# H263/review-based-recommender

Measured on AMD Instinct MI355X. Metric: (user,item) pairs/sec, DeepCoNN train step (fwd+MSE+bwd+clip+Adam), bsz256 2x512tok, higher is better.
Workload: dtype f32; 1 GPU; DeepCoNN cfg2: batch 256 pairs/GPU, 2x512-token docs, D=300, conv widths 3/5/7 x 50, latent 32, V=50002, fp32, Zipf ids; global_batch=256, parallelism=dp1, resident_batches=4, optimizer=HipClipAdam (clip + Adam, 2 launches; word-table gradient in compact row form)

## Files before the change

include/rbr_hip.h:

```cpp
#ifndef RBR_HIP_H
#define RBR_HIP_H

#include <stddef.h>
#include <stdint.h>

#ifdef __cplusplus
extern "C" {
#endif

#define RBR_MAX_WIDTHS 8

#define RBR_PAD_SAME 0
#define RBR_PAD_VALID 1
#define RBR_ACT_RELU 0
#define RBR_ACT_TANH 1

#define RBR_ERR_BAD_ARG (-1)
#define RBR_ERR_UNSUPPORTED (-2)

typedef struct rbr_textcnn_desc {
    int32_t n_docs;
    int32_t L;
    int32_t D;
    int32_t V;
    int32_t n_widths;
    int32_t kz[RBR_MAX_WIDTHS];
    int32_t ch[RBR_MAX_WIDTHS];
    int32_t pad_mode;
    int32_t act;
    int32_t padding_idx;
    int32_t flags;
} rbr_textcnn_desc;
#define RBR_CONV_PAD_RUNS 1
#define RBR_CONV_GATE_SPLIT(k) (((k) & 0xf) << 8)
#define RBR_CONV_GATE_SPLIT_OF(flags) (((flags) >> 8) & 0xf)
#define RBR_CONV_CLASS_STAMPED (1 << 19)
#define RBR_CONV_CLASS_PRECISION_OF(flags) (((flags) >> 16) & 0x3)
#define RBR_CONV_CLASS_T_BF16 (1 << 18)
void rbr_textcnn_desc_stamp(rbr_textcnn_desc* d);

int rbr_version(void);
const char* rbr_last_error(void);

int rbr_pair_begin(void);
int rbr_pair_next(void);
int rbr_pair_end(int32_t* n_paired, int32_t* n_single);
void rbr_pair_abort(void);


size_t rbr_textcnn_packed_floats(const rbr_textcnn_desc* d);
size_t rbr_textcnn_partial_elems(const rbr_textcnn_desc* d);

int rbr_textcnn_pack(const rbr_textcnn_desc* d, const float* const* W, float* packed, void* stream);

size_t rbr_textcnn_fwd_ws_bytes(const rbr_textcnn_desc* d);
void rbr_set_conv_mode(int32_t mode);
#define RBR_PROD_F32 0
#define RBR_PROD_BF16X3 1
#define RBR_PROD_BF16X2 2
#define RBR_PROD_BF16 3
void rbr_set_prod_precision(int32_t mode);
int32_t rbr_get_prod_precision(void);
void rbr_set_b16_storage(int32_t on);
int rbr_textcnn_conv_fwd(const rbr_textcnn_desc* d, const int64_t* ids, const uint8_t* mask, const float* gate,
                         const float* table, const float* const* W, const float* packed, float* pval, int32_t* pidx,
                         void* ws, void* stream);

int rbr_textcnn_prod_prepare(const rbr_textcnn_desc* d, const int64_t* ids, const uint8_t* mask, const float* const* W,
                             int32_t* pidx, void* ws, void* stream);
int rbr_textcnn_prod_table(const rbr_textcnn_desc* d, const float* table, void* ws, void* stream);
int rbr_textcnn_prod_pool(const rbr_textcnn_desc* d, const int64_t* ids, const uint8_t* mask, const float* gate,
                          float* pval, int32_t* pidx, void* ws, void* stream);
struct rbr_id_set;
int rbr_textcnn_prod_prepare_ids(const rbr_textcnn_desc* d, int32_t n_sets, const struct rbr_id_set* sets, int64_t* err,
                                 const int64_t* ids, const uint8_t* mask, const float* const* W, int32_t* pidx, void* ws,
                                 void* stream);

int rbr_textcnn_pool_finalize(const rbr_textcnn_desc* d, const float* pval, const int32_t* pidx,
                              const float* const* bias, float* feat, int32_t* argmax, void* stream);

size_t rbr_textcnn_bwd_ws_floats(const rbr_textcnn_desc* d);
int rbr_textcnn_bwd_dw(const rbr_textcnn_desc* d, const int64_t* ids, const uint8_t* mask, const float* gate,
                       const float* table, const float* feat, const int32_t* argmax, const float* d_feat,
                       float* const* dW, float* const* dbias, float* ws, void* stream);
int rbr_textcnn_bwd_dtable(const rbr_textcnn_desc* d, const int64_t* ids, const uint8_t* mask, const float* gate,
                           const float* table, const float* packed, const float* feat, const int32_t* argmax,
                           const float* d_feat, float* dtable, float* dgate, void* stream);
size_t rbr_textcnn_bwd_prod_ws_bytes(const rbr_textcnn_desc* d);
size_t rbr_textcnn_bwd_dtable_list_ws_bytes(const rbr_textcnn_desc* d);
int rbr_textcnn_bwd_dtable_list(const rbr_textcnn_desc* d, const int64_t* ids, const uint8_t* mask, const float* const* W,
                                const float* feat, const int32_t* argmax, const float* d_feat, void* ws, float* dtable,
                                void* stream);
#define RBR_G_BUILD 1
#define RBR_G_PRODUCT 2
#define RBR_G_ACCUMULATE 4
#define RBR_G_ROWS 8
#define RBR_G_ZEROED 16
int rbr_textcnn_bwd_dtable_prod_ex(const rbr_textcnn_desc* d, const int64_t* ids, const uint8_t* mask, const float* gate,
                                   const float* feat, const int32_t* argmax, const float* d_feat, void* fwd_ws, void* bwd_ws,
                                   float* dtable, float* dgate, float* sq_part, int32_t flags, void* stream);
size_t rbr_textcnn_row_grad_partials(const rbr_textcnn_desc* d);

int rbr_textcnn_token_list(const rbr_textcnn_desc* d, void* fwd_ws, const int32_t** row_of_token, const int32_t** n_rows,
                           const int64_t** tok_of_row, int32_t* cap);
size_t rbr_textcnn_bwd_dw_from_g_ws_floats(const rbr_textcnn_desc* d);
int rbr_textcnn_bwd_dw_from_g(const rbr_textcnn_desc* d, const float* table, const float* feat, const float* d_feat,
                              void* fwd_ws, void* bwd_ws, float* const* dW, float* const* dbias, float* ws, void* stream);
size_t rbr_textcnn_taps_count(const rbr_textcnn_desc* d);
int rbr_textcnn_bwd_taps(const rbr_textcnn_desc* d, const int64_t* ids, const uint8_t* mask, const float* feat,
                         const int32_t* argmax, const float* d_feat, int32_t* tok, float* val, void* stream);
size_t rbr_textcnn_dtable_from_taps_ws_bytes(const rbr_textcnn_desc* d, int32_t n_sets);
int rbr_textcnn_dtable_from_taps(const rbr_textcnn_desc* d, int32_t n_sets, const int32_t* tok, const float* val,
                                 const float* const* W, void* ws, float* dtable, void* stream);
int32_t rbr_textcnn_taps_owner_rows(const rbr_textcnn_desc* d, int32_t n_sets);
int rbr_textcnn_dtable_from_taps_owner(const rbr_textcnn_desc* d, int32_t n_sets, int32_t rank, const int32_t* tok,
                                       const float* val, const float* const* W, void* ws, float* slab, int32_t* overflow,
                                       void* stream);
int rbr_textcnn_bwd(const rbr_textcnn_desc* d, const int64_t* ids, const uint8_t* mask, const float* gate,
                    const float* table, const float* packed, const float* feat, const int32_t* argmax,
                    const float* d_feat, float* const* dW, float* const* dbias, float* dtable, float* dgate,
                    float* ws, void* stream);

int rbr_textcnn_saliency(const rbr_textcnn_desc* d, const int64_t* ids, const uint8_t* mask, const float* gate,
                         const float* table, const float* const* W, const float* feat, const int32_t* argmax,
                         const float* d_feat, float* sal, void* stream);

typedef struct rbr_head_params {
    const float* Wu; const float* bu; const float* Eu;
    const float* Wi; const float* bi; const float* Ei;
    const float* h;  const float* g;
    const float* ub; const float* ib;
} rbr_head_params;

typedef struct rbr_head_grads {
    float* dWu; float* dbu; float* dEu;
    float* dWi; float* dbi; float* dEi;
    float* dh;  float* dg;
    float* dub; float* dib;
} rbr_head_grads;

int rbr_pair_head_fwd(int32_t B, int32_t H, int32_t K, const float* u_feat, const float* i_feat,
                      const int64_t* u_id, const int64_t* i_id, const rbr_head_params* p, const float* drop,
                      float* ul, float* il, float* pred, void* stream);

int rbr_pair_head_fwd_train(int32_t B, int32_t H, int32_t K, const float* u_feat, const float* i_feat,
                            const int64_t* u_id, const int64_t* i_id, const rbr_head_params* p, float p_drop,
                            uint64_t seed, uint64_t* rng_state, float* drop_out, float* zero_buf, int64_t zero_n,
                            float* ul, float* il, float* pred, void* stream);

int rbr_pair_head_fwd_pool(const rbr_textcnn_desc* d, const float* pval, const int32_t* pidx, const float* const* bias,
                           float* feat, int32_t* argmax, const int64_t* first, int32_t K, const int64_t* u_id, const int64_t* i_id,
                           const rbr_head_params* p, const float* drop, float p_drop, uint64_t seed, uint64_t* rng_state,
                           float* drop_out, float* zero_buf, int64_t zero_n, float* ul, float* il, float* pred,
                           const float* target, float* loss, float* d_pred_unit, int32_t* ticket, void* stream);

size_t rbr_pair_head_fwd_pool_lds_bytes(const rbr_textcnn_desc* d, int32_t K, int32_t with_d_feat);
int rbr_pair_head_fwd_pool_ex(const rbr_textcnn_desc* d, const float* pval, const int32_t* pidx, const float* const* bias,
                              float* feat, int32_t* argmax, const int64_t* first, int32_t K, const int64_t* u_id, const int64_t* i_id,
                              const rbr_head_params* p, const float* drop, float p_drop, uint64_t seed, uint64_t* rng_state,
                              float* drop_out, float* zero_buf, int64_t zero_n, float* ul, float* il, float* pred,
                              const float* target, float* loss, float* d_pred_unit, int32_t* ticket, float* d_feat_unit,
                              void* stream);

size_t rbr_pair_head_bwd_ws_floats(int32_t B, int32_t K);
int rbr_pair_head_bwd(int32_t B, int32_t H, int32_t K, const float* u_feat, const float* i_feat,
                      const int64_t* u_id, const int64_t* i_id, const rbr_head_params* p, const float* drop,
                      const float* ul, const float* il, const float* d_pred, int32_t pad_u, int32_t pad_i,
                      const rbr_head_grads* g, float* d_ufeat, float* d_ifeat, float* ws, void* stream);
int rbr_dropout_multiplier(int64_t n, float p, uint64_t seed, uint64_t* state, float* out, void* stream);

int rbr_mse_loss_fwd(int64_t n, const float* pred, const float* target, float* loss, float* d_pred_unit, void* stream);
int rbr_pair_dot_fwd(int32_t B, int32_t K, const float* x, float* out, void* stream);
int rbr_pair_dot_bwd(int32_t B, int32_t K, const float* x, const float* d_out, float* d_x, void* stream);
int rbr_block_cat(int32_t B, int32_t C1, int32_t C2, const float* a, const float* b, const float* c, const float* d, float* out,
                  void* stream);
int rbr_block_split(int32_t B, int32_t C1, int32_t C2, const float* g, float* a, float* b, float* c, float* d, void* stream);
int rbr_mse_loss_bwd(int64_t n, const float* pred, const float* target, const float* d_loss, float* d_pred,
                     void* stream);

int rbr_bpr_loss_fwd(int32_t B, int32_t n_neg, const float* pred, const float* valid, float* loss, float* d_pred_unit,
                     void* stream);
int rbr_bpr_loss_bwd(int32_t B, int32_t n_neg, const float* pred, const float* valid, const float* d_loss, float* d_pred,
                     void* stream);

size_t rbr_pair_softmax_ws_bytes(int32_t B, int32_t K);
int rbr_pair_softmax_fwd(int32_t mode, int32_t B, int32_t K, const float* ul, const float* il, const float* h,
                         const float* row_bias, const float* col_bias, const float* drop, float p_drop, uint64_t seed,
                         uint64_t* rng_state, const int64_t* u_id, const int64_t* i_id, const int64_t* seen_off,
                         const int32_t* seen_item, int64_t seen_nnz, int32_t U, int64_t item_lo, const float* logq, float inv_temp,
                         float* loss, float* pos, float* d_ul, float* d_il, float* d_h, float* d_col_bias, float* d_row_bias,
                         uint64_t* call_out, void* ws, void* stream);
int rbr_pair_softmax_bwd(int32_t mode, int32_t B, int32_t K, const float* ul, const float* il, const float* h,
                         const float* row_bias, const float* col_bias, const float* drop, float p_drop, uint64_t seed,
                         const uint64_t* call, const int64_t* u_id, const int64_t* i_id, const int64_t* seen_off,
                         const int32_t* seen_item, int64_t seen_nnz, int32_t U, int64_t item_lo, const float* logq, float inv_temp,
                         const float* d_loss, float* pos_scratch, float* d_ul, float* d_il, float* d_h, float* d_col_bias,
                         float* d_row_bias, void* ws, void* stream);

typedef struct rbr_attn_params {
    const float* W_rv; const float* W_id; const float* h; const float* b1; const float* b2; const float* ebd;
} rbr_attn_params;

typedef struct rbr_attn_grads {
    float* dW_rv; float* dW_id; float* dh; float* db1; float* db2; float* debd;
} rbr_attn_grads;

int rbr_review_attn_fwd(int32_t B, int32_t R, int32_t H, int32_t A, const float* feat, const int64_t* other_id,
                        const rbr_attn_params* p, const float* drop, float* out, float* att, float* hid, void* stream);
size_t rbr_review_attn_bwd_ws_floats(int32_t B, int32_t R, int32_t H, int32_t A);
int rbr_review_attn_bwd(int32_t B, int32_t R, int32_t H, int32_t A, const float* feat, const int64_t* other_id,
                        const rbr_attn_params* p, const float* drop, const float* att, const float* hid, const float* d_out,
                        const float* d_att, int32_t pad_idx, const rbr_attn_grads* g, float* d_feat, float* ws,
                        void* stream);
int rbr_review_attn2_fwd(int32_t B, int32_t R, int32_t H, int32_t A, const float* feat, const int64_t* other_id,
                         const rbr_attn_params* p0, const rbr_attn_params* p1, const float* drop, float* out, float* att,
                         float* hid, void* stream);
int rbr_review_attn2_bwd(int32_t B, int32_t R, int32_t H, int32_t A, const float* feat, const int64_t* other_id,
                         const rbr_attn_params* p0, const rbr_attn_params* p1, const float* drop, const float* att,
                         const float* hid, const float* d_out, const float* d_att, int32_t pad_idx0, int32_t pad_idx1,
                         const rbr_attn_grads* g0, const rbr_attn_grads* g1, int64_t n_ebd0, int64_t n_ebd1, float* d_feat,
                         float* ws, void* stream);

int rbr_datt_local_gate_fwd(int32_t B, int32_t L, int32_t E, int32_t win, const int64_t* ids, const float* table,
                            const float* w, const float* b0, float* gate, void* stream);
int rbr_datt_global_gate_fwd(int32_t B, int32_t L, int32_t E, const int64_t* ids, const float* table,
                             const float* w, const float* b0, float* gate, void* stream);
size_t rbr_datt_gate_bwd_ws_floats(int32_t B, int32_t L, int32_t E, int32_t win, int32_t is_global);
size_t rbr_datt_local_gate_prod_ws_bytes(int32_t B, int32_t L, int32_t E, int32_t win, int32_t V);
int rbr_datt_local_gate_fwd_prod(int32_t B, int32_t L, int32_t E, int32_t win, int32_t V, const int64_t* ids, const float* table,
                                 const float* w, const float* b0, float* gate, void* ws, const void* rows, void* stream);
int rbr_datt_local_gate_bwd_prod(int32_t B, int32_t L, int32_t E, int32_t win, int32_t V, const int64_t* ids, const float* table,
                                 const float* w, const float* gate, const float* dgate, int32_t pad_idx, float* dw, float* db0,
                                 float* dtable, void* ws, const void* rows, int32_t accumulate, void* stream);
int rbr_datt_local_gate_bwd(int32_t B, int32_t L, int32_t E, int32_t win, const int64_t* ids, const float* table,
                            const float* w, const float* gate, const float* dgate, int32_t pad_idx, float* dw,
                            float* db0, float* dtable, float* ws, void* stream);
int rbr_datt_global_gate_bwd(int32_t B, int32_t L, int32_t E, const int64_t* ids, const float* table,
                             const float* w, const float* gate, const float* dgate, int32_t pad_idx, float* dw,
                             float* db0, float* dtable, float* ws, void* stream);
size_t rbr_datt_token_rows_ws_bytes(int32_t B, int32_t L, int32_t V);
int rbr_datt_token_rows(int32_t B, int32_t L, int32_t V, const int64_t* ids, void* rows, void* stream);
size_t rbr_datt_global_gate_bwd_rows_ws_floats(int32_t B, int32_t L, int32_t E, int32_t V);
int rbr_datt_global_gate_bwd_rows(int32_t B, int32_t L, int32_t E, int32_t V, const int64_t* ids, const float* table,
                                  const float* w, const float* gate, const float* dgate, int32_t pad_idx, float* dw,
                                  float* db0, float* dtable, float* ws, const void* rows, int32_t accumulate, void* stream);

int rbr_linear_fwd(int32_t N, int32_t IN, int32_t OUT, const float* x, const float* W, const float* b, int32_t relu,
                   const float* drop, float* y, void* stream);
size_t rbr_linear_bwd_ws_floats(int32_t N, int32_t OUT);
int rbr_linear_bwd(int32_t N, int32_t IN, int32_t OUT, const float* x, const float* W, const float* y, const float* d_y,
                   int32_t relu, const float* drop, float* d_x, float* dW, float* db, float* ws, void* stream);
// ... 104 lines not shown
```

review-based-recommender_amd/_lib.py:

```python
from __future__ import annotations

import ctypes as C
import os
import threading
from typing import Optional, Sequence

import torch

HERE = os.path.dirname(os.path.abspath(__file__))
LIB_PATH = os.environ.get("RBR_LIB_PATH") or os.path.join(HERE, "csrc", "librbr_hip.so")

RBR_MAX_WIDTHS = 8
PAD_SAME, PAD_VALID = 0, 1
ACT_RELU, ACT_TANH = 0, 1
PROD_F32, PROD_BF16X3, PROD_BF16X2, PROD_BF16 = 0, 1, 2, 3
SCORE_FM, SCORE_DOT = 0, 1
PROD_PRECISIONS = {"f32": PROD_F32, "bf16x3": PROD_BF16X3, "bf16x2": PROD_BF16X2, "bf16": PROD_BF16}

c_f32p = C.c_void_p
c_i64p = C.c_void_p
c_u8p = C.c_void_p
c_i32p = C.c_void_p
c_stream = C.c_void_p


class TextCNNDesc(C.Structure):
    _fields_ = [
        ("n_docs", C.c_int32), ("L", C.c_int32), ("D", C.c_int32), ("V", C.c_int32),
        ("n_widths", C.c_int32),
        ("kz", C.c_int32 * RBR_MAX_WIDTHS), ("ch", C.c_int32 * RBR_MAX_WIDTHS),
        ("pad_mode", C.c_int32), ("act", C.c_int32), ("padding_idx", C.c_int32), ("flags", C.c_int32),
    ]


class HeadParams(C.Structure):
    _fields_ = [(n, C.c_void_p) for n in ("Wu", "bu", "Eu", "Wi", "bi", "Ei", "h", "g", "ub", "ib")]


class HeadGrads(C.Structure):
    _fields_ = [(n, C.c_void_p) for n in ("dWu", "dbu", "dEu", "dWi", "dbi", "dEi", "dh", "dg", "dub", "dib")]


class AttnParams(C.Structure):
    _fields_ = [(n, C.c_void_p) for n in ("W_rv", "W_id", "h", "b1", "b2", "ebd")]


class IdSet(C.Structure):
    _fields_ = [("inp", C.c_void_p), ("out", C.c_void_p), ("n", C.c_int64), ("limit", C.c_int64), ("replace", C.c_int64)]


MAX_ID_SETS = 8


class RowGrad(C.Structure):
    _fields_ = [("tensor", C.c_int32), ("V", C.c_int32), ("D", C.c_int32), ("row_of_token", C.c_void_p), ("rows", C.c_void_p),
                ("sq_part", C.c_void_p), ("n_sq", C.c_int32), ("coef_out", C.c_void_p)]


G_BUILD, G_PRODUCT, G_ACCUMULATE, G_ROWS, G_ZEROED = 1, 2, 4, 8, 16


def conv_gate_split(k: int) -> int:
    return (int(k) & 0xF) << 8


class AttnGrads(C.Structure):
    _fields_ = [(n, C.c_void_p) for n in ("dW_rv", "dW_id", "dh", "db1", "db2", "debd")]


_PP = C.POINTER(C.c_void_p)
_DESC = C.POINTER(TextCNNDesc)
i32 = C.c_int32

SIGNATURES = {
    "rbr_version": (C.c_int, []),
    "rbr_last_error": (C.c_char_p, []),
    "rbr_pair_begin": (C.c_int, []),
    "rbr_pair_next": (C.c_int, []),
    "rbr_pair_end": (C.c_int, [C.POINTER(i32), C.POINTER(i32)]),
    "rbr_pair_abort": (None, []),
    "rbr_textcnn_packed_floats": (C.c_size_t, [_DESC]),
    "rbr_textcnn_partial_elems": (C.c_size_t, [_DESC]),
    "rbr_textcnn_pack": (C.c_int, [_DESC, _PP, c_f32p, c_stream]),
    "rbr_textcnn_fwd_ws_bytes": (C.c_size_t, [_DESC]),
    "rbr_set_conv_mode": (None, [i32]),
    "rbr_set_prod_precision": (None, [i32]),
    "rbr_get_prod_precision": (i32, []),
    "rbr_textcnn_desc_stamp": (None, [_DESC]),
    "rbr_set_b16_storage": (None, [i32]),
    "rbr_textcnn_conv_fwd": (C.c_int, [_DESC, c_i64p, c_u8p, c_f32p, c_f32p, _PP, c_f32p, c_f32p, c_i32p, C.c_void_p,
                                       c_stream]),
    "rbr_textcnn_prod_prepare": (C.c_int, [_DESC, c_i64p, c_u8p, _PP, c_i32p, C.c_void_p, c_stream]),
    "rbr_textcnn_prod_table": (C.c_int, [_DESC, c_f32p, C.c_void_p, c_stream]),
    "rbr_textcnn_prod_pool": (C.c_int, [_DESC, c_i64p, c_u8p, c_f32p, c_f32p, c_i32p, C.c_void_p, c_stream]),
    "rbr_textcnn_pool_finalize": (C.c_int, [_DESC, c_f32p, c_i32p, _PP, c_f32p, c_i32p, c_stream]),
    "rbr_textcnn_bwd_ws_floats": (C.c_size_t, [_DESC]),
    "rbr_textcnn_bwd_dw": (C.c_int, [_DESC, c_i64p, c_u8p, c_f32p, c_f32p, c_f32p, c_i32p, c_f32p, _PP, _PP, c_f32p,
                                     c_stream]),
    "rbr_textcnn_bwd_dtable": (C.c_int, [_DESC, c_i64p, c_u8p, c_f32p, c_f32p, c_f32p, c_f32p, c_i32p, c_f32p, c_f32p,
                                         c_f32p, c_stream]),
    "rbr_textcnn_bwd_prod_ws_bytes": (C.c_size_t, [_DESC]),
    "rbr_textcnn_bwd_dtable_prod_ex": (C.c_int, [_DESC, c_i64p, c_u8p, c_f32p, c_f32p, c_i32p, c_f32p, C.c_void_p, C.c_void_p,
                                                 c_f32p, c_f32p, c_f32p, i32, c_stream]),
    "rbr_textcnn_row_grad_partials": (C.c_size_t, [_DESC]),
    "rbr_textcnn_token_list": (C.c_int, [_DESC, C.c_void_p, _PP, _PP, _PP, C.POINTER(i32)]),
    "rbr_textcnn_prod_prepare_ids": (C.c_int, [_DESC, i32, C.POINTER(IdSet), C.c_void_p, c_i64p, c_u8p, _PP, c_i32p, C.c_void_p,
                                               c_stream]),
    "rbr_dedup_fold_rows": (C.c_int, [i32, i32, c_i64p, c_f32p, c_stream]),
    "rbr_pair_head_fwd_pool": (C.c_int, [_DESC, c_f32p, c_i32p, _PP, c_f32p, c_i32p, c_i64p, i32, c_i64p, c_i64p, C.POINTER(HeadParams),
                                         c_f32p, C.c_float, C.c_uint64, C.c_void_p, c_f32p, c_f32p, C.c_int64, c_f32p, c_f32p,
                                         c_f32p, c_f32p, c_f32p, c_f32p, c_i32p, c_stream]),
    "rbr_pair_head_fwd_pool_lds_bytes": (C.c_size_t, [_DESC, i32, i32]),
    "rbr_pair_head_fwd_pool_ex": (C.c_int, [_DESC, c_f32p, c_i32p, _PP, c_f32p, c_i32p, c_i64p, i32, c_i64p, c_i64p, C.POINTER(HeadParams),
                                            c_f32p, C.c_float, C.c_uint64, C.c_void_p, c_f32p, c_f32p, C.c_int64, c_f32p, c_f32p,
                                            c_f32p, c_f32p, c_f32p, c_f32p, c_i32p, c_f32p, c_stream]),
    "rbr_clip_adam_step_rows": (C.c_int, [i32, _PP, _PP, _PP, _PP, C.POINTER(C.c_int64), C.c_float, C.c_float, C.c_float,
                                          C.c_float, C.c_float, c_f32p, c_f32p, c_f32p, C.POINTER(RowGrad), c_stream]),
    "rbr_row_grad_to_dense": (C.c_int, [i32, i32, c_i32p, c_f32p, c_f32p, c_stream]),
    "rbr_textcnn_bwd_dtable_list_ws_bytes": (C.c_size_t, [_DESC]),
    "rbr_textcnn_bwd_dtable_list": (C.c_int, [_DESC, c_i64p, c_u8p, _PP, c_f32p, c_i32p, c_f32p, C.c_void_p, c_f32p, c_stream]),
    "rbr_textcnn_bwd_dw_from_g_ws_floats": (C.c_size_t, [_DESC]),
    "rbr_textcnn_bwd_dw_from_g": (C.c_int, [_DESC, c_f32p, c_f32p, c_f32p, C.c_void_p, C.c_void_p, _PP, _PP, c_f32p, c_stream]),
    "rbr_textcnn_taps_count": (C.c_size_t, [_DESC]),
    "rbr_textcnn_bwd_taps": (C.c_int, [_DESC, c_i64p, c_u8p, c_f32p, c_i32p, c_f32p, c_i32p, c_f32p, c_stream]),
    "rbr_textcnn_dtable_from_taps_ws_bytes": (C.c_size_t, [_DESC, i32]),
    "rbr_textcnn_dtable_from_taps": (C.c_int, [_DESC, i32, c_i32p, c_f32p, _PP, C.c_void_p, c_f32p, c_stream]),
    "rbr_textcnn_taps_owner_rows": (i32, [_DESC, i32]),
    "rbr_textcnn_dtable_from_taps_owner": (C.c_int, [_DESC, i32, i32, c_i32p, c_f32p, _PP, C.c_void_p, c_f32p, c_i32p, c_stream]),
    "rbr_textcnn_bwd": (C.c_int, [_DESC, c_i64p, c_u8p, c_f32p, c_f32p, c_f32p, c_f32p, c_i32p, c_f32p, _PP, _PP,
                                  c_f32p, c_f32p, c_f32p, c_stream]),
    "rbr_textcnn_saliency": (C.c_int, [_DESC, c_i64p, c_u8p, c_f32p, c_f32p, _PP, c_f32p, c_i32p, c_f32p, c_f32p, c_stream]),
    "rbr_datt_local_gate_prod_ws_bytes": (C.c_size_t, [i32, i32, i32, i32, i32]),
    "rbr_datt_local_gate_fwd_prod": (C.c_int, [i32, i32, i32, i32, i32, c_i64p, c_f32p, c_f32p, c_f32p, c_f32p, C.c_void_p,
                                               C.c_void_p, c_stream]),
    "rbr_datt_local_gate_bwd_prod": (C.c_int, [i32, i32, i32, i32, i32, c_i64p, c_f32p, c_f32p, c_f32p, c_f32p, i32, c_f32p,
                                               c_f32p, c_f32p, C.c_void_p, C.c_void_p, i32, c_stream]),
    "rbr_review_bag_fwd": (C.c_int, [i32, i32, i32, c_i64p, c_u8p, c_f32p, c_f32p, c_f32p, c_f32p, c_stream]),
    "rbr_review_bag_bwd_ws_bytes": (C.c_size_t, [i32, i32]),
    "rbr_review_bag_bwd": (C.c_int, [i32, i32, i32, i32, c_i64p, c_u8p, c_f32p, c_f32p, c_f32p, i32, c_f32p, C.c_void_p,
                                     c_stream]),
    "rbr_additive_attn_fwd": (C.c_int, [i32, i32, i32, i32, c_f32p, c_u8p, c_f32p, c_f32p, c_f32p, c_f32p, c_f32p, c_f32p,
                                        c_f32p, c_stream]),
    "rbr_additive_attn_bwd_ws_floats": (C.c_size_t, [i32, i32, i32, i32]),
    "rbr_additive_attn_bwd": (C.c_int, [i32, i32, i32, i32, c_f32p, c_u8p, c_f32p, c_f32p, c_f32p, c_f32p, c_f32p, c_f32p,
                                        c_f32p, c_f32p, c_f32p, c_f32p, c_f32p, c_stream]),
    "rbr_clip_adam_ws_floats": (C.c_size_t, []),
    "rbr_clip_adam_step": (C.c_int, [i32, _PP, _PP, _PP, _PP, C.POINTER(C.c_int64), C.c_float, C.c_float, C.c_float,
                                     C.c_float, C.c_float, c_f32p, c_f32p, c_f32p, c_stream]),
    "rbr_pair_head_fwd": (C.c_int, [i32, i32, i32, c_f32p, c_f32p, c_i64p, c_i64p, C.POINTER(HeadParams), c_f32p,
                                    c_f32p, c_f32p, c_f32p, c_stream]),
    "rbr_pair_head_fwd_train": (C.c_int, [i32, i32, i32, c_f32p, c_f32p, c_i64p, c_i64p, C.POINTER(HeadParams), C.c_float,
                                          C.c_uint64, C.c_void_p, c_f32p, c_f32p, C.c_int64, c_f32p, c_f32p, c_f32p, c_stream]),
    "rbr_pair_head_bwd_ws_floats": (C.c_size_t, [i32, i32]),
    "rbr_pair_head_bwd": (C.c_int, [i32, i32, i32, c_f32p, c_f32p, c_i64p, c_i64p, C.POINTER(HeadParams), c_f32p,
                                    c_f32p, c_f32p, c_f32p, i32, i32, C.POINTER(HeadGrads), c_f32p, c_f32p, c_f32p,
                                    c_stream]),
    "rbr_dropout_multiplier": (C.c_int, [C.c_int64, C.c_float, C.c_uint64, C.c_void_p, c_f32p, c_stream]),
    "rbr_mse_loss_fwd": (C.c_int, [C.c_int64, c_f32p, c_f32p, c_f32p, c_f32p, c_stream]),
    "rbr_pair_dot_fwd": (C.c_int, [i32, i32, c_f32p, c_f32p, c_stream]),
    "rbr_pair_dot_bwd": (C.c_int, [i32, i32, c_f32p, c_f32p, c_f32p, c_stream]),
    "rbr_block_cat": (C.c_int, [i32, i32, i32, c_f32p, c_f32p, c_f32p, c_f32p, c_f32p, c_stream]),
    "rbr_block_split": (C.c_int, [i32, i32, i32, c_f32p, c_f32p, c_f32p, c_f32p, c_f32p, c_stream]),
    "rbr_mse_loss_bwd": (C.c_int, [C.c_int64, c_f32p, c_f32p, c_f32p, c_f32p, c_stream]),
    "rbr_bpr_loss_fwd": (C.c_int, [i32, i32, c_f32p, c_f32p, c_f32p, c_f32p, c_stream]),
    "rbr_bpr_loss_bwd": (C.c_int, [i32, i32, c_f32p, c_f32p, c_f32p, c_f32p, c_stream]),
    "rbr_pair_softmax_ws_bytes": (C.c_size_t, [i32, i32]),
    "rbr_pair_softmax_fwd": (C.c_int, [i32, i32, i32, c_f32p, c_f32p, c_f32p, c_f32p, c_f32p, c_f32p, C.c_float, C.c_uint64,
                                       C.c_void_p, c_i64p, c_i64p, c_i64p, c_i32p, C.c_int64, i32, C.c_int64, c_f32p, C.c_float,
                                       c_f32p, c_f32p, c_f32p, c_f32p, c_f32p, c_f32p, c_f32p, C.c_void_p, C.c_void_p, c_stream]),
    "rbr_pair_softmax_bwd": (C.c_int, [i32, i32, i32, c_f32p, c_f32p, c_f32p, c_f32p, c_f32p, c_f32p, C.c_float, C.c_uint64,
                                       C.c_void_p, c_i64p, c_i64p, c_i64p, c_i32p, C.c_int64, i32, C.c_int64, c_f32p, C.c_float,
                                       c_f32p, c_f32p, c_f32p, c_f32p, c_f32p, c_f32p, c_f32p, C.c_void_p, c_stream]),
    "rbr_sample_negatives": (C.c_int, [i32, i32, i32, i32, c_i64p, c_i64p, c_i64p, c_i32p, C.c_int64, i32, C.c_uint64, C.c_void_p,
                                       i32, C.c_int64, c_i64p, c_i64p, c_f32p, c_stream]),
    "rbr_review_attn_fwd": (C.c_int, [i32, i32, i32, i32, c_f32p, c_i64p, C.POINTER(AttnParams), c_f32p, c_f32p, c_f32p,
                                      c_f32p, c_stream]),
    "rbr_review_attn_bwd_ws_floats": (C.c_size_t, [i32, i32, i32, i32]),
    "rbr_review_attn_bwd": (C.c_int, [i32, i32, i32, i32, c_f32p, c_i64p, C.POINTER(AttnParams), c_f32p, c_f32p, c_f32p,
                                      c_f32p, c_f32p, i32, C.POINTER(AttnGrads), c_f32p, c_f32p, c_stream]),
    "rbr_review_attn2_fwd": (C.c_int, [i32, i32, i32, i32, c_f32p, c_i64p, C.POINTER(AttnParams), C.POINTER(AttnParams), c_f32p,
                                       c_f32p, c_f32p, c_f32p, c_stream]),
    "rbr_review_attn2_bwd": (C.c_int, [i32, i32, i32, i32, c_f32p, c_i64p, C.POINTER(AttnParams), C.POINTER(AttnParams), c_f32p,
                                       c_f32p, c_f32p, c_f32p, c_f32p, i32, i32, C.POINTER(AttnGrads), C.POINTER(AttnGrads),
                                       C.c_int64, C.c_int64, c_f32p, c_f32p, c_stream]),
    "rbr_datt_local_gate_fwd": (C.c_int, [i32, i32, i32, i32, c_i64p, c_f32p, c_f32p, c_f32p, c_f32p, c_stream]),
    "rbr_datt_global_gate_fwd": (C.c_int, [i32, i32, i32, c_i64p, c_f32p, c_f32p, c_f32p, c_f32p, c_stream]),
    "rbr_datt_gate_bwd_ws_floats": (C.c_size_t, [i32, i32, i32, i32, i32]),
    "rbr_datt_local_gate_bwd": (C.c_int, [i32, i32, i32, i32, c_i64p, c_f32p, c_f32p, c_f32p, c_f32p, i32, c_f32p,
                                          c_f32p, c_f32p, c_f32p, c_stream]),
    "rbr_datt_global_gate_bwd": (C.c_int, [i32, i32, i32, c_i64p, c_f32p, c_f32p, c_f32p, c_f32p, i32, c_f32p,
                                           c_f32p, c_f32p, c_f32p, c_stream]),
    "rbr_datt_token_rows_ws_bytes": (C.c_size_t, [i32, i32, i32]),
    "rbr_datt_token_rows": (C.c_int, [i32, i32, i32, c_i64p, C.c_void_p, c_stream]),
    "rbr_datt_global_gate_bwd_rows_ws_floats": (C.c_size_t, [i32, i32, i32, i32]),
    "rbr_datt_global_gate_bwd_rows": (C.c_int, [i32, i32, i32, i32, c_i64p, c_f32p, c_f32p, c_f32p, c_f32p, i32, c_f32p,
                                                c_f32p, c_f32p, c_f32p, C.c_void_p, i32, c_stream]),
    "rbr_linear_fwd": (C.c_int, [i32, i32, i32, c_f32p, c_f32p, c_f32p, i32, c_f32p, c_f32p, c_stream]),
    "rbr_linear_bwd_ws_floats": (C.c_size_t, [i32, i32]),
    "rbr_linear_bwd": (C.c_int, [i32, i32, i32, c_f32p, c_f32p, c_f32p, c_f32p, i32, c_f32p, c_f32p, c_f32p, c_f32p,
                                 c_f32p, c_stream]),
    "rbr_linear_fwd_ws_floats": (C.c_size_t, [i32, i32, i32]),
    "rbr_linear_bwd_ex_ws_floats": (C.c_size_t, [i32, i32, i32]),
    "rbr_linear_fwd_ex": (C.c_int, [i32, i32, i32, c_f32p, c_f32p, c_f32p, i32, c_f32p, c_f32p, c_f32p, c_stream]),
    "rbr_linear_bwd_ex": (C.c_int, [i32, i32, i32, c_f32p, c_f32p, c_f32p, c_f32p, i32, c_f32p, c_f32p, c_f32p, c_f32p,
                                    c_f32p, c_stream]),
    "rbr_conv_shift_add_fwd": (C.c_int, [i32, i32, i32, C.POINTER(i32), C.POINTER(i32), c_f32p, _PP, c_f32p, c_stream]),
    "rbr_conv_shift_add_bwd": (C.c_int, [i32, i32, i32, C.POINTER(i32), C.POINTER(i32), c_f32p, c_f32p, _PP, c_stream]),
    "rbr_sanitize_ids": (C.c_int, [i32, C.POINTER(IdSet), C.c_void_p, c_stream]),
    "rbr_dedup_ws_bytes": (C.c_size_t, [i32, i32]),
    "rbr_dedup_rows": (C.c_int, [i32, i32, c_i64p, c_i64p, i32, i32, c_u8p, C.c_void_p, c_i64p, c_u8p, c_stream]),
    "rbr_doc_gather": (C.c_int, [i32, i32, c_i64p, c_i64p, c_i32p, i32, c_i32p, i32, C.c_int64, C.c_int64, c_i64p, c_u8p, c_i64p,
                                 c_i64p, c_stream]),
    "rbr_review_gather": (C.c_int, [i32, i32, i32, c_i64p, c_i64p, c_i32p, c_i32p, i32, c_i32p, c_i32p, i32, i32, C.c_int64, C.c_int64,
                                    c_i64p, c_u8p, c_u8p, c_i64p, c_i64p, c_i64p, c_stream]),
    "rbr_pair_score_ids": (C.c_int, [i32, i32, i32, c_f32p, i32, c_f32p, i32, c_i64p, c_i64p, c_f32p, c_f32p, c_f32p, c_f32p, c_f32p,
                                     c_i64p, c_stream]),
    "rbr_pair_score_dense": (C.c_int, [i32, i32, i32, i32, c_f32p, c_f32p, c_f32p, c_f32p, c_f32p, c_f32p, c_f32p, c_stream]),
    "rbr_pair_score_topk_ws_bytes": (C.c_size_t, [i32, i32, i32, i32]),
    "rbr_pair_score_topk": (C.c_int, [i32, i32, i32, i32, i32, i32, c_f32p, c_f32p, c_f32p, c_f32p, c_f32p, c_f32p, c_i64p, c_i32p,
                                      C.c_int64, c_i64p, i32, c_i64p, c_f32p, C.c_void_p, c_stream]),
    "rbr_pair_score_rank_ws_bytes": (C.c_size_t, [i32, i32, i32]),
    "rbr_pair_score_rank": (C.c_int, [i32, i32, i32, i32, i32, c_f32p, c_f32p, c_f32p, c_f32p, c_f32p, c_f32p, c_i64p, c_i64p, c_i32p,
                                      C.c_int64, c_i64p, i32, c_i32p, c_i32p, c_i64p, C.c_void_p, c_stream]),
    "rbr_embedding_fwd": (C.c_int, [C.c_int64, i32, c_i64p, c_f32p, c_f32p, c_stream]),
    "rbr_embedding_bwd": (C.c_int, [C.c_int64, i32, c_i64p, c_f32p, i32, c_f32p, c_stream]),
    "rbr_hier_pool_fwd": (C.c_int, [i32, i32, i32, i32, c_i64p, c_u8p, c_f32p, i32, c_f32p, c_i32p, c_stream]),
    "rbr_hier_pool_bwd": (C.c_int, [i32, i32, i32, i32, c_i64p, c_u8p, c_i32p, c_f32p, c_f32p, i32, i32, c_f32p,
                                    c_stream]),
}

_lib = None
_lock = threading.Lock()


def lib() -> C.CDLL:
    global _lib
    if _lib is not None:
        return _lib
    with _lock:
# ... 121 lines not shown
```

review-based-recommender_amd/csrc/pair_head.hip:

```cpp
#include "rbr_common.h"

#include <algorithm>

namespace rbr {

__device__ __forceinline__ void head_dl(float su, float si, float dr, float dp, float hk, float& dul, float& dil, float& zdp) {
    const float prod = su * si;
    const float dz = (prod > 0.f) ? dp * hk * dr : 0.f;
    dul = dz * si;
    dil = dz * su;
    zdp = fmaxf(prod, 0.f) * dr * dp;
}

__device__ __forceinline__ void head_pair_dfeat(int H, int K, const float* ulb, const float* ilb, const float* drb, float dp,
                                                const rbr_head_params& p, float* s_dul, float* s_dil, float* d_uf, float* d_if) {
    const int t = threadIdx.x;
    for (int k = t; k < K; k += 256) {
        const float dr = (drb != nullptr) ? drb[k] : 1.f;
        float dul, dil, zdp;
        head_dl(ulb[k], ilb[k], dr, dp, p.h[k], dul, dil, zdp);
        s_dul[k] = dul;
        s_dil[k] = dil;
    }
    __syncthreads();
// ... 142 lines not shown
__global__ __launch_bounds__(256) void head_fwd_pool_kernel(const ConvPlan P, const HeadPool hp, int B, int K,
                                                            const long long* __restrict__ uid, const long long* __restrict__ iid,
                                                            const rbr_head_params p, const float* __restrict__ drop,
                                                            float* __restrict__ ul, float* __restrict__ il, float* __restrict__ pred,
                                                            const HeadTrain tr, const HeadMse mse, float* __restrict__ d_feat_unit) {
    __shared__ float s_part[2][4][32];
    __shared__ float s_l[2][32];
    __shared__ int s_last;
    __shared__ float s_dp;
    extern __shared__ __attribute__((aligned(16))) float s_feat[];
    const int b = blockIdx.x, t = threadIdx.x;
    if (b >= B) {
        for (long k = (long)(b - B) * 256 + t; k < tr.zero_n; k += (long)(gridDim.x - B) * 256) tr.zero_buf[k] = 0.f;
        if (t == 0) head_rng_ticket(tr, 0);
        return;
    }
    const int* flags = hp.pidx + (long)P.total_wt * P.nslots_total;
    const int nslots = P.ntiles * kTile, wpd = P.wpd;
    float* s_val = s_feat + 2 * P.C;
    int* s_flag = reinterpret_cast<int*>(s_val + 2 * wpd * nslots);
    __shared__ short s_chan[kMaxSlots];
    __shared__ unsigned char s_sw[kMaxSlots], s_skz[kMaxSlots];
    __shared__ int s_choff[RBR_MAX_WIDTHS];
    __shared__ const float* s_biasp[RBR_MAX_WIDTHS];
    static_assert(kMaxSlots <= 256, "one thread per slot below");
    if (t < kMaxSlots) { s_chan[t] = P.slot_chan[t]; s_sw[t] = P.slot_w[t]; s_skz[t] = P.slot_kz[t]; }
    if (t < RBR_MAX_WIDTHS) { s_choff[t] = P.ch_off[t]; s_biasp[t] = hp.bias.p[t]; }
    __shared__ int s_src[2];
    if (t < 2) s_src[t] = hp.first != nullptr ? (int)hp.first[t * B + b] : t * B + b;
    __syncthreads();
    for (int i = t; i < 2 * wpd; i += 256) {
        const int side = i >= wpd, w = side ? i - wpd : i;
        s_flag[i] = flags[s_src[side] * wpd + w];
    }
    __syncthreads();
    const float NEG = -__builtin_huge_valf();
    for (int i = t; i < 2 * wpd * nslots; i += 256) {
        const int side = i >= wpd * nslots, r = side ? i - wpd * nslots : i;
        const int w = r / nslots, ls = r - w * nslots;
        const long base = ((long)s_src[side] * wpd + w) * P.nslots_total + (long)P.tile_base * kTile + ls;
        float v = NEG;
        if (s_chan[ls] >= 0) {
            const int Lv = (P.pad_mode == RBR_PAD_VALID) ? (P.L - (int)s_skz[ls] + 1) : P.L;
            const int fl = s_flag[side * wpd + w];
            v = (fl == 1) ? hp.pval[base] : ((fl == 0 && w * kTile < Lv) ? 0.f : NEG);
        }
        s_val[i] = v;
    }
    __syncthreads();
    for (int idx = t; idx < 2 * nslots; idx += 256) {
        const int side = idx >= nslots, ls = side ? idx - nslots : idx;
        const int doc = side * B + b;
        const int chan = s_chan[ls];
        if (chan < 0) continue;
        float best = NEG;
        int bw_tile = -1;
        for (int w = 0; w < wpd; ++w) {
            const float v = s_val[(side * wpd + w) * nslots + ls];
            if (v > best) { best = v; bw_tile = w; }
        }
        int bidx = 0;
        if (bw_tile >= 0) {
            if (s_flag[side * wpd + bw_tile] == 1) bidx = hp.pidx[((long)s_src[side] * wpd + bw_tile) * P.nslots_total + (long)P.tile_base * kTile + ls];
            else bidx = bw_tile * kTile;
        }
        const int bw = s_sw[ls];
        const float y = best + s_biasp[bw][chan - s_choff[bw]];
        const float f = (P.act == RBR_ACT_RELU) ? fmaxf(y, 0.f) : tanhf(y);
        hp.feat[(long)doc * P.C + chan] = f;
        hp.argmax[(long)doc * P.C + chan] = bidx;
        s_feat[side * P.C + chan] = f;
    }
    __syncthreads();
    float* s_bwd = d_feat_unit != nullptr ? s_feat + ((2 * P.C + 2 * wpd * nslots + 2 * wpd + 3) & ~3) : nullptr;
    const float pr = head_pair(b, B, P.C, K, s_feat, s_feat + P.C, uid, iid, p, drop, ul, il, pred, tr, s_part, s_l, s_bwd);
    if (mse.target == nullptr) return;
    if (d_feat_unit != nullptr) {
        const int K4 = (K + 3) & ~3;
        if (t == 0) s_dp = (pr - mse.target[b]) * (2.f / (float)B);
        __syncthreads();
        head_pair_dfeat(P.C, K, s_bwd, s_bwd + K4, s_bwd + 2 * K4, s_dp, p, s_bwd, s_bwd + K4, d_feat_unit + (long)b * P.C,
                        d_feat_unit + (long)(B + b) * P.C);
    }
    if (t == 0) {
        __threadfence();
        s_last = atomicAdd(mse.ticket, 1) == B - 1;
    }
    __syncthreads();
    if (!s_last) return;
    __threadfence();
    float acc = 0.f;
    for (int i = t; i < B; i += 256) {
        const float d = __hip_atomic_load(pred + i, __ATOMIC_RELAXED, __HIP_MEMORY_SCOPE_AGENT) - mse.target[i];
        acc += d * d;
        if (mse.d_unit != nullptr) mse.d_unit[i] = d * (2.f / (float)B);
    }
    acc = wave_sum(acc);
    __syncthreads();
    if ((t & 63) == 0) s_l[0][t >> 6] = acc;
    __syncthreads();
    if (t == 0) {
        *mse.loss = (s_l[0][0] + s_l[0][1] + s_l[0][2] + s_l[0][3]) / (float)B;
        *mse.ticket = 0;
    }
}

__global__ __launch_bounds__(256) void head_bwd_kernel(int B, int H, int K, const float* __restrict__ uf,
                                                       const float* __restrict__ itf, const long long* __restrict__ uid,
                                                       const long long* __restrict__ iid, const rbr_head_params p,
                                                       const float* __restrict__ drop, const float* __restrict__ ul,
                                                       const float* __restrict__ il, const float* __restrict__ d_pred,
                                                       int pad_u, int pad_i, const rbr_head_grads g,
                                                       float* __restrict__ d_uf, float* __restrict__ d_if) {
    extern __shared__ __attribute__((aligned(16))) float sm[];
    const int t = threadIdx.x;
    if ((int)blockIdx.x < B) {
        const int K4 = (K + 3) & ~3;
        const int b = blockIdx.x;
        float* s_dul = sm;
        float* s_dil = sm + K4;
        const long u = uid[b], it = iid[b];
        const float dp = d_pred[b];
        head_pair_dfeat(H, K, ul + (long)b * K, il + (long)b * K, drop != nullptr ? drop + (long)b * K : nullptr, dp, p, s_dul, s_dil,
                        d_uf != nullptr ? d_uf + (long)b * H : nullptr, d_uf != nullptr ? d_if + (long)b * H : nullptr);
        for (int k = t; k < K; k += 256) {
            if (u != pad_u) atomicAdd(g.dEu + u * K + k, s_dul[k]);
            if (it != pad_i) atomicAdd(g.dEi + it * K + k, s_dil[k]);
        }
        if (t == 0) {
            if (u != pad_u) atomicAdd(g.dub + u, dp);
            if (it != pad_i) atomicAdd(g.dib + it, dp);
        }
        return;
    }
    float (*red)[8][32] = reinterpret_cast<float (*)[8][32]>(sm);
    const int rows = H + 1;
    const int rb = blockIdx.x - B;
    const int side = rb / rows, r = rb % rows;
    const int kk = t & 31, grp = t >> 5;
    const float* ft = side ? itf : uf;
    for (int k0 = 0; k0 < K; k0 += 32) {
        const int k = k0 + kk;
        float s = 0.f, hs = 0.f, gs = 0.f;
        if (k < K) {
            const float hk = p.h[k];
            for (int b0 = grp; b0 < B; b0 += 64) {
                float vu[8], vi[8], vd[8], vp[8], vf[8];
#pragma unroll
                for (int u = 0; u < 8; ++u) {
                    const int b = b0 + 8 * u;
                    const bool ok = b < B;
                    const long bb = ok ? b : grp;
                    vu[u] = ul[bb * K + k];
                    vi[u] = il[bb * K + k];
                    vd[u] = (drop != nullptr) ? drop[bb * K + k] : 1.f;
                    vp[u] = ok ? d_pred[bb] : 0.f;
                    vf[u] = (r < H) ? ft[bb * H + r] : 0.f;
                }
#pragma unroll
                for (int u = 0; u < 8; ++u) {
                    float dul, dil, zdp;
                    head_dl(vu[u], vi[u], vd[u], vp[u], hk, dul, dil, zdp);
                    const float dl = side ? dil : dul;
                    if (r < H) {
                        s = fmaf(vf[u], dl, s);
                    } else {
                        s += dl;
                        if (side == 0) {
                            hs += zdp;
                            if (k == 0) gs += vp[u];
                        }
                    }
                }
            }
        }
        __syncthreads();
        red[0][grp][kk] = s; red[1][grp][kk] = hs; red[2][grp][kk] = gs;
        __syncthreads();
        if (grp == 0 && k < K) {
            float a = 0.f, bsum = 0.f, c = 0.f;
#pragma unroll
            for (int q = 0; q < 8; ++q) { a += red[0][q][kk]; bsum += red[1][q][kk]; c += red[2][q][kk]; }
            if (r < H) {
                (side ? g.dWi : g.dWu)[(long)r * K + k] = a;
            } else {
                (side ? g.dbi : g.dbu)[k] = a;
                if (side == 0) {
                    g.dh[k] = bsum;
                    if (k == 0) g.dg[0] = c;
                }
            }
        }
    }
}

}

using namespace rbr;

static bool head_args_ok(int B, int H, int K) {
    if (B <= 0 || H <= 0 || K <= 0) { set_error("bad head shape B=%d H=%d K=%d", B, H, K); return false; }
    return true;
}

namespace rbr {
__global__ __launch_bounds__(256) void mse_fwd_kernel(long n, const float* __restrict__ pred, const float* __restrict__ target,
                                                      float* __restrict__ loss, float* __restrict__ d_unit) {
    __shared__ float s_red[4];
    float acc = 0.f;
    for (long i = threadIdx.x; i < n; i += 256) {
        const float d = pred[i] - target[i];
        acc += d * d;
        if (d_unit != nullptr) d_unit[i] = d * (2.f / (float)n);
    }
    acc = wave_sum(acc);
    if ((threadIdx.x & 63) == 0) s_red[threadIdx.x >> 6] = acc;
    __syncthreads();
    if (threadIdx.x == 0) *loss = (s_red[0] + s_red[1] + s_red[2] + s_red[3]) / (float)n;
}

__global__ __launch_bounds__(256) void mse_bwd_kernel(long n, const float* __restrict__ pred, const float* __restrict__ target,
                                                      const float* __restrict__ d_loss, float* __restrict__ d_pred) {
    const long i = (long)blockIdx.x * 256 + threadIdx.x;
    if (i < n) d_pred[i] = (pred[i] - target[i]) * (2.f / (float)n) * d_loss[0];
}

__device__ __forceinline__ float bpr_softplus(float x) { return fmaxf(x, 0.f) + log1pf(expf(-fabsf(x))); }
__device__ __forceinline__ float bpr_sigmoid(float x) {
    const float e = expf(-fabsf(x));
    return x >= 0.f ? 1.f / (1.f + e) : e / (1.f + e);
}

__global__ __launch_bounds__(256) void bpr_loss_kernel(int B, int n_neg, const float* __restrict__ pred, const float* __restrict__ valid,
                                                       const float* __restrict__ d_loss, float* __restrict__ loss,
                                                       float* __restrict__ d_pred) {
    __shared__ float s_red[2][4];
    float acc = 0.f, cnt = 0.f;
    for (int b = threadIdx.x; b < B; b += 256) {
        const float p = pred[b];
        for (int j = 0; j < n_neg; ++j) {
// ... 55 lines not shown
extern "C" int rbr_bpr_loss_fwd(int32_t B, int32_t n_neg, const float* pred, const float* valid, float* loss, float* d_pred_unit,
                                void* stream) {
    if (!bpr_args_ok("bpr_loss_fwd", B, n_neg, pred)) return RBR_ERR_BAD_ARG;
    if (!loss) { set_error("bpr_loss_fwd: null pointer"); return RBR_ERR_BAD_ARG; }
    hipLaunchKernelGGL(rbr::bpr_loss_kernel, dim3(1), dim3(256), 0, (hipStream_t)stream, B, n_neg, pred, valid,
                       (const float*)nullptr, loss, d_pred_unit);
    RBR_CHECK_LAUNCH("bpr_loss_fwd launch");
    return 0;
}

extern "C" int rbr_bpr_loss_bwd(int32_t B, int32_t n_neg, const float* pred, const float* valid, const float* d_loss, float* d_pred,
                                void* stream) {
    if (!bpr_args_ok("bpr_loss_bwd", B, n_neg, pred)) return RBR_ERR_BAD_ARG;
    if (!d_loss || !d_pred) { set_error("bpr_loss_bwd: null pointer"); return RBR_ERR_BAD_ARG; }
    hipLaunchKernelGGL(rbr::bpr_loss_kernel, dim3(1), dim3(256), 0, (hipStream_t)stream, B, n_neg, pred, valid, d_loss,
                       (float*)nullptr, d_pred);
    RBR_CHECK_LAUNCH("bpr_loss_bwd launch");
    return 0;
}

extern "C" int rbr_pair_head_fwd(int32_t B, int32_t H, int32_t K, const float* u_feat, const float* i_feat,
                                 const int64_t* u_id, const int64_t* i_id, const rbr_head_params* p, const float* drop,
                                 float* ul, float* il, float* pred, void* stream) {
    if (!head_args_ok(B, H, K)) return RBR_ERR_BAD_ARG;
    if (!u_feat || !i_feat || !u_id || !i_id || !p || !ul || !il || !pred) { set_error("null pointer"); return RBR_ERR_BAD_ARG; }
    hipLaunchKernelGGL(head_fwd_kernel, dim3(B), dim3(256), 0, (hipStream_t)stream, B, H, K, u_feat, i_feat,
                       reinterpret_cast<const long long*>(u_id), reinterpret_cast<const long long*>(i_id), *p, drop, ul,
                       il, pred, HeadTrain{});
    RBR_CHECK_LAUNCH("pair_head_fwd launch");
    return 0;
}

extern "C" int rbr_pair_head_fwd_train(int32_t B, int32_t H, int32_t K, const float* u_feat, const float* i_feat,
                                       const int64_t* u_id, const int64_t* i_id, const rbr_head_params* p, float p_drop,
                                       uint64_t seed, uint64_t* rng_state, float* drop_out, float* zero_buf, int64_t zero_n,
                                       float* ul, float* il, float* pred, void* stream) {
    if (!head_args_ok(B, H, K)) return RBR_ERR_BAD_ARG;
    if (!u_feat || !i_feat || !u_id || !i_id || !p || !ul || !il || !pred) { set_error("null pointer"); return RBR_ERR_BAD_ARG; }
    if (!(p_drop >= 0.f && p_drop < 1.f)) { set_error("pair_head_fwd_train: p_drop=%f outside [0,1)", (double)p_drop); return RBR_ERR_BAD_ARG; }
    if (p_drop > 0.f && (!rng_state || !drop_out)) { set_error("pair_head_fwd_train: dropout needs rng_state and drop_out"); return RBR_ERR_BAD_ARG; }
    if (zero_n < 0 || (zero_n > 0 && !zero_buf)) { set_error("pair_head_fwd_train: bad zero buffer"); return RBR_ERR_BAD_ARG; }
    HeadTrain tr{};
    tr.p_drop = p_drop; tr.seed = seed;
    tr.rng_state = (p_drop > 0.f) ? reinterpret_cast<unsigned long long*>(rng_state) : nullptr;
    tr.drop_out = drop_out; tr.zero_buf = zero_buf; tr.zero_n = zero_n;
    const int zblocks = zero_n > 0 ? (int)std::min<long>((zero_n + 1023) / 1024, 256) : 0;
    hipLaunchKernelGGL(head_fwd_kernel, dim3(B + zblocks), dim3(256), 0, (hipStream_t)stream, B, H, K, u_feat, i_feat,
                       reinterpret_cast<const long long*>(u_id), reinterpret_cast<const long long*>(i_id), *p,
                       static_cast<const float*>(nullptr), ul, il, pred, tr);
    RBR_CHECK_LAUNCH("pair_head_fwd_train launch");
    return 0;
}

static size_t head_fwd_pool_lds(const ConvPlan& P, int K, bool with_d_feat) {
    size_t lds = ((size_t)2 * P.C + (size_t)2 * P.wpd * P.ntiles * kTile + (size_t)2 * P.wpd) * sizeof(float);
    if (with_d_feat) lds = ((lds + 15) & ~(size_t)15) + (size_t)3 * ((K + 3) & ~3) * sizeof(float);
    return lds;
}

extern "C" size_t rbr_pair_head_fwd_pool_lds_bytes(const rbr_textcnn_desc* d, int32_t K, int32_t with_d_feat) {
    ConvPlan plans[kMaxGroups];
    if (K <= 0 || build_plans(d, plans, kMaxTiles) != 1) return 0;
    const size_t lds = head_fwd_pool_lds(plans[0], K, with_d_feat != 0);
    return lds > 60 * 1024 ? 0 : lds;
}

extern "C" int rbr_pair_head_fwd_pool_ex(const rbr_textcnn_desc* d, const float* pval, const int32_t* pidx, const float* const* bias,
                                         float* feat, int32_t* argmax, const int64_t* first, int32_t K, const int64_t* u_id,
                                         const int64_t* i_id, const rbr_head_params* p, const float* drop, float p_drop, uint64_t seed,
                                         uint64_t* rng_state, float* drop_out, float* zero_buf, int64_t zero_n, float* ul, float* il,
                                         float* pred, const float* target, float* loss, float* d_pred_unit, int32_t* ticket,
                                         float* d_feat_unit, void* stream) {
    ConvPlan plans[kMaxGroups];
    const int ng = build_plans(d, plans, kMaxTiles);
    if (!ng) return RBR_ERR_BAD_ARG;
    if (ng != 1) { set_error("pair_head_fwd_pool: %d channel groups (one launch covers %d slots)", ng, kMaxSlots); return RBR_ERR_UNSUPPORTED; }
    if (d->n_docs % 2) { set_error("pair_head_fwd_pool: odd document count %d", d->n_docs); return RBR_ERR_BAD_ARG; }
    const int B = d->n_docs / 2, C = plans[0].C;
    if (!head_args_ok(B, C, K)) return RBR_ERR_BAD_ARG;
    if (!pval || !pidx || !bias || !feat || !argmax || !u_id || !i_id || !p || !ul || !il || !pred) { set_error("null pointer"); return RBR_ERR_BAD_ARG; }
    if (!(p_drop >= 0.f && p_drop < 1.f)) { set_error("pair_head_fwd_pool: p_drop=%f outside [0,1)", (double)p_drop); return RBR_ERR_BAD_ARG; }
    if (p_drop > 0.f && (!rng_state || !drop_out)) { set_error("pair_head_fwd_pool: dropout needs rng_state and drop_out"); return RBR_ERR_BAD_ARG; }
    if (zero_n < 0 || (zero_n > 0 && !zero_buf)) { set_error("pair_head_fwd_pool: bad zero buffer"); return RBR_ERR_BAD_ARG; }
    if (target != nullptr && (!loss || !ticket)) { set_error("pair_head_fwd_pool: the loss needs loss and ticket"); return RBR_ERR_BAD_ARG; }
    if (d_feat_unit != nullptr && !target) { set_error("pair_head_fwd_pool: d_feat_unit needs the loss target"); return RBR_ERR_BAD_ARG; }
    HeadTrain tr{};
    tr.p_drop = p_drop; tr.seed = seed;
    tr.rng_state = (p_drop > 0.f) ? reinterpret_cast<unsigned long long*>(rng_state) : nullptr;
    tr.drop_out = drop_out; tr.zero_buf = zero_buf; tr.zero_n = zero_n;
    HeadPool hp{};
    hp.pval = pval; hp.pidx = pidx; hp.feat = feat; hp.argmax = argmax; hp.first = reinterpret_cast<const long long*>(first);
    for (int w = 0; w < d->n_widths; ++w) hp.bias.p[w] = bias[w];
    HeadMse mse{target, loss, d_pred_unit, ticket};
    const int zblocks = zero_n > 0 ? (int)std::min<long>((zero_n + 1023) / 1024, 256) : 0;
    const size_t lds = head_fwd_pool_lds(plans[0], K, d_feat_unit != nullptr);
    if (lds > 60 * 1024) { set_error("pair_head_fwd_pool: %zu bytes of LDS for the slab partials (documents too long)", lds); return RBR_ERR_UNSUPPORTED; }
    hipLaunchKernelGGL(head_fwd_pool_kernel, dim3(B + zblocks), dim3(256), lds, (hipStream_t)stream,
                       plans[0], hp, B, K, reinterpret_cast<const long long*>(u_id), reinterpret_cast<const long long*>(i_id), *p,
                       (p_drop > 0.f) ? nullptr : drop, ul, il, pred, tr, mse, d_feat_unit);
    RBR_CHECK_LAUNCH("pair_head_fwd_pool launch");
    return 0;
}

extern "C" int rbr_pair_head_fwd_pool(const rbr_textcnn_desc* d, const float* pval, const int32_t* pidx, const float* const* bias,
                                      float* feat, int32_t* argmax, const int64_t* first, int32_t K, const int64_t* u_id,
                                      const int64_t* i_id, const rbr_head_params* p, const float* drop, float p_drop, uint64_t seed,
                                      uint64_t* rng_state, float* drop_out, float* zero_buf, int64_t zero_n, float* ul, float* il,
                                      float* pred, const float* target, float* loss, float* d_pred_unit, int32_t* ticket, void* stream) {
    return rbr_pair_head_fwd_pool_ex(d, pval, pidx, bias, feat, argmax, first, K, u_id, i_id, p, drop, p_drop, seed, rng_state, drop_out,
                                     zero_buf, zero_n, ul, il, pred, target, loss, d_pred_unit, ticket, nullptr, stream);
}

extern "C" size_t rbr_pair_head_bwd_ws_floats(int32_t B, int32_t K) { (void)B; (void)K; return 0; }

extern "C" int rbr_pair_head_bwd(int32_t B, int32_t H, int32_t K, const float* u_feat, const float* i_feat,
                                 const int64_t* u_id, const int64_t* i_id, const rbr_head_params* p, const float* drop,
                                 const float* ul, const float* il, const float* d_pred, int32_t pad_u, int32_t pad_i,
                                 const rbr_head_grads* g, float* d_ufeat, float* d_ifeat, float* ws, void* stream) {
    if (!head_args_ok(B, H, K)) return RBR_ERR_BAD_ARG;
    if (!u_feat || !i_feat || !u_id || !i_id || !p || !ul || !il || !d_pred || !g || (!d_ufeat != !d_ifeat)) {
        set_error("null pointer");
        return RBR_ERR_BAD_ARG;
    }
    (void)ws;
    const size_t lds = std::max((size_t)2 * ((K + 3) & ~3), (size_t)3 * 8 * 32) * sizeof(float);
    hipLaunchKernelGGL(head_bwd_kernel, dim3((unsigned)(B + 2 * (H + 1))), dim3(256), lds, (hipStream_t)stream, B, H, K, u_feat,
                       i_feat, reinterpret_cast<const long long*>(u_id), reinterpret_cast<const long long*>(i_id), *p, drop,
                       ul, il, d_pred, pad_u, pad_i, *g, d_ufeat, d_ifeat);
    RBR_CHECK_LAUNCH("pair_head_bwd launch");
    return 0;
}

namespace rbr {
__global__ __launch_bounds__(256) void pair_dot_fwd_kernel(int B, int K, const float* __restrict__ x, float* __restrict__ out) {
    const int b = blockIdx.x * 16 + (threadIdx.x >> 4), l = threadIdx.x & 15;
    float s = 0.f;
    if (b < B)
        for (int k = l; k < K; k += 16) s = fmaf(x[(long)b * K + k], x[(long)(B + b) * K + k], s);
    s = wave_sum<16>(s);
    if (b < B && l == 0) out[b] = s;
}

__global__ __launch_bounds__(256) void pair_dot_bwd_kernel(int B, int K, const float* __restrict__ x, const float* __restrict__ d_out,
                                                           float* __restrict__ d_x) {
    const long n = (long)2 * B * K;
    for (long e = (long)blockIdx.x * 256 + threadIdx.x; e < n; e += (long)gridDim.x * 256) {
        const int row = (int)(e / K), k = (int)(e - (long)row * K);
        const int b = row < B ? row : row - B, other = row < B ? row + B : row - B;
        d_x[e] = d_out[b] * x[(long)other * K + k];
    }
}
}

extern "C" int rbr_pair_dot_fwd(int32_t B, int32_t K, const float* x, float* out, void* stream) {
    if (B <= 0 || K <= 0 || !x || !out) { set_error("bad pair_dot arguments"); return RBR_ERR_BAD_ARG; }
    hipLaunchKernelGGL(pair_dot_fwd_kernel, dim3((B + 15) / 16), dim3(256), 0, (hipStream_t)stream, B, K, x, out);
    RBR_CHECK_LAUNCH("pair_dot fwd launch");
    return 0;
}

extern "C" int rbr_pair_dot_bwd(int32_t B, int32_t K, const float* x, const float* d_out, float* d_x, void* stream) {
    if (B <= 0 || K <= 0 || !x || !d_out || !d_x) { set_error("bad pair_dot arguments"); return RBR_ERR_BAD_ARG; }
    const long n = (long)2 * B * K;
    hipLaunchKernelGGL(pair_dot_bwd_kernel, dim3((unsigned)std::min<long>((n + 255) / 256, 2048)), dim3(256), 0, (hipStream_t)stream, B, K,
                       x, d_out, d_x);
    RBR_CHECK_LAUNCH("pair_dot bwd launch");
    return 0;
}
```

review-based-recommender_amd/csrc/rbr_common.h:

```cpp
#pragma once

#include <hip/hip_runtime.h>

#include <algorithm>
#include <cstdarg>
#include <cstdio>
#include <cstring>

#include "../../include/rbr_hip.h"
#include "rbr_launch.h"
#include "rbr_wave.h"

namespace rbr {

constexpr int kWave = 64;
constexpr int kTile = 32;
constexpr int kMaxTiles = 8;
constexpr int kMaxGroups = 32;
constexpr int kMaxSlots = kMaxTiles * kTile;
constexpr int kMaxKF = 9;
constexpr int kMaxDim = 1 << 14;
constexpr int kMaxChannels = kMaxGroups * kMaxTiles * kTile;
constexpr int kMaxPieces = kMaxTiles * kMaxKF;
constexpr int kWavesPerWG = 4;
// ... 5 lines not shown
    int KF;
    int P;
    int DC;
    int nchunks;
    int wpd;
    int total_wt;
    int nslots_total;
    int tile_base;
    int group;
    int store_rows;
    int ntiles;
    int npieces;
    int pad_mode, act;
    int tiles_total;
    int piece_st[kMaxPieces];
    short slot_chan[kMaxSlots];
    unsigned char slot_w[kMaxSlots];
    unsigned char slot_off[kMaxSlots];
    unsigned char slot_kz[kMaxSlots];
    int n_widths;
    int kz[RBR_MAX_WIDTHS], ch[RBR_MAX_WIDTHS], ch_off[RBR_MAX_WIDTHS];
    int gate_split;
    int pad_runs;
};

struct PtrArray {
    const float* p[RBR_MAX_WIDTHS];
};
struct MutPtrArray {
    float* p[RBR_MAX_WIDTHS];
};

__device__ __forceinline__ float act_grad(int act, float f, float d) {
    return (act == RBR_ACT_RELU) ? (f > 0.f ? d : 0.f) : d * (1.f - f * f);
}

void set_error(const char* fmt, ...);
int check_hip(hipError_t e, const char* what);

bool desc_valid(const rbr_textcnn_desc* d);
int build_plans(const rbr_textcnn_desc* d, ConvPlan* plans , int tiles_per_group = 5);
constexpr int kProdGroupTiles = 8;

int run_conv_groups(const ConvPlan* plans, int ngroups, const long long* ids, const unsigned char* mask, const float* gate,
                    const float* table, const float* packed, float* pval, int* pidx, const int* sched, hipStream_t st);
int run_token_product(const rbr_textcnn_desc* d, const long long* ids, const unsigned char* mask, const float* gate,
                      const float* table, const float* const* W, float* pval, int* pidx, void* ws, hipStream_t st);
int forced_conv_mode();
int prod_precision();
int prod_precision_of(const rbr_textcnn_desc* d);
bool prod_b16_applicable(const rbr_textcnn_desc* d);
int prod_b16_groups(int cp_real);
size_t prod_b16_image_bytes(const rbr_textcnn_desc* d, int cp_real);
struct B16Pack;
B16Pack prod_b16_pack_job(const rbr_textcnn_desc* d);
int prod_b16_gemm(const rbr_textcnn_desc* d, int cp_real, int cap, int pitch, const int* counter, const long long* tok_of_row,
                  const float* table, const void* bimg, void* T, void* a16, hipStream_t st);
bool prod_b16_rows_applicable(const rbr_textcnn_desc* d);
size_t prod_b16_rows_image_bytes(int KG, int D);
long prod_b16_rows_image_items(int KG, int D);
int prod_b16_rows_partials(int cap, int D);
int prod_b16_rows_gemm(int KG, int D, int cap, const int* counter, const float* G, const void* bimg_t, float* rows, float* sq_part, bool plain_bf16,
                       hipStream_t st);
bool prod_t_bf16(const rbr_textcnn_desc* d);
size_t prod_b16_rows_bytes(const rbr_textcnn_desc* d, int cap);
struct ZeroRegions {
    int* p[3];
    long n[3];
};
int zero_regions(const ZeroRegions& r, hipStream_t st);
inline int zero_words(void* p, size_t bytes, hipStream_t st) {
    ZeroRegions r{{static_cast<int*>(p), nullptr, nullptr}, {(long)(bytes / sizeof(int)), 0, 0}};
    return zero_regions(r, st);
}

struct IdSets {
    const long long* in[RBR_MAX_ID_SETS];
    long long* out[RBR_MAX_ID_SETS];
    long long n[RBR_MAX_ID_SETS], limit[RBR_MAX_ID_SETS], replace[RBR_MAX_ID_SETS];
    long long first[RBR_MAX_ID_SETS + 1];
    int count;
};
int fill_id_sets(int n_sets, const rbr_id_set* sets, IdSets& S);
__device__ __forceinline__ void sanitize_id(const IdSets& S, long long k, long long* __restrict__ err) {
    int s = 0;
#pragma unroll
    for (int q = 1; q < RBR_MAX_ID_SETS; ++q)
        if (q < S.count && k >= S.first[q]) s = q;
    const long long e = k - S.first[s];
    long long v = S.in[s][e];
    const bool bad = (unsigned long long)v >= (unsigned long long)S.limit[s];
    if (bad) {
        err[1] = v; err[2] = s;
        atomicAdd(reinterpret_cast<unsigned long long*>(err), 1ull);
        v = S.replace[s];
    }
    S.out[s][e] = v;
}

constexpr int kSlabDup = 2;
constexpr int kPadRunHalo = 8;
__device__ __forceinline__ void tile_scan_block(const ConvPlan& P, const unsigned char* __restrict__ mask,
                                                int* __restrict__ sched, int blk, const long long* __restrict__ ids = nullptr) {
    const int wt = blk * 256 + threadIdx.x;
    int act = 0;
    if (wt < P.total_wt) {
        act = 1;
        if (mask != nullptr) {
            const int doc = wt / P.wpd, l0 = (wt % P.wpd) * kTile;
            const int lo = max(0, l0 - P.P), hi = min(P.L, l0 + kTile + P.KF - 1 - P.P);
            act = 0;
            const unsigned char* row = mask + (long)doc * P.L;
            if (l0 + kTile <= P.L && ((((uintptr_t)(row + l0)) & 15) == 0)) {
                const uint4 a = *reinterpret_cast<const uint4*>(row + l0), c = *reinterpret_cast<const uint4*>(row + l0 + 16);
                unsigned halo = 0;
                for (int p = lo; p < l0; ++p) halo |= row[p];
                for (int p = l0 + kTile; p < hi; ++p) halo |= row[p];
                act = (a.x | a.y | a.z | a.w | c.x | c.y | c.z | c.w | halo) != 0;
            } else {
                for (int p = lo; p < hi; ++p) act |= mask[(long)doc * P.L + p];
            }
            act = act ? 1 : 0;
        }
        sched[wt] = act;
    }
    if (mask == nullptr && ids != nullptr && P.pad_runs >= 0) {
        __shared__ unsigned char s_own[256];
        bool own = false;
        if (wt < P.total_wt) {
            const int doc = wt / P.wpd, l0 = (wt % P.wpd) * kTile;
            const int lo = l0 - P.P - kPadRunHalo, hi = l0 + kTile + P.KF - 1 - P.P + kPadRunHalo;
            if (lo >= 0 && hi <= P.L) {
                const long long* row = ids + (long)doc * P.L;
                const long long pad = (long long)P.pad_runs;
                own = true;
                int p = lo;
                if ((((uintptr_t)(row + p)) & 15) == 0) {
                    for (; p + 16 <= hi && own; p += 16) {
                        longlong2 t[8];
#pragma unroll
                        for (int u = 0; u < 8; ++u) t[u] = *reinterpret_cast<const longlong2*>(row + p + 2 * u);
#pragma unroll
                        for (int u = 0; u < 8; ++u) own = own && t[u].x == pad && t[u].y == pad;
                    }
                }
                for (; p < hi && own; ++p) own = row[p] == pad;
            }
        }
        s_own[threadIdx.x] = own ? 1 : 0;
        __syncthreads();
        if (wt < P.total_wt && own && (wt % P.wpd) != 0) {
            bool prev;
            if (threadIdx.x > 0) {
                prev = s_own[threadIdx.x - 1] != 0;
            } else {
                const int doc = wt / P.wpd, l0 = (wt % P.wpd - 1) * kTile;
                const int lo = l0 - P.P - kPadRunHalo, hi = l0 + kTile + P.KF - 1 - P.P + kPadRunHalo;
                prev = lo >= 0 && hi <= P.L;
                for (int q = lo; q < hi && prev; ++q) prev = ids[(long)doc * P.L + q] == (long long)P.pad_runs;
            }
            if (prev) { act = kSlabDup; sched[wt] = act; }
        }
    }
    const unsigned long long b = __ballot(act == 1);
    act = act == 1;
    const int lane = threadIdx.x & 63;
    int base = 0;
    if (lane == 0 && b) base = atomicAdd(sched + 2 * (long)P.total_wt, __popcll(b));
    base = __shfl(base, 0);
    if (act) sched[(long)P.total_wt + base + __popcll(b & ((1ull << lane) - 1))] = wt;
}
int scan_tiles(const ConvPlan& p, const unsigned char* mask, int* sched, hipStream_t st);

inline int choose_dc(int D) {
    if (D % 4 != 0) return 20;
    const int cands[3] = {60, 52, 20};
    int best_pad = 1 << 30;
    for (int c : cands) best_pad = std::min(best_pad, ((D + c - 1) / c) * c);
    for (int c : cands)
        if (((D + c - 1) / c) * c * 100 <= best_pad * 108) return c;
    return 20;
}


__device__ __forceinline__ void philox_round(unsigned& c0, unsigned& c1, unsigned& c2, unsigned& c3, unsigned k0, unsigned k1) {
    const unsigned long long p0 = 0xD2511F53ull * c0, p1 = 0xCD9E8D57ull * c2;
    const unsigned n0 = (unsigned)(p1 >> 32) ^ c1 ^ k0, n1 = (unsigned)p1;
    const unsigned n2 = (unsigned)(p0 >> 32) ^ c3 ^ k1, n3 = (unsigned)p0;
    c0 = n0; c1 = n1; c2 = n2; c3 = n3;
}

__device__ __forceinline__ void philox4x32_10(unsigned long long quad, unsigned long long call, unsigned long long seed,
                                              unsigned& c0, unsigned& c1, unsigned& c2, unsigned& c3) {
    c0 = (unsigned)quad; c1 = (unsigned)(quad >> 32); c2 = (unsigned)call; c3 = (unsigned)(call >> 32);
    unsigned k0 = (unsigned)seed, k1 = (unsigned)(seed >> 32);
#pragma unroll
    for (int r = 0; r < 10; ++r) {
        philox_round(c0, c1, c2, c3, k0, k1);
        k0 += 0x9E3779B9u; k1 += 0xBB67AE85u;
    }
}
__device__ __forceinline__ bool dropout_keep(unsigned word, float p) {
    return (float)(word >> 8) * (1.f / 16777216.f) >= p;
}

}

#define RBR_CHECK_LAUNCH(what)                                   \
    do {                                                         \
        int _e = rbr::check_hip(hipGetLastError(), what);        \
        if (_e) return _e;                                       \
        if (rbr::pair_region_open()) {                           \
            rbr::set_error("%s: this entry point launches directly and cannot be used inside rbr_pair_begin / rbr_pair_end", what); \
            return RBR_ERR_UNSUPPORTED;                          \
        }                                                        \
    } while (0)
```

review-based-recommender_amd/csrc/textcnn_prod.hip:

```cpp
#include "rbr_common.h"
#include "textcnn_b16.h"

#include <rocprim/rocprim.hpp>

#include <algorithm>
#include <cstdlib>

namespace rbr {

struct ProdArgs {
    int n_docs, L, V, cap;
    int zrow;
    int pitch;
    int poff[RBR_MAX_WIDTHS];
    int rank_off[RBR_MAX_WIDTHS];
    int cp_real;
};
RBR_SHARED_KERNEL_ARG(ProdArgs);

__device__ __forceinline__ void mark_scan_kernel(const ConvPlan& P, int nb_scan, long n_tok, const long long* __restrict__ ids,
                                                        const unsigned char* __restrict__ mask, int* __restrict__ sched,
                                                        unsigned char* __restrict__ used) {
    if ((int)blockIdx.x < nb_scan) {
        tile_scan_block(P, mask, sched, blockIdx.x, ids);
        return;
    }
    const long nb = gridDim.x - nb_scan;
    for (long k = (long)(blockIdx.x - nb_scan) * 256 + threadIdx.x; k < n_tok; k += nb * 256)
        if (mask == nullptr || mask[k]) used[ids[k]] = 1;
}

__global__ __launch_bounds__(256) void prep_kernel(const IdSets S, long long* __restrict__ err, const ZeroRegions R, int nb_ids) {
    if ((int)blockIdx.x < nb_ids) {
        const long long total = S.first[S.count];
        for (long long k = (long long)blockIdx.x * 256 + threadIdx.x; k < total; k += (long long)nb_ids * 256) sanitize_id(S, k, err);
        return;
    }
    const long nz = R.n[0] + R.n[1] + R.n[2], nb = gridDim.x - nb_ids;
    for (long k = (long)(blockIdx.x - nb_ids) * 256 + threadIdx.x; k < nz; k += nb * 256) {
        if (k < R.n[0]) R.p[0][k] = 0;
        else if (k < R.n[0] + R.n[1]) R.p[1][k - R.n[0]] = 0;
        else R.p[2][k - R.n[0] - R.n[1]] = 0;
    }
}

struct PackJob {
    ConvPlan P;
    int n_widths, D, cp_real;
    int kz[RBR_MAX_WIDTHS], ch[RBR_MAX_WIDTHS], poff[RBR_MAX_WIDTHS];
};

__device__ __forceinline__ float prod_weight(const PackJob& J, const PtrArray& W, int pc, int d) {
    int w = 0;
#pragma unroll
    for (int k = 1; k < RBR_MAX_WIDTHS; ++k)
        if (k < J.n_widths && pc >= J.poff[k]) w = k;
    const int rel = pc - J.poff[w];
    const int j = rel / J.ch[w], cl = rel - j * J.ch[w];
    return W.p[w][((long)cl * J.D + d) * J.kz[w] + j];
}

__device__ __forceinline__ void compact_pack_kernel(const PackJob& J, int nb_compact, int V, int cap,
                                                           const unsigned char* __restrict__ used, int* __restrict__ row_of_token,
                                                           long long* __restrict__ tok_of_row, unsigned char* __restrict__ row_mask,
                                                           int* __restrict__ counter, float* __restrict__ zero_row, int pitch,
                                                           const PtrArray& W, float* __restrict__ packed, float* __restrict__ WT,
                                                           const B16Pack& JB, unsigned char* __restrict__ bimg) {
    if ((int)blockIdx.x < nb_compact) {
        if (blockIdx.x == 0)
            for (int k = threadIdx.x; k < pitch; k += 256) zero_row[k] = 0.f;
        __shared__ int s_cnt[4], s_wave[4];
        const int lane = threadIdx.x & 63, wave = threadIdx.x >> 6;
        const int below = blockIdx.x * 256;
        int c = 0;
        const int4* u4 = reinterpret_cast<const int4*>(used);
        for (int q = threadIdx.x; q < below / 16; q += 256) {
            const int4 m = u4[q];
            c += __popc(m.x) + __popc(m.y) + __popc(m.z) + __popc(m.w);
        }
        c = wave_sum(c);
        const int v = below + threadIdx.x;
        const int u = (v < V) ? used[v] : 0;
        const unsigned long long b = __ballot(u);
        if (lane == 0) { s_cnt[wave] = c; s_wave[wave] = __popcll(b); }
        __syncthreads();
        int base = (s_cnt[0] + s_cnt[1]) + (s_cnt[2] + s_cnt[3]);
        for (int k = 0; k < wave; ++k) base += s_wave[k];
        if (v < V) {
            int row = -1;
            if (u) {
                row = base + __popcll(b & ((1ull << lane) - 1));
                if (row < cap) { tok_of_row[row] = v; row_mask[row] = 1; } else row = -1;
            }
            row_of_token[v] = row;
        }
        if ((int)blockIdx.x == nb_compact - 1 && threadIdx.x == 0)
            *counter = (s_cnt[0] + s_cnt[1]) + (s_cnt[2] + s_cnt[3]) + s_wave[0] + s_wave[1] + s_wave[2] + s_wave[3];
        return;
    }
    const long nb = gridDim.x - nb_compact, b0 = blockIdx.x - nb_compact;
    const ConvPlan& P = J.P;
    const int DC = P.DC;
    const long n_img = packed != nullptr ? (long)P.nchunks * P.tiles_total * kTile * DC : 0;
    const long n_wt = (long)J.cp_real * J.D;
    const long n_b16 = bimg != nullptr ? b16_pack_items(JB) : 0;
    for (long idx = b0 * 256 + threadIdx.x; idx < n_img + n_wt + n_b16; idx += nb * 256) {
        if (idx >= n_img + n_wt) {
            b16_pack_item(JB, W, bimg, idx - n_img - n_wt);
        } else if (idx < n_img) {
            long r = idx;
            const int dd = (int)(r % DC); r /= DC;
            const int slot = (int)(r % kTile); r /= kTile;
            const int t = (int)(r % P.tiles_total);
            const int dc = (int)(r / P.tiles_total);
            const int pc = t * kTile + slot;
            const int d = dc * DC + dd;
            packed[idx] = (pc < J.cp_real && d < J.D) ? prod_weight(J, W, pc, d) : 0.f;
        } else {
            const long e = idx - n_img;
            const int pc = (int)(e / J.D), d = (int)(e - (long)pc * J.D);
            WT[e] = prod_weight(J, W, pc, d);
        }
    }
}

typedef float f32x4 __attribute__((ext_vector_type(4)));
typedef float f32x4u __attribute__((ext_vector_type(4), aligned(4)));

typedef unsigned u32x2u __attribute__((ext_vector_type(2), aligned(2)));
template <bool TB16>
__device__ __forceinline__ void gather_pool_kernel(const ConvPlan& P, const ProdArgs& A, const long long* __restrict__ ids,
                                                          const unsigned char* __restrict__ mask, const float* __restrict__ gate,
                                                          const int* __restrict__ row_of_token, const void* __restrict__ Tv,
                                                          const int* __restrict__ sched, float* __restrict__ pval,
                                                          int* __restrict__ pidx) {
    const float* T = static_cast<const float*>(Tv);
    const unsigned short* T16 = static_cast<const unsigned short*>(Tv);
    __shared__ int s_row[kWavesPerWG][kTile + kMaxKF];
    __shared__ float s_gate[kWavesPerWG][kTile + kMaxKF];
    __shared__ float s_gate_b[kWavesPerWG][kTile + kMaxKF];
    const int wave = threadIdx.x >> 6, lane = threadIdx.x & 63;
    const int n_active = sched[2 * (long)P.total_wt];
    const int slot_in_list = blockIdx.x * kWavesPerWG + wave;
    if (slot_in_list >= n_active) return;
    const int wt = sched[P.total_wt + slot_in_list];
    const int doc = wt / P.wpd, l0 = (wt % P.wpd) * kTile;
    const int L = P.L, XR = kTile + P.KF - 1;
    for (int r = lane; r < XR; r += 64) {
        const int p = l0 - P.P + r;
        int row = A.zrow;
        float gv = 1.f, gvb = 1.f;
        if (p >= 0 && p < L) {
            const long tok = (long)doc * L + p;
            if (mask == nullptr || mask[tok]) {
                const int rr = row_of_token[ids[tok]];
                row = rr >= 0 ? rr : A.zrow;
                if (gate != nullptr) {
                    gv = gate[tok];
                    if (P.gate_split > 0) gvb = gate[(long)P.n_docs * L + tok];
                }
            }
        }
        s_row[wave][r] = row;
        s_gate[wave][r] = gv;
        s_gate_b[wave][r] = gvb;
    }
    __builtin_amdgcn_wave_barrier();
    const float NEG = -__builtin_huge_valf();
    for (int w = 0; w < P.n_widths; ++w) {
        const int kz = P.kz[w], ch = P.ch[w];
        const int off = (P.pad_mode == RBR_PAD_SAME) ? (P.KF - kz) / 2 : 0;
        const int Lv = (P.pad_mode == RBR_PAD_VALID) ? (L - kz + 1) : L;
        const int nquads = (ch + 3) >> 2;
        const int lq = nquads <= 16 ? 4 : (nquads <= 32 ? 5 : 6);
        const int QL = 1 << lq, PS = 64 >> lq;
        const int ps = lane >> lq, ql = lane & (QL - 1);
        const float* sg = (P.gate_split > 0 && w >= P.gate_split) ? s_gate_b[wave] : s_gate[wave];
        for (int qb = 0; qb < nquads; qb += QL) {
            const int q = qb + ql;
            const bool valid = q < nquads;
            const float* tcol = T + A.poff[w] + 4 * (valid ? q : 0);
            const unsigned short* tcol16 = T16 + A.poff[w] + 4 * (valid ? q : 0);
            float best[4] = {NEG, NEG, NEG, NEG};
            int bidx[4] = {0x7fffffff, 0x7fffffff, 0x7fffffff, 0x7fffffff};
            for (int p0 = 0; p0 < kTile; p0 += 2 * PS) {
                f32x4 y[2] = {{0.f, 0.f, 0.f, 0.f}, {0.f, 0.f, 0.f, 0.f}};
#pragma unroll
                for (int j = 0; j < kMaxKF; ++j) {
                    if (j < kz) {
#pragma unroll
                        for (int u = 0; u < 2; ++u) {
                            const int r = p0 + PS * u + ps + j + off;
                            f32x4 v;
                            if (TB16) {
                                const u32x2u b = *reinterpret_cast<const u32x2u*>(tcol16 + (long)s_row[wave][r] * A.pitch + j * ch);
                                v = f32x4{__uint_as_float(b.x << 16), __uint_as_float(b.x & 0xffff0000u),
                                          __uint_as_float(b.y << 16), __uint_as_float(b.y & 0xffff0000u)};
                            } else {
                                v = *reinterpret_cast<const f32x4u*>(tcol + (long)s_row[wave][r] * A.pitch + j * ch);
                            }
                            const float gv = sg[r];
                            y[u].x = fmaf(v.x, gv, y[u].x); y[u].y = fmaf(v.y, gv, y[u].y);
                            y[u].z = fmaf(v.z, gv, y[u].z); y[u].w = fmaf(v.w, gv, y[u].w);
                        }
                    }
                }
// ... 974 lines not shown
        A.t_pitch = pp[0].nslots_total;
    }
    int cp_real = 0;
    for (int w = 0; w < d->n_widths; ++w) {
        A.kz[w] = d->kz[w]; A.ch[w] = d->ch[w]; A.ch_off[w] = plans[0].ch_off[w];
        A.poff[w] = cp_real; cp_real += d->kz[w] * d->ch[w];
    }
    const bool want_g = dtable != nullptr || !(phases & kGProduct);
    if (phases & kGBuild) {
        if ((want_g && !(phases & kGZeroed)) || dgate != nullptr || B.rows_gemm) {
            const long n_img = B.rows_gemm ? prod_b16_rows_image_items(B.KG, d->D) : 0;
            const int nb_zero = 2048, nb_img = (int)std::min<long>((n_img + 255) / 256, 1024);
            if (int e_ = rbr::launch<zero_g_rows_kernel, 256>(dim3(nb_zero + nb_img), dim3(256), 0, st, "textcnn zero_g_rows launch", counter, Lo.cap, B.KG / 4, (want_g && !(phases & kGZeroed)) ? reinterpret_cast<f32x4*>(G) : nullptr, dgate, dgate != nullptr ? (long)d->n_docs * d->L * (RBR_CONV_GATE_SPLIT_OF(d->flags) ? 2 : 1) : 0L, nb_zero, WT, cp_real, d->D, n_img, reinterpret_cast<unsigned char*>(static_cast<char*>(bwd_ws) + B.bimg_t))) return e_;
        }
        const long n_items = (long)d->n_docs * A.C * A.KF;
        if (int e_ = rbr::launch<build_g_kernel, 256>(dim3((unsigned)((n_items + 255) / 256)), dim3(256), 0, st, "textcnn build_g launch", A, reinterpret_cast<const long long*>(ids), mask, gate, row_of_token, T, feat, argmax, d_feat, want_g ? G : nullptr, dgate, prod_t_bf16(d) ? 1 : 0)) return e_;
    }
    if (dtable == nullptr || !(phases & kGProduct)) return 0;
    const size_t lds = (size_t)B.KGW * 8 * kWavesPerWG + (size_t)kWavesPerWG * d->D * sizeof(float);
    const dim3 grid((unsigned)std::min(Lo.cap, kGtwMaxBlocks));
    if (phases & kGRows) {
        if (sq_part == nullptr) { set_error("compact row gradient needs sq_part"); return RBR_ERR_BAD_ARG; }
        if (B.rows_gemm)
            return prod_b16_rows_gemm(B.KG, d->D, Lo.cap, counter, G, static_cast<char*>(bwd_ws) + B.bimg_t, dtable, sq_part,
                                      prod_precision_of(d) == RBR_PROD_BF16, st);
        if (int e_ = rbr::launch<g_times_w_kernel<kGtwRows>, 256>(grid, dim3(256), lds, st, "textcnn g_times_w launch", A, B.KGW, counter, G, WT, tok_of_row, row_of_token, d->V, dtable, sq_part)) return e_;
    } else if (phases & kGAccumulate) {
        if (int e_ = rbr::launch<g_times_w_kernel<kGtwAccumulate>, 256>(grid, dim3(256), lds, st, "textcnn g_times_w launch", A, B.KGW, counter, G, WT, tok_of_row, row_of_token, d->V, dtable, (float*)nullptr)) return e_;
    } else {
        if (int e_ = rbr::launch<g_times_w_kernel<kGtwDense>, 256>(grid, dim3(256), lds, st, "textcnn g_times_w launch", A, B.KGW, counter, G, WT, tok_of_row, row_of_token, d->V, dtable, (float*)nullptr)) return e_;
    }
    return 0;
}

namespace {

struct ProdState {
    ProdLayout Lo;
    ConvPlan pp[kMaxGroups];
    ProdArgs A;
    unsigned char* used;
    int *row_of_token, *counter, *sched_p;
    long long* tok_of_row;
    unsigned char* row_mask;
    float *packed_p, *WT, *T;
    char* base;
};

int prod_state(const rbr_textcnn_desc* d, void* ws, ProdState& S) {
    if (ws == nullptr) { set_error("null workspace"); return RBR_ERR_BAD_ARG; }
    if (!prod_applicable(d)) { set_error("token-product path does not apply to this shape"); return RBR_ERR_UNSUPPORTED; }
    if (!prod_layout(d, S.Lo)) return RBR_ERR_BAD_ARG;
    const ProdLayout& Lo = S.Lo;
    S.base = static_cast<char*>(ws);
    S.used = reinterpret_cast<unsigned char*>(S.base + Lo.used);
    S.row_of_token = reinterpret_cast<int*>(S.base + Lo.row_of_token);
    S.tok_of_row = reinterpret_cast<long long*>(S.base + Lo.tok_of_row);
    S.row_mask = reinterpret_cast<unsigned char*>(S.base + Lo.row_mask);
    S.counter = reinterpret_cast<int*>(S.base + Lo.counter);
    S.sched_p = reinterpret_cast<int*>(S.base + Lo.sched);
    S.packed_p = reinterpret_cast<float*>(S.base + Lo.packed);
    S.WT = reinterpret_cast<float*>(S.base + Lo.wt);
    S.T = reinterpret_cast<float*>(S.base + Lo.table_T);
    if (!build_plans(&S.Lo.dp, S.pp, kProdGroupTiles)) return RBR_ERR_BAD_ARG;
    S.pp[0].store_rows = 1;
    ProdArgs A{};
    A.n_docs = d->n_docs; A.L = d->L; A.V = d->V; A.cap = Lo.cap; A.zrow = Lo.cap; A.pitch = S.pp[0].nslots_total;
    int o = 0;
    for (int w = 0; w < d->n_widths; ++w) { A.poff[w] = o; o += d->kz[w] * d->ch[w]; }
    A.cp_real = o;
    for (int w = 0; w < d->n_widths; ++w) {
        int r = 0;
        for (int v = 0; v < d->n_widths; ++v)
            if (d->kz[v] < d->kz[w] || (d->kz[v] == d->kz[w] && v < w)) r += d->ch[v];
        A.rank_off[w] = r;
    }
    S.A = A;
    return 0;
}

}

static int prod_prepare(const rbr_textcnn_desc* d, const int64_t* ids, const uint8_t* mask, const float* const* W, int32_t* pidx,
                        void* ws, void* stream, const IdSets* id_sets, int64_t* err) {
    ConvPlan plans[kMaxGroups];
    if (!build_plans(d, plans)) return RBR_ERR_BAD_ARG;
    if (!ids || !W || !pidx) { set_error("null pointer"); return RBR_ERR_BAD_ARG; }
    ProdState S;
    if (int e = prod_state(d, ws, S)) return e;
    hipStream_t st = (hipStream_t)stream;
    int* sched = pidx + (size_t)plans[0].total_wt * plans[0].nslots_total;
    ZeroRegions zr{{reinterpret_cast<int*>(S.base + S.Lo.used), S.sched_p + 2 * (size_t)S.pp[0].total_wt,
                    sched + 2 * (size_t)plans[0].total_wt},
                   {(long)((S.Lo.row_of_token - S.Lo.used) / sizeof(int)), kSchedCounters, kSchedCounters}};
    if (id_sets != nullptr) {
        const long long total = id_sets->first[id_sets->count];
        const int nb_ids = (int)std::min<long long>((total + 255) / 256, 2048);
        const long nz = zr.n[0] + zr.n[1] + zr.n[2];
        const int nb_zero = (int)std::min<long>((nz + 255) / 256, 256);
        hipLaunchKernelGGL(prep_kernel, dim3(nb_ids + nb_zero), dim3(256), 0, st, *id_sets, reinterpret_cast<long long*>(err), zr, nb_ids);
        RBR_CHECK_LAUNCH("textcnn prep launch");
    } else if (int e = zero_regions(zr, st)) {
        return e;
    }
    const long n_tok = (long)d->n_docs * d->L;
    const int nb_scan = (plans[0].total_wt + 255) / 256;
    const int nb_mark = (int)std::min<long>((n_tok + 255) / 256, 2048);
    if (int e_ = rbr::launch<mark_scan_kernel, 256>(dim3(nb_scan + nb_mark), dim3(256), 0, st, "textcnn mark_scan launch", plans[0], nb_scan, n_tok, reinterpret_cast<const long long*>(ids), mask, sched, S.used)) return e_;
    PackJob J{};
    J.P = S.pp[0]; J.n_widths = d->n_widths; J.D = d->D; J.cp_real = S.A.cp_real;
    for (int w = 0; w < d->n_widths; ++w) { J.kz[w] = d->kz[w]; J.ch[w] = d->ch[w]; J.poff[w] = S.A.poff[w]; }
    PtrArray wp{};
    for (int w = 0; w < d->n_widths; ++w) wp.p[w] = W[w];
    const int nb_compact = (d->V + 255) / 256;
    const bool b16 = prod_b16_applicable(d);
    B16Pack JB{};
    if (b16) JB = prod_b16_pack_job(d);
    const long n_pack = (b16 ? (long)JB.ngroups * JB.nchunks * 4 * 64 : (long)S.pp[0].nchunks * S.pp[0].tiles_total * kTile * S.pp[0].DC) +
                        (long)S.A.cp_real * d->D;
    const int nb_pack = (int)std::min<long>((n_pack + 255) / 256, 2048);
    if (int e_ = rbr::launch<compact_pack_kernel, 256>(dim3(nb_compact + nb_pack), dim3(256), 0, st, "textcnn compact_pack launch", J, nb_compact, d->V, S.Lo.cap, S.used, S.row_of_token, S.tok_of_row, S.row_mask, S.counter, prod_t_bf16(d) ? reinterpret_cast<float*>(reinterpret_cast<unsigned short*>(S.T) + (size_t)S.Lo.cap * S.A.pitch)
                                      : S.T + (size_t)S.Lo.cap * S.A.pitch, prod_t_bf16(d) ? S.A.pitch / 2 : S.A.pitch, wp, b16 ? nullptr : S.packed_p, S.WT, JB, b16 ? reinterpret_cast<unsigned char*>(S.base + S.Lo.bimg) : nullptr)) return e_;
    return 0;
}

extern "C" int rbr_textcnn_prod_prepare(const rbr_textcnn_desc* d, const int64_t* ids, const uint8_t* mask,
                                        const float* const* W, int32_t* pidx, void* ws, void* stream) {
    return prod_prepare(d, ids, mask, W, pidx, ws, stream, nullptr, nullptr);
}

extern "C" int rbr_textcnn_prod_prepare_ids(const rbr_textcnn_desc* d, int32_t n_sets, const rbr_id_set* sets, int64_t* err,
                                            const int64_t* ids, const uint8_t* mask, const float* const* W, int32_t* pidx, void* ws,
                                            void* stream) {
    if (!err) { set_error("null err"); return RBR_ERR_BAD_ARG; }
    IdSets S;
    if (int e = fill_id_sets(n_sets, sets, S)) return e;
    const long long n_tok = (long long)d->n_docs * d->L;
    const bool one = sets[0].out == ids && sets[0].n == n_tok;
    const bool two = n_sets >= 2 && sets[0].out == ids && sets[1].out == sets[0].out + sets[0].n && sets[0].n + sets[1].n == n_tok;
    if (!one && !two) { set_error("prod_prepare_ids: `ids` is not the clean copy of the first id set(s)"); return RBR_ERR_BAD_ARG; }
    return prod_prepare(d, ids, mask, W, pidx, ws, stream, &S, err);
}

namespace {
constexpr size_t kListMaxG = (size_t)256 << 20;
bool list_bwd_layout(const rbr_textcnn_desc* d, ProdLayout& Lo, ProdBwdLayout& B, size_t& list_bytes) {
    if (!prod_layout(d, Lo) || !prod_bwd_layout(d, Lo, B)) return false;
    if (B.total > kListMaxG) return false;
    ConvPlan pp[kMaxGroups];
    if (!build_plans(&Lo.dp, pp, kProdGroupTiles)) return false;
    list_bytes = Lo.table_T + align256((size_t)pp[0].nslots_total * sizeof(float));
    return true;
}
}

extern "C" size_t rbr_textcnn_bwd_dtable_list_ws_bytes(const rbr_textcnn_desc* d) {
    ConvPlan plans[kMaxGroups];
    if (!build_plans(d, plans)) return 0;
    static const char* env = getenv("RBR_DTABLE_MODE");
    if (env && !strcmp(env, "scatter")) return 0;
    ProdLayout Lo; ProdBwdLayout B; size_t list_bytes;
    if (!list_bwd_layout(d, Lo, B, list_bytes)) return 0;
    return align256(list_bytes) + B.total;
}

extern "C" int rbr_textcnn_bwd_dtable_list(const rbr_textcnn_desc* d, const int64_t* ids, const uint8_t* mask, const float* const* W,
                                           const float* feat, const int32_t* argmax, const float* d_feat, void* ws, float* dtable,
                                           void* stream) {
    ConvPlan plans[kMaxGroups];
    if (!build_plans(d, plans)) return RBR_ERR_BAD_ARG;
    if (!ids || !W || !feat || !argmax || !d_feat || !ws || !dtable) { set_error("null pointer"); return RBR_ERR_BAD_ARG; }
    ProdLayout Lo; ProdBwdLayout B; size_t list_bytes;
    if (!list_bwd_layout(d, Lo, B, list_bytes)) { set_error("token-list table gradient does not apply to this shape"); return RBR_ERR_UNSUPPORTED; }
    hipStream_t st = (hipStream_t)stream;
    char* base = static_cast<char*>(ws);
    ConvPlan pp[kMaxGroups];
    if (!build_plans(&Lo.dp, pp, kProdGroupTiles)) return RBR_ERR_BAD_ARG;
    int* sched_p = reinterpret_cast<int*>(base + Lo.sched);
    ZeroRegions zr{{reinterpret_cast<int*>(base + Lo.used), sched_p + 2 * (size_t)pp[0].total_wt, nullptr},
                   {(long)((Lo.row_of_token - Lo.used) / sizeof(int)), kSchedCounters, 0}};
    if (int e = zero_regions(zr, st)) return e;
    const long n_tok = (long)d->n_docs * d->L;
    if (int e_ = rbr::launch<mark_scan_kernel, 256>(dim3((unsigned)std::min<long>((n_tok + 255) / 256, 2048)), dim3(256), 0, st, "textcnn mark launch", plans[0], 0, n_tok, reinterpret_cast<const long long*>(ids), mask, (int*)nullptr, reinterpret_cast<unsigned char*>(base + Lo.used))) return e_;
    PackJob J{};
    J.P = pp[0]; J.n_widths = d->n_widths; J.D = d->D;
    int o = 0;
    for (int w = 0; w < d->n_widths; ++w) { J.kz[w] = d->kz[w]; J.ch[w] = d->ch[w]; J.poff[w] = o; o += d->kz[w] * d->ch[w]; }
    J.cp_real = o;
    PtrArray wp{};
    for (int w = 0; w < d->n_widths; ++w) wp.p[w] = W[w];
    const int nb_compact = (d->V + 255) / 256;
    const int nb_pack = (int)std::min<long>(((long)J.cp_real * d->D + 255) / 256, 2048);
    if (int e_ = rbr::launch<compact_pack_kernel, 256>(dim3(nb_compact + nb_pack), dim3(256), 0, st, "textcnn compact launch", J, nb_compact, d->V, Lo.cap, reinterpret_cast<unsigned char*>(base + Lo.used), reinterpret_cast<int*>(base + Lo.row_of_token), reinterpret_cast<long long*>(base + Lo.tok_of_row), reinterpret_cast<unsigned char*>(base + Lo.row_mask), reinterpret_cast<int*>(base + Lo.counter), reinterpret_cast<float*>(base + Lo.table_T), pp[0].nslots_total, wp, (float*)nullptr, reinterpret_cast<float*>(base + Lo.wt), B16Pack{}, (unsigned char*)nullptr)) return e_;
    return dtable_through_list(d, plans, ids, mask, nullptr, feat, argmax, d_feat, base, base + align256(list_bytes), dtable, nullptr, st);
}

extern "C" int rbr_textcnn_prod_table(const rbr_textcnn_desc* d, const float* table, void* ws, void* stream) {
    if (!table) { set_error("null pointer"); return RBR_ERR_BAD_ARG; }
    PairSolo solo;
    ProdState S;
    if (int e = prod_state(d, ws, S)) return e;
    if (prod_b16_applicable(d))
        return prod_b16_gemm(d, S.A.cp_real, S.Lo.cap, S.A.pitch, S.counter, S.tok_of_row, table, S.base + S.Lo.bimg, S.T,
                             S.base + S.Lo.a16, (hipStream_t)stream);
    return run_conv_groups(S.pp, 1, S.tok_of_row, S.row_mask, nullptr, table, S.packed_p, S.T, nullptr, S.sched_p, (hipStream_t)stream);
}

extern "C" int rbr_textcnn_prod_pool(const rbr_textcnn_desc* d, const int64_t* ids, const uint8_t* mask, const float* gate,
                                     float* pval, int32_t* pidx, void* ws, void* stream) {
    ConvPlan plans[kMaxGroups];
    const int ngroups = build_plans(d, plans);
    if (!ngroups) return RBR_ERR_BAD_ARG;
    if (!ids || !pval || !pidx) { set_error("null pointer"); return RBR_ERR_BAD_ARG; }
    PairSolo solo;
    ProdState S;
    if (int e = prod_state(d, ws, S)) return e;
    hipStream_t st = (hipStream_t)stream;
    const int* sched = pidx + (size_t)plans[0].total_wt * plans[0].nslots_total;
    const int max_items = (plans[0].total_wt + kWavesPerWG - 1) / kWavesPerWG;
    if (prod_t_bf16(d))
        { if (int e_ = rbr::launch<gather_pool_kernel<true>, 256>(dim3(max_items), dim3(256), 0, st, "textcnn gather_pool launch", plans[0], S.A, reinterpret_cast<const long long*>(ids), mask, gate, S.row_of_token, static_cast<const void*>(S.T), sched, pval, pidx)) return e_; }
    else
        if (int e_ = rbr::launch<gather_pool_kernel<false>, 256>(dim3(max_items), dim3(256), 0, st, "textcnn gather_pool launch", plans[0], S.A, reinterpret_cast<const long long*>(ids), mask, gate, S.row_of_token, static_cast<const void*>(S.T), sched, pval, pidx)) return e_;
    return 0;
// ... 236 lines not shown
```

review-based-recommender_amd/functional.py:

```python
from __future__ import annotations

import contextlib
import ctypes as C
import os
import weakref
from typing import Optional, Sequence

import torch

from . import _lib
from ._lib import ACT_RELU, ACT_TANH, PAD_SAME, PAD_VALID, TIMER, check, current_stream, dev_ptr, ptr_array

F32, I64, I32, U8 = torch.float32, torch.int64, torch.int32, torch.uint8


def _mask_u8(mask: Optional[torch.Tensor]) -> Optional[torch.Tensor]:
    if mask is None:
        return None
    if mask.dtype == torch.bool:
        return mask.contiguous().view(torch.uint8)
    if mask.dtype == torch.uint8:
        return mask.contiguous()
    raise RuntimeError(f"mask must be bool or uint8, got {mask.dtype}")

# ... 168 lines not shown
            raise RuntimeError(f"{name} must be a contiguous {dtype} tensor of shape {list(shape)}, got {t.dtype} {list(t.shape)}")
    if B == 0:
        return revs, word_masks, rev_masks, rids, ids
    _call(None, _lib.lib().rbr_review_gather, B, R, T, dev_ptr(u_ids, I64, "u_ids"), dev_ptr(i_ids, I64, "i_ids"),
          dev_ptr(user_revs, I32, "user_revs"), dev_ptr(user_rids, I32, "user_rids"), user_revs.shape[0],
          dev_ptr(item_revs, I32, "item_revs"), dev_ptr(item_rids, I32, "item_rids"), item_revs.shape[0],
          int(bool(leave_one_out)), int(pad_token), int(replace_id), dev_ptr(revs, I64, "revs"),
          dev_ptr(word_masks.view(U8), U8, "word_masks"), dev_ptr(None if rev_masks is None else rev_masks.view(U8), U8, "rev_masks"),
          dev_ptr(rids, I64, "rids"), dev_ptr(ids, I64, "ids"), _id_err(dev).data_ptr(), current_stream())
    return revs, word_masks, rev_masks, rids, ids


def set_tap_sink(sink, table: Optional[torch.Tensor] = None) -> None:
    if sink is None:
        if table is None:
            _TAP_SINKS.clear()
        else:
            _TAP_SINKS.pop(table.data_ptr(), None)
        return
    _TAP_SINKS[sink.table.data_ptr()] = sink


def _fanout_acc(table: torch.Tensor):
    node = table.grad_fn
    return getattr(node, "acc", None) if type(node).__name__ == "_TableFanoutBackward" else None


def _table_acc(acc, device):
    if acc is None or acc[1] != torch.cuda.current_stream(device):
        return None
    return acc[0]


class _TableFanout(torch.autograd.Function):

    @staticmethod
    def forward(ctx, table, n):
        ctx.set_materialize_grads(False)
        ctx.acc = (torch.zeros_like(table), torch.cuda.current_stream(table.device))
        return tuple(table.view(table.shape) for _ in range(n))

    @staticmethod
    def backward(ctx, *grads):
        total, seen = None, set()
        for g in grads:
            if g is None or g.data_ptr() in seen:
                continue
            seen.add(g.data_ptr())
            total = g if total is None else total + g
        return total, None


def table_fanout(table: torch.Tensor, n: int):
    if not (torch.is_grad_enabled() and table.requires_grad and table.is_cuda):
        return (table,) * n
    return _TableFanout.apply(table, n)


class _ConvSaved:

    def __init__(self, **kw):
        self.__dict__.update(kw)


def _conv_desc(table, n_docs, L, ws, pad_mode, act, padding_idx, flags: int = 0):
    V, D = table.shape
    return _lib.make_desc(n_docs, L, D, V, [int(w.shape[2]) for w in ws], [int(w.shape[0]) for w in ws], pad_mode, act, padding_idx,
                          flags)


def _conv_operands(table, ids, mask, weights, pad_mode, act, padding_idx, flags: int = 0):
    table_c = table.contiguous()
    dev_ptr(table_c, F32, "word table")
    if ids.dim() != 2:
        raise RuntimeError("ids must be [n_docs, L]")
    ids = ids.contiguous()
    mask8 = _mask_u8(mask)
    if mask8 is not None and mask8.shape != ids.shape:
        raise AssertionError("inputs.shape[:-1] == masks.shape")
    ws = [w.contiguous() for w in weights]
    return table_c, ids, mask8, ws, _conv_desc(table_c, ids.shape[0], ids.shape[1], ws, pad_mode, act, padding_idx, flags)


def _conv_fwd_buffers(rec, desc, dev, feat=None, argmax=None):
    L_ = _lib.lib()
    n_part = L_.rbr_textcnn_partial_elems(C.byref(desc))
    if not n_part:
        check(-1, "rbr_textcnn plan")
    ws_bytes = L_.rbr_textcnn_fwd_ws_bytes(C.byref(desc))
    Ctot = sum(desc.ch[:desc.n_widths])
    rec.pval = torch.empty(n_part, dtype=F32, device=dev)
    rec.pidx = torch.empty(n_part, dtype=I32, device=dev)
    rec.feat = feat if feat is not None else torch.empty(desc.n_docs, Ctot, dtype=F32, device=dev)
    rec.argmax = argmax if argmax is not None else torch.empty(desc.n_docs, Ctot, dtype=I32, device=dev)
    rec.prod_ws = torch.empty(ws_bytes, dtype=torch.uint8, device=dev) if ws_bytes else None
    return rec


def _prod_forward(desc, rec, table, ids, mask8, gate, ws, st, *, id_sets=None, prepare_key="textcnn_prod_prepare"):
    L_ = _lib.lib()
    d, wsp = C.byref(desc), rec.prod_ws.data_ptr()
    ids_p, mask_p, pidx_p = dev_ptr(ids, I64, "ids"), dev_ptr(mask8, U8, "mask"), dev_ptr(rec.pidx, I32, "pidx")
    if id_sets is not None:
        _call(prepare_key, L_.rbr_textcnn_prod_prepare_ids, d, *id_sets, ids_p, mask_p, ptr_array(ws, F32, "conv weight"), pidx_p,
              wsp, st)
    else:
        _call(prepare_key, L_.rbr_textcnn_prod_prepare, d, ids_p, mask_p, ptr_array(ws, F32, "conv weight"), pidx_p, wsp, st)
    _call("textcnn_prod_table", L_.rbr_textcnn_prod_table, d, dev_ptr(table, F32, "word table"), wsp, st)
    _call("textcnn_prod_pool", L_.rbr_textcnn_prod_pool, d, ids_p, mask_p, dev_ptr(gate, F32, "gate"), dev_ptr(rec.pval, F32, "pval"),
          pidx_p, wsp, st)


def _pool_finalize(desc, rec, bs, st):
    _call(None, _lib.lib().rbr_textcnn_pool_finalize, C.byref(desc), dev_ptr(rec.pval, F32, "pval"), dev_ptr(rec.pidx, I32, "pidx"),
          ptr_array(bs, F32, "conv bias"), dev_ptr(rec.feat, F32, "feat"), dev_ptr(rec.argmax, I32, "argmax"), st)


class _TextCNN(torch.autograd.Function):

    @staticmethod
    def forward(ctx, table, gate, ids, mask, kernel_sizes, pad_mode, act, padding_idx, conv_flags, *wb):
        ctx.fanout_acc = _fanout_acc(table)
        n = len(kernel_sizes)
        weights, biases = wb[:n], wb[n:]
        table_c, ids, mask8, ws, desc = _conv_operands(table, ids, mask, weights, pad_mode, act, padding_idx, conv_flags)
        for k, w, b in zip(kernel_sizes, weights, biases):
            assert w.shape[1] == table.shape[1] and w.shape[2] == k and b.shape[0] == w.shape[0]
        bs = [b.contiguous() for b in biases]
        if gate is not None:
            gate = gate.contiguous()
        L_ = _lib.lib()
        dev = table.device
        n_packed = L_.rbr_textcnn_packed_floats(C.byref(desc))
        if not n_packed:
            check(-1, "rbr_textcnn plan")
        buf = _conv_fwd_buffers(_ConvSaved(), desc, dev)
        st = current_stream()
        packed = None
        if buf.prod_ws is not None:
            _prod_forward(desc, buf, table_c, ids, mask8, gate, ws, st)
        else:
            packed = _TextCNN._pack(L_, desc, ws, n_packed, dev, st)
            _call("textcnn_conv_fwd", L_.rbr_textcnn_conv_fwd, C.byref(desc), dev_ptr(ids, I64, "ids"), dev_ptr(mask8, U8, "mask"),
                  dev_ptr(gate, F32, "gate"), dev_ptr(table_c, F32, "word table"), ptr_array(ws, F32, "conv weight"),
                  dev_ptr(packed, F32, "packed"), dev_ptr(buf.pval, F32, "pval"), dev_ptr(buf.pidx, I32, "pidx"), None, st)
        _pool_finalize(desc, buf, bs, st)
        feat, argmax = buf.feat, buf.argmax
        ctx.desc = desc
        ctx.n = n
        ctx.has_gate = gate is not None
        ctx.has_mask = mask8 is not None
        ctx.prod_ws = buf.prod_ws
        ctx.save_for_backward(table_c, ids, packed, feat, argmax, *([mask8] if mask8 is not None else []),
                              *([gate] if gate is not None else []), *ws)
        ctx.mark_non_differentiable(argmax)
        ctx.set_materialize_grads(False)
        return feat, argmax

    @staticmethod
    def _pack(L_, desc, ws, n_packed, dev, st):
        packed = torch.empty(n_packed, dtype=F32, device=dev)
        _call(None, L_.rbr_textcnn_pack, C.byref(desc), ptr_array(ws, F32, "conv weight"), dev_ptr(packed, F32, "packed"), st)
        return packed

    @staticmethod
    def backward(ctx, d_feat, _d_argmax):
        saved = list(ctx.saved_tensors)
        table, ids, packed, feat, argmax = saved[:5]
        k = 5
        mask8 = None
        gate = None
        if ctx.has_mask:
            mask8 = saved[k]; k += 1
        if ctx.has_gate:
            gate = saved[k]; k += 1
        S = _ConvSaved(table=table, ids=ids, packed=packed, feat=feat, argmax=argmax, mask8=mask8, gate=gate, ws=list(saved[k:]),
                       desc=ctx.desc, prod_ws=ctx.prod_ws, fanout_acc=ctx.fanout_acc)
        dtable, dgate, dWs, dbs = _textcnn_backward(S, d_feat, ctx.needs_input_grad[0], ctx.has_gate and ctx.needs_input_grad[1])
        return (dtable, dgate, None, None, None, None, None, None, None, *dWs, *dbs)


class _Fork:

    def __init__(self, dev, on: bool = True):
        self.side = _side_stream(dev) if on else None
        self.done = None
# ... 300 lines not shown

    @staticmethod
    def forward(ctx, u_feat, i_feat, u_id, i_id, drop, pad_u, pad_i, Wu, bu, Eu, Wi, bi, Ei, h, g, ub, ib):
        ctx.stacked = i_feat is None
        if ctx.stacked:
            pair = u_feat.contiguous()
            if pair.shape[0] % 2:
                raise RuntimeError(f"stacked pair features need an even row count, got {tuple(pair.shape)}")
            u_feat, i_feat = pair[:pair.shape[0] // 2], pair[pair.shape[0] // 2:]
        B, H = u_feat.shape
        K = Wu.shape[1]
        dev = u_feat.device
        L_ = _lib.lib()
        u_feat, i_feat = u_feat.contiguous(), i_feat.contiguous()
        u_id, i_id = u_id.contiguous(), i_id.contiguous()
        params = [t.contiguous() for t in (Wu, bu, Eu, Wi, bi, Ei, h, g, ub, ib)]
        hp = _lib.HeadParams(*[dev_ptr(t, F32, n) for t, n in zip(params, ("Wu", "bu", "Eu", "Wi", "bi", "Ei", "h", "g", "ub", "ib"))])
        ul = torch.empty(B, K, dtype=F32, device=dev)
        il = torch.empty(B, K, dtype=F32, device=dev)
        pred = torch.empty(B, dtype=F32, device=dev)
        ctx.flat = None
        if isinstance(drop, float):
            p_drop = drop
            if p_drop >= 1.0:
                raise RuntimeError("pair_head: drop probability must be < 1 on the fused path")
            acc_n = sum(t.numel() for t, n in zip(params, _HEAD_NAMES) if n in _HEAD_ACC) if any(ctx.needs_input_grad[7:]) else 0
            flat = torch.empty(acc_n, dtype=F32, device=dev) if acc_n else None
            seed, state = _drop_rng(dev)
            drop = torch.empty(B, K, dtype=F32, device=dev) if p_drop > 0.0 else None
            _call(None, L_.rbr_pair_head_fwd_train, B, H, K, dev_ptr(u_feat, F32, "u_feat"), dev_ptr(i_feat, F32, "i_feat"),
                  dev_ptr(u_id, I64, "u_id"), dev_ptr(i_id, I64, "i_id"), C.byref(hp), float(p_drop), seed, state.data_ptr(),
                  dev_ptr(drop, F32, "drop"), dev_ptr(flat, F32, "zero_buf"), acc_n, dev_ptr(ul, F32, "ul"), dev_ptr(il, F32, "il"),
                  dev_ptr(pred, F32, "pred"), current_stream())
            ctx.flat = flat
        else:
            if drop is not None:
                drop = drop.contiguous()
            _call(None, L_.rbr_pair_head_fwd, B, H, K, dev_ptr(u_feat, F32, "u_feat"), dev_ptr(i_feat, F32, "i_feat"),
                  dev_ptr(u_id, I64, "u_id"), dev_ptr(i_id, I64, "i_id"), C.byref(hp), dev_ptr(drop, F32, "drop"),
                  dev_ptr(ul, F32, "ul"), dev_ptr(il, F32, "il"), dev_ptr(pred, F32, "pred"), current_stream())
        ctx.dims = (B, H, K, int(pad_u), int(pad_i))
        ctx.has_drop = drop is not None
        ctx.save_for_backward(u_feat, i_feat, u_id, i_id, ul, il, *params, *([drop] if drop is not None else []))
        return pred

    @staticmethod
    def backward(ctx, d_pred):
        B, H, K, pad_u, pad_i = ctx.dims
        saved = list(ctx.saved_tensors)
        u_feat, i_feat, u_id, i_id, ul, il = saved[:6]
        params = saved[6:16]
        drop = saved[16] if ctx.has_drop else None
        dev = u_feat.device
        L_ = _lib.lib()
        names = ("Wu", "bu", "Eu", "Wi", "bi", "Ei", "h", "g", "ub", "ib")
        hp = _lib.HeadParams(*[dev_ptr(t, F32, n) for t, n in zip(params, names)])
        acc = [t for t, n in zip(params, names) if n in _HEAD_ACC]
        flat, ctx.flat = ctx.flat, None
        if flat is None:
            flat = torch.zeros(sum(t.numel() for t in acc), dtype=F32, device=dev)
        zeroed = iter(v.view_as(t) for v, t in zip(flat.split([t.numel() for t in acc]), acc))
        grads = [next(zeroed) if n in ("Eu", "Ei", "ub", "ib") else torch.empty_like(t) for t, n in zip(params, names)]
        hg = _lib.HeadGrads(*[dev_ptr(t, F32, "d" + n) for t, n in zip(grads, names)])
        d_pair = torch.empty(2 * B, H, dtype=F32, device=dev)
        d_uf, d_if = d_pair[:B], d_pair[B:]
        wsn = L_.rbr_pair_head_bwd_ws_floats(B, K)
        ws = torch.empty(wsn, dtype=F32, device=dev) if wsn else None
        d_pred = d_pred.contiguous()
        _call(None, L_.rbr_pair_head_bwd, B, H, K, dev_ptr(u_feat, F32, "u_feat"), dev_ptr(i_feat, F32, "i_feat"),
              dev_ptr(u_id, I64, "u_id"), dev_ptr(i_id, I64, "i_id"), C.byref(hp), dev_ptr(drop, F32, "drop"),
              dev_ptr(ul, F32, "ul"), dev_ptr(il, F32, "il"), dev_ptr(d_pred, F32, "d_pred"), pad_u, pad_i, C.byref(hg),
              dev_ptr(d_uf, F32, "d_ufeat"), dev_ptr(d_if, F32, "d_ifeat"), dev_ptr(ws, F32, "ws"), current_stream())
        if ctx.stacked:
            return (d_pair, None, None, None, None, None, None, *grads)
        return (d_uf, d_if, None, None, None, None, None, *grads)


def pair_head(u_feat, i_feat, u_id, i_id, Wu, bu, Eu, Wi, bi, Ei, h, g, ub, ib, *, drop=None, pad_u=0, pad_i=0):
    return _PairHead.apply(u_feat, i_feat, u_id, i_id, drop, pad_u, pad_i, Wu, bu, Eu, Wi, bi, Ei, h, g, ub, ib)


class _LossRequest:

    def __init__(self, target):
        self.target, self.pred_ptr, self.loss = target, None, None

    def loss_for(self, pred: torch.Tensor):
        if self.loss is not None and self.pred_ptr == pred.data_ptr() and pred.numel() == self.target.numel():
            return self.loss
        return None


_LOSS_REQUEST: list = []


@contextlib.contextmanager
def fused_loss(target: torch.Tensor):
    req = _LossRequest(target)
    _LOSS_REQUEST.append(req)
    try:
        yield req
    finally:
        _LOSS_REQUEST.remove(req)


_TICKETS: dict = {}


def _ticket(dev) -> torch.Tensor:
    idx = dev.index if dev.index is not None else torch.cuda.current_device()
    key = (idx, torch.cuda.current_stream(idx).cuda_stream)
    t = _TICKETS.get(key)
    if t is None:
        t = _TICKETS[key] = torch.zeros(4, dtype=I32, device=dev)
    return t


def prepare_stream_state(dev) -> None:
    dev = torch.device(dev)
    _ticket(dev)
    idx = dev.index if dev.index is not None else torch.cuda.current_device()
    need = max((t.numel() for (d, _), t in _PS_WS.items() if d == idx), default=0)
    if need:
        _pair_softmax_ws(dev, need)


def encode_head_applicable(table, n_docs, L, kernel_sizes, channels, padding_idx) -> bool:
    if not table.is_cuda or table.dtype != F32 or n_docs % 2 or os.environ.get("RBR_FUSED_STEP", "1") == "0":
        return False
    ntiles, wpd = (sum(channels) + 31) // 32, (L + 31) // 32
    if ntiles > 8 or (2 * sum(channels) + 2 * wpd * ntiles * 32 + 2 * wpd) * 4 > 60 * 1024:
        return False
    desc = _lib.make_desc(n_docs, L, table.shape[1], table.shape[0], kernel_sizes, channels, PAD_SAME, ACT_RELU, padding_idx)
    return _lib.lib().rbr_textcnn_fwd_ws_bytes(C.byref(desc)) > 0


class _EncodeHead(torch.autograd.Function):

    @staticmethod
    def forward(ctx, table, id_sets, ids, mask, u_id, i_id, drop, target, padding_idx, pad_u, pad_i, n_widths, first, *params):
        bs_ = [b.contiguous() for b in params[n_widths:2 * n_widths]]
        head = [t.contiguous() for t in params[2 * n_widths:]]
        L_ = _lib.lib()
        dev = table.device
        st = current_stream()
        sets = None
        if id_sets is not None:
            tens = [t.contiguous() for t, _, _ in id_sets]
            flat = torch.empty(sum(t.numel() for t in tens), dtype=I64, device=dev)
            arr = (_lib.IdSet * len(tens))()
            outs, o = [], 0
            for k, (t, (_, rows, rep)) in enumerate(zip(tens, id_sets)):
                dev_ptr(t, I64, "ids")
                v = flat[o:o + t.numel()].view(t.shape)
                outs.append(v)
                o += t.numel()
                arr[k] = _lib.IdSet(t.data_ptr(), v.data_ptr(), t.numel(), int(rows), 0 if rep is None or rep < 0 else int(rep))
            n_tok = tens[0].numel() + tens[1].numel()
            ids = flat[:n_tok].view(2 * tens[0].shape[0], tens[0].shape[1])
            u_id, i_id = outs[2], outs[3]
            sets = (len(tens), arr, _id_err(dev).data_ptr())
        else:
            u_id, i_id = u_id.contiguous(), i_id.contiguous()
        table_c, ids, mask8, ws_, desc = _conv_operands(table, ids, mask, params[:n_widths], PAD_SAME, ACT_RELU, padding_idx)
        B = ids.shape[0] // 2
        conv = _conv_fwd_buffers(_ConvSaved(), desc, dev)
        if conv.prod_ws is None:
            check(-1, "encode_head plan (encode_head_applicable() was not consulted)")
        pval, pidx, feat, argmax = conv.pval, conv.pidx, conv.feat, conv.argmax
        training = any(ctx.needs_input_grad)
        _prod_forward(desc, conv, table_c, ids, mask8, None, ws_, st, id_sets=sets)
        K = head[0].shape[1]
        hp = _lib.HeadParams(*[dev_ptr(t, F32, n) for t, n in zip(head, _HEAD_NAMES)])
        ul = torch.empty(B, K, dtype=F32, device=dev)
        il = torch.empty(B, K, dtype=F32, device=dev)
        pred = torch.empty(B, dtype=F32, device=dev)
        p_drop, drop_t, flat_zero, acc_n = 0.0, None, None, 0
        seed, state = 0, None
        if isinstance(drop, float):
            if drop >= 1.0:
                raise RuntimeError("pair_head: drop probability must be < 1 on the fused path")
            p_drop = drop
            acc_n = sum(t.numel() for t, n in zip(head, _HEAD_NAMES) if n in _HEAD_ACC) if training else 0
            flat_zero = torch.empty(acc_n, dtype=F32, device=dev) if acc_n else None
            if p_drop > 0.0:
                seed, state = _drop_rng(dev)
                drop_t = torch.empty(B, K, dtype=F32, device=dev)
        elif drop is not None:
            drop_t = drop.contiguous()
        loss = d_unit = d_feat_unit = None
        if target is not None:
            target = target.contiguous()
            loss = torch.empty((), dtype=F32, device=dev)
            d_unit = torch.empty(B, dtype=F32, device=dev)
            if training and first is None and os.environ.get("RBR_HEAD_BWD_IN_FWD", "1") != "0" \
                    and L_.rbr_pair_head_fwd_pool_lds_bytes(C.byref(desc), K, 1):
                d_feat_unit = torch.empty(2 * B, feat.shape[1], dtype=F32, device=dev)
        _call("pair_head_fwd_pool", L_.rbr_pair_head_fwd_pool_ex, C.byref(desc), dev_ptr(pval, F32, "pval"), dev_ptr(pidx, I32, "pidx"),
              ptr_array(bs_, F32, "conv bias"), dev_ptr(feat, F32, "feat"), dev_ptr(argmax, I32, "argmax"),
              dev_ptr(first, I64, "first"), K, dev_ptr(u_id, I64, "u_id"), dev_ptr(i_id, I64, "i_id"), C.byref(hp),
              dev_ptr(drop_t, F32, "drop") if p_drop == 0.0 else None, float(p_drop), seed,
              state.data_ptr() if state is not None else None,
              dev_ptr(drop_t, F32, "drop") if p_drop > 0.0 else None, dev_ptr(flat_zero, F32, "zero_buf"),
              acc_n, dev_ptr(ul, F32, "ul"), dev_ptr(il, F32, "il"), dev_ptr(pred, F32, "pred"),
              dev_ptr(target, F32, "target"), dev_ptr(loss, F32, "loss"), dev_ptr(d_unit, F32, "d_unit"),
              _ticket(dev).data_ptr() if target is not None else None, dev_ptr(d_feat_unit, F32, "d_feat_unit"), st)
        ctx.d_feat_unit = d_feat_unit
        ctx.conv = _ConvSaved(table=table_c, ids=ids, packed=None, feat=feat, argmax=argmax, mask8=mask8, gate=None, ws=ws_,
                              desc=desc, prod_ws=conv.prod_ws, fanout_acc=None)
        ctx.head = (u_id, i_id, ul, il, head, drop_t, flat_zero, d_unit)
        ctx.first = first
        ctx.dims = (B, feat.shape[1], K, int(pad_u), int(pad_i), n_widths)
        ctx.set_materialize_grads(False)
        if loss is None:
            loss = torch.empty((), dtype=F32, device=dev)
            ctx.mark_non_differentiable(loss)
        return pred, loss

    @staticmethod
    def backward(ctx, d_pred, d_loss):
        B, H, K, pad_u, pad_i, n_widths = ctx.dims
        u_id, i_id, ul, il, head, drop_t, flat, d_unit = ctx.head
        S = ctx.conv
        dev = S.table.device
        L_ = _lib.lib()
        need_conv = any(ctx.needs_input_grad[13:13 + 2 * n_widths]) or ctx.needs_input_grad[0]
        unit = _UNIT.get(dev)
        early = (ctx.d_feat_unit is not None and need_conv and d_pred is None and ctx.first is None and d_loss is not None
                 and unit is not None and d_loss.data_ptr() == unit.data_ptr())
        if d_loss is not None:
            g = d_unit if (unit is not None and d_loss.data_ptr() == unit.data_ptr()) else d_unit * d_loss
            d_pred = g if d_pred is None else d_pred + g
        if d_pred is None:
            d_pred = torch.zeros(B, dtype=F32, device=dev)
        d_pred = d_pred.contiguous()
        hp = _lib.HeadParams(*[dev_ptr(t, F32, n) for t, n in zip(head, _HEAD_NAMES)])
        accs = [t for t, n in zip(head, _HEAD_NAMES) if n in _HEAD_ACC]
        if flat is None:
            flat = torch.zeros(sum(t.numel() for t in accs), dtype=F32, device=dev)
        ctx.head = (u_id, i_id, ul, il, head, drop_t, None, d_unit)
        zeroed = iter(v.view_as(t) for v, t in zip(flat.split([t.numel() for t in accs]), accs))
        grads = [next(zeroed) if n in _HEAD_ACC else torch.empty_like(t) for t, n in zip(head, _HEAD_NAMES)]
        hg = _lib.HeadGrads(*[dev_ptr(t, F32, "d" + n) for t, n in zip(grads, _HEAD_NAMES)])
        d_pair = ctx.d_feat_unit if early else torch.empty(2 * B, H, dtype=F32, device=dev)
        feat = S.feat

        def head_bwd():
            _call(None, L_.rbr_pair_head_bwd, B, H, K, dev_ptr(feat[:B], F32, "u_feat"), dev_ptr(feat[B:], F32, "i_feat"),
                  dev_ptr(u_id, I64, "u_id"), dev_ptr(i_id, I64, "i_id"), C.byref(hp), dev_ptr(drop_t, F32, "drop"),
                  dev_ptr(ul, F32, "ul"), dev_ptr(il, F32, "il"), dev_ptr(d_pred, F32, "d_pred"), pad_u, pad_i, C.byref(hg),
                  None if early else dev_ptr(d_pair[:B], F32, "d_ufeat"), None if early else dev_ptr(d_pair[B:], F32, "d_ifeat"),
                  None, current_stream())

        if early:
            dtable, _, dWs, dbs = _textcnn_backward(S, d_pair, ctx.needs_input_grad[0], False, side_job=head_bwd)
            return (dtable, None, None, None, None, None, None, None, None, None, None, None, None, *dWs, *dbs, *grads)
        head_bwd()
        if need_conv and ctx.first is not None:
            _call(None, L_.rbr_dedup_fold_rows, 2 * B, H, dev_ptr(ctx.first, I64, "first"), dev_ptr(d_pair, F32, "d_feat"),
                  current_stream())
        if need_conv:
            dtable, _, dWs, dbs = _textcnn_backward(S, d_pair, ctx.needs_input_grad[0], False)
        else:
            dtable, dWs, dbs = None, [None] * n_widths, [None] * n_widths
        return (dtable, None, None, None, None, None, None, None, None, None, None, None, None, *dWs, *dbs, *grads)


def encode_head(table, ids, mask, u_id, i_id, conv_weights, conv_biases, head_params, *, id_sets=None, drop=None,
                padding_idx=0, pad_u=0, pad_i=0, first=None):
    req = _LOSS_REQUEST[-1] if _LOSS_REQUEST else None
    target = None
    if req is not None and req.loss is None and req.target.is_cuda and req.target.dtype == F32 and req.target.dim() == 1 \
            and torch.is_grad_enabled():
        B = (id_sets[0][0].shape[0] if id_sets is not None else ids.shape[0] // 2)
        if req.target.shape[0] == B:
            target = req.target
    pred, loss = _EncodeHead.apply(table, id_sets, ids, mask, u_id, i_id, drop, target, padding_idx, pad_u, pad_i,
                                   len(conv_weights), first, *conv_weights, *conv_biases, *head_params)
    if target is not None:
        req.pred_ptr, req.loss = pred.data_ptr(), loss
    return pred


def stack_rows(a: torch.Tensor, b: torch.Tensor) -> torch.Tensor:
    if (a.dtype == b.dtype and a.shape[1:] == b.shape[1:] and a.is_contiguous() and b.is_contiguous()
            and not a.requires_grad and not b.requires_grad and a.device == b.device
            and a.untyped_storage().data_ptr() == b.untyped_storage().data_ptr()
            and b.storage_offset() == a.storage_offset() + a.numel()):
        return a.as_strided((a.shape[0] + b.shape[0], *a.shape[1:]), a.stride(), a.storage_offset())
    return torch.cat([a, b], dim=0)


def clone_adjacent(tensors):
    out = list(tensors)
    k = 0
    while k < len(out):
        a = out[k]
        b = out[k + 1] if k + 1 < len(out) else None
        if b is not None and a.shape == b.shape and a.dtype == b.dtype and a.device == b.device and a.dim() >= 1:
            both = torch.empty((2 * a.shape[0], *a.shape[1:]), dtype=a.dtype, device=a.device)
            both[:a.shape[0]].copy_(a)
            both[a.shape[0]:].copy_(b)
            out[k], out[k + 1] = both[:a.shape[0]], both[a.shape[0]:]
            k += 2
        else:
            out[k] = a.clone()
            k += 1
    return tuple(out)


def dropout_multiplier(shape, p: float, training: bool, device, lane: int = 0) -> Optional[torch.Tensor]:
    if not training or p <= 0.0:
        return None
    if p >= 1.0:
        return torch.zeros(shape, dtype=F32, device=device)
    dev = torch.device(device)
    seed, state = _drop_rng(dev, lane)
    out = torch.empty(shape, dtype=F32, device=dev)
    _call(None, _lib.lib().rbr_dropout_multiplier, out.numel(), float(p), seed, state.data_ptr(), dev_ptr(out, F32, "out"),
          current_stream())
    return out


def _drop_rng(dev, lane: int = 0):
    dev = torch.device(dev)
    if dev.type != "cuda":
        raise RuntimeError(f"dropout: device must be a HIP device (got {dev}); there is no CPU path")
    idx = dev.index if dev.index is not None else torch.cuda.current_device()
    state = _DROP_STATE.get((idx, lane))
    if state is None:
        state = _DROP_STATE[(idx, lane)] = torch.zeros(2, dtype=torch.int64, device=dev)
    seed = (torch.cuda.default_generators[idx].initial_seed() + 0x9E3779B97F4A7C15 * lane) & 0xFFFFFFFFFFFFFFFF
    return seed, state


_DROP_STATE: dict = {}



class _MseLoss(torch.autograd.Function):

    @staticmethod
    def forward(ctx, pred, target):
        pred, target = pred.contiguous(), target.contiguous()
        if pred.shape != target.shape:
            raise RuntimeError(f"mse_loss: pred {tuple(pred.shape)} vs target {tuple(target.shape)}")
        loss = torch.empty((), dtype=F32, device=pred.device)
        d_unit = torch.empty_like(pred) if ctx.needs_input_grad[0] else None
        _call(None, _lib.lib().rbr_mse_loss_fwd, pred.numel(), dev_ptr(pred, F32, "pred"), dev_ptr(target, F32, "target"),
              dev_ptr(loss, F32, "loss"), dev_ptr(d_unit, F32, "d_pred_unit"), current_stream())
        ctx.save_for_backward(pred, target, *([d_unit] if d_unit is not None else []))
        return loss

    @staticmethod
    def backward(ctx, d_loss):
        pred, target = ctx.saved_tensors[:2]
        unit = _UNIT.get(pred.device)
        if unit is not None and len(ctx.saved_tensors) == 3 and d_loss.data_ptr() == unit.data_ptr():
            return ctx.saved_tensors[2], None
        d_pred = torch.empty_like(pred)
        d_loss = d_loss.contiguous()
# ... 1051 lines not shown
```

review-based-recommender_amd/models/deepconn/deepconn.py:

```python
import torch
import torch.nn as nn

from ... import functional as RF
from .layers import FM, LastFeat, NgramFeat, WordEmbedding, latent_rows, rating_head


class DeepCoNNpp(nn.Module):
    def __init__(self, user_size, item_size, vocab_size, kernel_sizes, embedding_dim, hidden_dim, latent_dim, doc_len,
                 pretrained_embeddings, dropout, arch="CNN"):
        super().__init__()
        self.user_size = user_size
        self.item_size = item_size
        self.vocab_size = vocab_size
        self.hidden_dim = hidden_dim

        self.word_embeddings = WordEmbedding(vocab_size, embedding_dim, pretrained_embeddings=pretrained_embeddings)
        self.ngram = NgramFeat(kernel_sizes, embedding_dim, hidden_dim, doc_len, arch=arch)
        self.user_feat = LastFeat(user_size, hidden_dim, latent_dim, padding_idx=0)
        self.item_feat = LastFeat(item_size, hidden_dim, latent_dim, padding_idx=0)
        self.fm = FM(user_size, item_size, latent_dim, dropout, user_padding_idx=0, item_padding_idx=0)
        self.dedup_by_id = False
        self.validate_ids = True

    def _fused_ok(self, u_revs, i_revs) -> bool:
        if self.ngram.arch != "CNN" or u_revs.shape != i_revs.shape or u_revs.dim() != 2:
            return False
        conv = self.ngram.feature_layer[0]
        return RF.encode_head_applicable(self.word_embeddings.weight, 2 * u_revs.shape[0], u_revs.shape[1], conv.kernel_sizes,
                                         [conv.out_features_per_kz] * len(conv.kernel_sizes), self.word_embeddings.padding_idx)

    def forward(self, u_revs, i_revs, u_rev_masks, i_rev_masks, u_ids, i_ids):
        bz = u_revs.shape[0]
        stacked = None
        if self._fused_ok(u_revs, i_revs):
            pad = self.word_embeddings.padding_idx
            conv = self.ngram.feature_layer[0]
            uf, itf, fm = self.user_feat, self.item_feat, self.fm
            training = fm.training and torch.is_grad_enabled()
            if training and fm.dropout.p < 1.0:
                drop = float(fm.dropout.p)
            else:
                drop = RF.dropout_multiplier((bz, fm.h.shape[0]), fm.dropout.p, fm.training, u_revs.device)
            head = (uf.W, uf.b, uf.ebd.weight, itf.W, itf.b, itf.ebd.weight, fm.h, fm.g_bias, fm.user_bias.weight, fm.item_bias.weight)
            masks = RF.stack_rows(u_rev_masks, i_rev_masks)
            first = None
            if self.dedup_by_id:
                first, masks = RF.dedup_rows(u_ids, i_ids, self.user_size, self.item_size, masks, u_revs.shape[1])
            if self.validate_ids:
                sets = [(u_revs, self.vocab_size, pad), (i_revs, self.vocab_size, pad), (u_ids, self.user_size, 0),
                        (i_ids, self.item_size, 0)]
                preds = RF.encode_head(self.word_embeddings.weight, None, masks, None, None, conv.weights(), conv.biases(), head,
                                       id_sets=sets, drop=drop, padding_idx=pad, pad_u=fm.user_padding_idx, pad_i=fm.item_padding_idx,
                                       first=first)
            else:
                preds = RF.encode_head(self.word_embeddings.weight, RF.stack_rows(u_revs, i_revs), masks, u_ids, i_ids,
                                       conv.weights(), conv.biases(), head, drop=drop, padding_idx=pad,
                                       pad_u=fm.user_padding_idx, pad_i=fm.item_padding_idx, first=first)
            return preds.view(bz)
        if self.validate_ids:
            pad = self.word_embeddings.padding_idx
            stacked, u_ids, i_ids = RF.sanitize_ids([(u_revs, self.vocab_size, pad), (i_revs, self.vocab_size, pad),
                                                     (u_ids, self.user_size, 0), (i_ids, self.item_size, 0)], stack_first_two=True)
            u_revs, i_revs = stacked[:bz], stacked[bz:]
        if self.dedup_by_id:
            ids = stacked if stacked is not None else RF.stack_rows(u_revs, i_revs)
            first, masks = RF.dedup_rows(u_ids, i_ids, self.user_size, self.item_size,
                                         RF.stack_rows(u_rev_masks, i_rev_masks), ids.shape[1])
            feats = self.ngram.encode(self.word_embeddings.weight, ids, masks, padding_idx=self.word_embeddings.padding_idx)
            u_rev_feats, i_rev_feats = feats.index_select(0, first), None
        else:
            ids = stacked if stacked is not None else RF.stack_rows(u_revs, i_revs)
            masks = RF.stack_rows(u_rev_masks, i_rev_masks)
            feats = self.ngram.encode(self.word_embeddings.weight, ids, masks, padding_idx=self.word_embeddings.padding_idx)
            u_rev_feats, i_rev_feats = feats, None
        preds = rating_head(self.user_feat, self.item_feat, self.fm, u_rev_feats, i_rev_feats, u_ids, i_ids)
        return preds.view(bz)

    def pair_latents(self, u_revs, i_revs, u_rev_masks, i_rev_masks, u_ids, i_ids):
        pad = self.word_embeddings.padding_idx
        if self.validate_ids:
            ids, u_ids, i_ids = RF.sanitize_ids([(u_revs, self.vocab_size, pad), (i_revs, self.vocab_size, pad),
                                                 (u_ids, self.user_size, 0), (i_ids, self.item_size, 0)], stack_first_two=True)
        else:
            ids = RF.stack_rows(u_revs, i_revs)
        masks = RF.stack_rows(u_rev_masks, i_rev_masks)
        feats = self.ngram.encode(self.word_embeddings.weight, ids, masks, padding_idx=pad)
        return latent_rows(self.user_feat, self.item_feat, feats, u_ids, i_ids)

    def _encode_side(self, docs, masks, ids, last):
        with RF.eval_mode(self):
            pad = self.word_embeddings.padding_idx
            if self.validate_ids:
                (docs,) = RF.sanitize_ids([(docs, self.vocab_size, pad)])
            feats = self.ngram.encode(self.word_embeddings.weight, docs.contiguous(), masks.contiguous(), padding_idx=pad)
            return last(feats, ids)

    def encode_users(self, u_revs, u_rev_masks, u_ids):
        return self._encode_side(u_revs, u_rev_masks, u_ids, self.user_feat)

    def encode_items(self, i_revs, i_rev_masks, i_ids):
        return self._encode_side(i_revs, i_rev_masks, i_ids, self.item_feat)

    def _explain_side(self, docs, masks, d_latent, last):
        if self.ngram.arch != "CNN":
            raise ValueError("explain_users / explain_items cover DeepCoNN++ and NARRE with arch='CNN' (the TextCNN's max-pool "
                             f"routing is what they read); arch={self.ngram.arch!r} is not covered")
        with RF.eval_mode(self):
            pad = self.word_embeddings.padding_idx
            if self.validate_ids:
                (docs,) = RF.sanitize_ids([(docs, self.vocab_size, pad)])
            conv, table = self.ngram.feature_layer[0], self.word_embeddings.weight
            docs, masks = docs.contiguous(), masks.contiguous()
            feat, argmax = RF.textcnn(table, docs, masks, conv.weights(), conv.biases(), padding_idx=pad, return_argmax=True)
            g = RF.linear(d_latent, last.W)
            tokens = RF.textcnn_saliency(table, docs, masks, conv.weights(), feat, argmax, g)
            return tokens, (g * feat).sum(1)

    def explain_users(self, u_revs, u_rev_masks, u_ids, d_latent):
        return self._explain_side(u_revs, u_rev_masks, d_latent, self.user_feat)

    def explain_items(self, i_revs, i_rev_masks, i_ids, d_latent):
        return self._explain_side(i_revs, i_rev_masks, d_latent, self.item_feat)

    def score_mode_and_params(self):
        fm = self.fm
        return "fm", fm.h, fm.g_bias, fm.user_bias.weight, fm.item_bias.weight
```

review-based-recommender_amd/train_step.py:

```python
from __future__ import annotations

import contextlib
import os

import torch
import torch.nn as nn
import torch.nn.functional as F

from . import functional as RF

LR = 2e-3
MAX_GRAD_NORM = 5.0


def make_optimizer(model: nn.Module, lr: float = LR, fused: bool | None = None,
                   capturable: bool = False, hip_clip_adam: bool = False) -> torch.optim.Optimizer:
    params = list(model.parameters())
    if hip_clip_adam:
        return HipClipAdam(params, lr=lr)
    if fused is None:
        fused = len(params) > 0 and all(p.is_cuda for p in params)
    if fused:
        return torch.optim.Adam(params, lr=lr, fused=True, capturable=capturable)
    return torch.optim.Adam(params, lr=lr, capturable=capturable)
# ... 117 lines not shown
            for ps in by_counter.values():
                for k in range(0, len(ps), self.MAX_TENSORS):
                    batches.append((g, ps[k:k + self.MAX_TENSORS]))
        if self._row_grads and (len(batches) > 1 or len(self._row_grads) > 1):
            self.materialize_grads()
        if len(batches) > 1 and max_grad_norm is not None:
            gn = nn.utils.clip_grad_norm_([p for _, p in todo], max_grad_norm)
            self._gnorm.copy_(gn)
            max_grad_norm = None
        elif len(batches) > 1:
            self._gnorm.copy_(torch.linalg.vector_norm(torch.stack(torch._foreach_norm([p.grad for _, p in todo]))))
        for g, ps in batches:
            step = self._shared_counter(ps)
            states = [self.state[p] for p in ps]
            grads = [p.grad for p in ps]
            for p, gr in zip(ps, grads):
                if not (p.is_contiguous() and (gr is None or gr.is_contiguous())):
                    raise RuntimeError("HipClipAdam needs contiguous parameters and gradients")
            numel = (C.c_int64 * len(ps))(*[p.numel() for p in ps])
            b1, b2 = g["betas"]
            ev = _lib.TIMER.record("clip_adam_step")
            args = (len(ps), _lib.ptr_array(ps, torch.float32, "param"), _lib.ptr_array(grads, torch.float32, "grad"),
                    _lib.ptr_array([s_["exp_avg"] for s_ in states], torch.float32, "exp_avg"),
                    _lib.ptr_array([s_["exp_avg_sq"] for s_ in states], torch.float32, "exp_avg_sq"),
                    numel, float(max_grad_norm) if max_grad_norm is not None else 0.0,
                    float(g["lr"]), float(b1), float(b2), float(g["eps"]), _lib.dev_ptr(step, torch.float32, "step"),
                    _lib.dev_ptr(self._gnorm, torch.float32, "gnorm") if len(batches) == 1 else None,
                    _lib.dev_ptr(self._ws, torch.float32, "ws"))
            rowp = [k for k, p in enumerate(ps) if p in self._row_grads]
            if rowp:
                rg = self._row_grads[ps[rowp[0]]]
                if rg.coef is None:
                    rg.coef = torch.empty((), dtype=torch.float32, device=dev)
                crg = _lib.RowGrad(rowp[0], rg.V, rg.D, rg.row_of_token_ptr, rg.rows.data_ptr(), rg.sq.data_ptr(), rg.sq.numel(),
                                   rg.coef.data_ptr())
                _lib.check(L_.rbr_clip_adam_step_rows(*args, C.byref(crg), st), "rbr_clip_adam_step_rows")
            else:
                _lib.check(L_.rbr_clip_adam_step(*args, st), "rbr_clip_adam_step")
            if ev is not None:
                ev.record()
        return self._gnorm

    @torch.no_grad()
    def step(self, closure=None):
        loss = None
        if closure is not None:
            with torch.enable_grad():
                loss = closure()
        self.clip_and_step(None)
        return loss

    def load_state_dict(self, state_dict):
        super().load_state_dict(state_dict)
        for g in self.param_groups:
            shared = {}
            for p in g["params"]:
                st = self.state.get(p)
                if st and "step" in st:
                    key = (float(st["step"]), st["exp_avg"].device)
                    if key not in shared:
                        shared[key] = torch.as_tensor(key[0], dtype=torch.float32, device=key[1])
                    st["step"] = shared[key]


def train_step(model: nn.Module, optimizer: torch.optim.Optimizer, batch, ratings: torch.Tensor,
               max_grad_norm: float = MAX_GRAD_NORM, grad_sync=None, objective=None):
    optimizer.zero_grad()
    if objective is None:
        pred, loss = _forward_loss_backward(model, batch, ratings, optimizer if grad_sync is None else None)
    else:
        pred, loss = _forward_objective_backward(model, batch, objective, optimizer if grad_sync is None else None)
    if grad_sync is not None:
        if isinstance(optimizer, HipClipAdam):
            optimizer.materialize_grads()
        grad_sync(model)
    gnorm = clip_and_step(model, optimizer, max_grad_norm)
    return loss.detach(), gnorm, pred.detach()


def _forward_loss_backward(model: nn.Module, batch, ratings: torch.Tensor, optimizer=None):
    scope = optimizer.row_grad_scope() if isinstance(optimizer, HipClipAdam) else contextlib.nullcontext()
    fusable = ratings.is_cuda and ratings.dtype == torch.float32
    with scope:
        with (RF.fused_loss(ratings) if fusable else contextlib.nullcontext()) as req:
            out = model(*batch)
            pred = out[0] if isinstance(out, tuple) else out
            loss = req.loss_for(pred) if req is not None else None
        if loss is not None:
            loss.backward(RF.unit_scalar(pred.device))
            return pred, loss
        return pred, _loss_and_backward(pred, ratings)


def _forward_objective_backward(model: nn.Module, batch, objective, optimizer=None):
    scope = optimizer.row_grad_scope() if isinstance(optimizer, HipClipAdam) else contextlib.nullcontext()
    with scope:
        if hasattr(objective, "forward_loss"):
            pred, loss = objective.forward_loss(model, batch)
        else:
            out = model(*batch)
            pred = out[0] if isinstance(out, tuple) else out
            loss = objective(pred)
        loss.backward(RF.unit_scalar(pred.device) if pred.is_cuda else None)
    return pred, loss


class BprObjective:

    def __init__(self, feed):
        self.feed = feed

    def __call__(self, pred: torch.Tensor) -> torch.Tensor:
        n_neg = self.feed.n_neg
        if pred.dim() != 1 or pred.shape[0] % (1 + n_neg):
            raise RuntimeError(f"BprObjective: pred {tuple(pred.shape)} is not (1 + {n_neg}) * B scores")
        return RF.bpr_loss(pred, n_neg, self.feed.buffers(pred.shape[0] // (1 + n_neg))[2])


class InBatchSoftmaxObjective:

    def __init__(self, model, feed, temperature: float = 1.0, logq=None):
        for name in ("pair_latents", "score_mode_and_params"):
            if not hasattr(model, name):
                raise ValueError(f"InBatchSoftmaxObjective needs a two-tower model with {name}(); {type(model).__name__} has none")
        if not hasattr(feed, "seen") or not hasattr(feed, "item_lo") or not hasattr(feed, "_last"):
            raise ValueError("InBatchSoftmaxObjective takes a data.InBatchFeed (the batch's ids, the seen CSR, item_lo)")
        temperature = float(temperature)
        if not (temperature > 0.0 and temperature < float("inf")):
            raise ValueError(f"temperature must be positive and finite, got {temperature}")
        self.feed, self.temperature = feed, temperature
        self.logq = None if logq is None else logq.detach().to(torch.float32).contiguous().view(-1, 1)

    def forward_loss(self, model, batch):
        feed = self.feed
        if feed._last is None:
            raise RuntimeError("InBatchSoftmaxObjective: the feed has gathered no batch yet (feed.inputs / feed.gather come first)")
        u_ids, i_ids = feed.u_ids, feed.i_ids
        ul, il = model.pair_latents(*batch)
        if ul.shape[0] != u_ids.shape[0]:
            raise RuntimeError(f"InBatchSoftmaxObjective: the batch has {ul.shape[0]} pairs, the feed's last gather {u_ids.shape[0]}")
        mode, h, g, ub, ib = model.score_mode_and_params()
        row_bias = col_bias = logq = None
        p_drop = 0.0
        u_idx, i_idx = u_ids, i_ids
        if getattr(model, "validate_ids", True) and (ub is not None or ib is not None or self.logq is not None):
            u_idx, i_idx = RF.sanitize_ids([(u_ids, ub.shape[0] if ub is not None else (1 << 62), 0),
                                            (i_ids, ib.shape[0] if ib is not None else self.logq.shape[0], 0)])
        if mode == "fm":
            fm = model.fm
            if fm.training and torch.is_grad_enabled():
                p_drop = float(fm.dropout.p)
            if ub is not None:
                row_bias = RF.embedding(ub, u_idx, fm.user_padding_idx).view(-1) + g
                col_bias = RF.embedding(ib, i_idx, fm.item_padding_idx).view(-1)
            else:
                row_bias = g.expand(ul.shape[0])
        if self.logq is not None:
            logq = RF.embedding(self.logq, i_idx, None).view(-1)
        drop = None
        if p_drop >= 1.0:
            drop, p_drop = torch.zeros(ul.shape[0], ul.shape[0], ul.shape[1], dtype=torch.float32, device=ul.device), 0.0
        loss, pos = RF.pair_softmax_loss(ul, il, u_ids, i_ids, mode, h=h, row_bias=row_bias, col_bias=col_bias, drop=drop,
                                         seen=feed.seen, item_lo=feed.item_lo, logq=logq, temperature=self.temperature, p_drop=p_drop)
        return pos, loss


def _loss_and_backward(pred: torch.Tensor, ratings: torch.Tensor) -> torch.Tensor:
# ... 2 lines not shown
        loss.backward(RF.unit_scalar(pred.device))
    else:
        loss = F.mse_loss(pred, ratings)
        loss.backward()
    return loss


def clip_and_step(model: nn.Module, optimizer: torch.optim.Optimizer, max_grad_norm: float) -> torch.Tensor:
    if isinstance(optimizer, HipClipAdam):
        return optimizer.clip_and_step(max_grad_norm)
    gnorm = nn.utils.clip_grad_norm_(model.parameters(), max_grad_norm)
    optimizer.step()
    return gnorm


def _flat_layout(tensors, align: int = 256):
    offs, o, k = [], 0, 0
    while k < len(tensors):
        a = tensors[k]
        b = tensors[k + 1] if k + 1 < len(tensors) else None
        o = (o + align - 1) // align * align
        offs.append(o)
        o += a.numel() * a.element_size()
        if b is not None and a.shape == b.shape and a.dtype == b.dtype and a.dim() >= 1:
            offs.append(o)
            o += b.numel() * b.element_size()
            k += 2
        else:
            k += 1
    offs.append((o + align - 1) // align * align)
    return offs


def _flat_views(flat: torch.Tensor, layout, like):
    return [flat[o:o + t.numel() * t.element_size()].view(t.dtype).view(t.shape) for o, t in zip(layout, like)]


def _lib_mod():
    from . import _lib
    return _lib


def _capture_stream(dev) -> torch.cuda.Stream:
    cs = torch.cuda.Stream(device=dev)
    with torch.cuda.stream(cs):
        RF.prepare_stream_state(dev)
    torch.cuda.synchronize(dev)
    return cs


class GraphedForward:

    def __init__(self, model: nn.Module, batch, warmup: int = 2, capture_error_mode: str = "global", feed=None,
                 with_ids: bool = True):
        batch = list(batch)
        if not batch or not batch[0].is_cuda:
            raise RuntimeError("GraphedForward needs HIP tensors")
        self.model = model
        self._feed, self._with_ids = feed, with_ids
        self.ids = None
        if feed is not None:
            self._id_layout = _flat_layout(batch)
            self._id_flat = torch.empty(self._id_layout[-1], dtype=torch.uint8, device=batch[0].device)
            self.ids = tuple(_flat_views(self._id_flat, self._id_layout, batch))
            for v, src in zip(self.ids, batch):
                v.copy_(src)
            batch = list(feed.empty_inputs(batch[0].shape[0], with_ids))
        self._layout = _flat_layout(batch)
        self._flat = torch.empty(self._layout[-1], dtype=torch.uint8, device=batch[0].device)
        views = _flat_views(self._flat, self._layout, batch)
        for v, src in zip(views, batch):
            v.copy_(src)
        self.batch = tuple(views)
        side = torch.cuda.Stream()
        side.wait_stream(torch.cuda.current_stream())
        with torch.cuda.stream(side), torch.no_grad():
            for _ in range(warmup):
                self._prologue()
                model(*self.batch)
        torch.cuda.current_stream().wait_stream(side)
        torch.cuda.synchronize()
        self.graph = torch.cuda.CUDAGraph()
        self._capture_stream = _capture_stream(batch[0].device)
        with torch.no_grad(), _lib_mod().capture_guard(self._capture_stream), \
                torch.cuda.graph(self.graph, stream=self._capture_stream, capture_error_mode=capture_error_mode):
            self._prologue()
            out = model(*self.batch)
        self.pred = out[0] if isinstance(out, tuple) else out

    @classmethod
    def from_ids(cls, model: nn.Module, cache, u_ids: torch.Tensor, i_ids: torch.Tensor, with_ids: bool = True, **kw):
        return cls(model, (u_ids, i_ids), feed=cache, with_ids=with_ids, **kw)

    def _prologue(self):
        if self._feed is not None:
            self._feed.gather(self.ids[0], self.ids[1], out=self.batch)

    def _inputs(self):
        return (self.ids, self._id_flat, self._id_layout) if self._feed is not None else (self.batch, self._flat, self._layout)

    def matches(self, batch) -> bool:
        ref = self._inputs()[0]
        return len(batch) == len(ref) and all(a.shape == b.shape and a.dtype == b.dtype for a, b in zip(batch, ref))

    def pack(self, batch) -> torch.Tensor:
        _, flat, layout = self._inputs()
        blob = torch.empty_like(flat)
        for v, src in zip(_flat_views(blob, layout, list(batch)), batch):
            v.copy_(src)
        return blob

    def __call__(self, batch=None, packed: torch.Tensor | None = None) -> torch.Tensor:
        dsts, flat, _ = self._inputs()
        if packed is not None:
            if packed.shape != flat.shape or packed.dtype != torch.uint8:
                raise RuntimeError("packed batch does not match the forward's input layout (use GraphedForward.pack)")
            flat.copy_(packed, non_blocking=True)
        if batch is not None:
            if not self.matches(batch):
                raise RuntimeError("batch shapes differ from the recorded forward's (run ragged batches eagerly)")
            for dst, src in zip(dsts, batch):
                if dst is not src:
                    dst.copy_(src, non_blocking=True)
        self.graph.replay()
        return self.pred


def _count_kernel_nodes(graph: torch.cuda.CUDAGraph) -> int:
    import ctypes as C
    hip = C.CDLL("libamdhip64.so")
    g = C.c_void_p(graph.raw_cuda_graph())
    n = C.c_size_t(0)
    if hip.hipGraphGetNodes(g, None, C.byref(n)) != 0:
        raise RuntimeError("hipGraphGetNodes failed")
    nodes = (C.c_void_p * max(1, n.value))()
    if hip.hipGraphGetNodes(g, nodes, C.byref(n)) != 0:
        raise RuntimeError("hipGraphGetNodes failed")
    kernels = 0
    for k in range(n.value):
        ty = C.c_int(-1)
        if hip.hipGraphNodeGetType(C.c_void_p(nodes[k]), C.byref(ty)) != 0:
            raise RuntimeError("hipGraphNodeGetType failed")
        kernels += int(ty.value == 0)
    return kernels


class _StepSlot:
    __slots__ = ("flat", "batch", "ratings", "ids", "id_flat", "g_fwd_bwd", "g_update", "static_grads", "loss", "gnorm", "pred")


class GraphedTrainStep:

    def __init__(self, model: nn.Module, optimizer: torch.optim.Optimizer, batch, ratings: torch.Tensor,
                 max_grad_norm: float = MAX_GRAD_NORM, grad_sync=None, warmup: int = 3, capture_error_mode: str | None = None,
                 slots: int = 1, keep_graph: bool = False, feed=None, with_ids: bool = True, objective=None):
        if not ratings.is_cuda:
            raise RuntimeError("GraphedTrainStep needs HIP tensors")
        if slots < 1:
            raise ValueError("slots must be >= 1")
        if objective is not None and grad_sync is not None:
            raise ValueError("a recorded step with an objective is not available with grad_sync (data-parallel training keeps "
                             "the MSE step)")
        self.objective = objective
        self.model, self.optimizer, self.grad_sync, self.max_grad_norm = model, optimizer, grad_sync, max_grad_norm
        self._keep_graph = bool(keep_graph)
        self._feed, self._with_ids = feed, with_ids
        id_block = None
        if feed is not None:
            id_block = list(batch) + [ratings]
            self._id_layout = _flat_layout(id_block)
            inputs = list(feed.empty_inputs(batch[0].shape[0], with_ids))
        else:
            inputs = list(batch) + [ratings]
        self._layout = _flat_layout(inputs)
        self._slots = []
        for _ in range(slots):
            sl = _StepSlot()
            sl.flat = torch.empty(self._layout[-1], dtype=torch.uint8, device=ratings.device)
            views = _flat_views(sl.flat, self._layout, inputs)
            for v, src in zip(views, inputs):
                v.copy_(src)
            if id_block is None:
                sl.batch, sl.ratings = tuple(views[:-1]), views[-1]
                sl.ids = sl.id_flat = None
            else:
                sl.batch = tuple(views)
                sl.id_flat = torch.empty(self._id_layout[-1], dtype=torch.uint8, device=ratings.device)
                idv = _flat_views(sl.id_flat, self._id_layout, id_block)
                for v, src in zip(idv, id_block):
                    v.copy_(src)
                sl.ids, sl.ratings = tuple(idv[:-1]), idv[-1]
            sl.g_update = sl.static_grads = None
            self._slots.append(sl)
        first = self._slots[0]
        saved_params = [p.detach().clone() for p in model.parameters()]
        saved_state = {p: {k: v.clone() for k, v in optimizer.state[p].items() if torch.is_tensor(v)}
                       for group in optimizer.param_groups for p in group["params"] if p in optimizer.state}
        side = torch.cuda.Stream()
        side.wait_stream(torch.cuda.current_stream())
        with torch.cuda.stream(side):
            for _ in range(warmup):
                self._prologue(first)
                train_step(model, optimizer, first.batch, first.ratings, max_grad_norm, grad_sync, objective)
        torch.cuda.current_stream().wait_stream(side)
        torch.cuda.synchronize()
        mode = capture_error_mode or ("thread_local" if grad_sync is not None else "global")
        self._capture_stream = _capture_stream(ratings.device)
        cs = self._capture_stream
        for sl in self._slots:
            optimizer.zero_grad(set_to_none=True)
            sl.g_fwd_bwd = torch.cuda.CUDAGraph(keep_graph=True) if self._keep_graph else torch.cuda.CUDAGraph()
            if grad_sync is None:
                with _lib_mod().capture_guard(cs), torch.cuda.graph(sl.g_fwd_bwd, stream=cs, capture_error_mode=mode):
                    self._prologue(sl)
                    sl.loss, sl.gnorm, sl.pred = train_step(model, optimizer, sl.batch, sl.ratings, max_grad_norm,
                                                            objective=objective)
                sl.static_grads = [(p, p.grad) for p in model.parameters()]
            else:
                with _lib_mod().capture_guard(cs), torch.cuda.graph(sl.g_fwd_bwd, stream=cs, capture_error_mode=mode):
                    self._prologue(sl)
                    optimizer.zero_grad()
                    pred, loss = _forward_loss_backward(model, sl.batch, sl.ratings)
                    sl.loss, sl.pred = loss.detach(), pred.detach()
                    if isinstance(optimizer, HipClipAdam):
                        optimizer.materialize_grads()
                grad_sync(model)
                sl.static_grads = [(p, p.grad) for p in model.parameters()]
                sl.g_update = torch.cuda.CUDAGraph(keep_graph=True) if self._keep_graph else torch.cuda.CUDAGraph()
                with _lib_mod().capture_guard(cs), torch.cuda.graph(sl.g_update, pool=sl.g_fwd_bwd.pool(), stream=cs, capture_error_mode=mode):
                    sl.gnorm = clip_and_step(model, optimizer, max_grad_norm)
        with torch.no_grad():
            for p, v in zip(model.parameters(), saved_params):
                p.copy_(v)
            for group in optimizer.param_groups:
                for p in group["params"]:
                    for k, v in optimizer.state.get(p, {}).items():
                        if torch.is_tensor(v):
                            old = saved_state.get(p, {}).get(k)
                            v.copy_(old) if old is not None else v.zero_()
        if self._slots[-1].static_grads is not None:
            for p, g in first.static_grads:
                p.grad = g

    @classmethod
    def from_ids(cls, model: nn.Module, optimizer: torch.optim.Optimizer, cache, u_ids: torch.Tensor, i_ids: torch.Tensor,
                 ratings: torch.Tensor, max_grad_norm: float = MAX_GRAD_NORM, grad_sync=None, with_ids: bool = True, **kw):
        return cls(model, optimizer, (u_ids, i_ids), ratings, max_grad_norm, grad_sync, feed=cache, with_ids=with_ids, **kw)

    def _prologue(self, sl) -> None:
        if self._feed is not None:
            self._feed.gather(sl.ids[0], sl.ids[1], out=sl.batch)

    batch = property(lambda self: self._slots[0].batch)
    ratings = property(lambda self: self._slots[0].ratings)
    loss = property(lambda self: self._slots[0].loss)
    gnorm = property(lambda self: self._slots[0].gnorm)
    pred = property(lambda self: self._slots[0].pred)
    g_fwd_bwd = property(lambda self: self._slots[0].g_fwd_bwd)
    g_update = property(lambda self: self._slots[0].g_update)
    _flat = property(lambda self: self._slots[0].flat)

    @property
    def slots(self) -> int:
        return len(self._slots)

    def kernel_launches(self, slot: int = 0):
        sl = self._slots[slot]
        try:
            return sum(_count_kernel_nodes(g) for g in (sl.g_fwd_bwd, sl.g_update) if g is not None)
        except Exception:
            return None

    def slot_inputs(self, slot: int = 0):
        sl = self._slots[slot]
        if self._feed is not None:
            return sl.ids, sl.ratings, sl.id_flat
        return sl.batch, sl.ratings, sl.flat

    def slot_batch(self, slot: int = 0):
        return self._slots[slot].batch

    def pack(self, batch, ratings: torch.Tensor) -> torch.Tensor:
        flat, layout = (self._slots[0].id_flat, self._id_layout) if self._feed is not None else (self._slots[0].flat, self._layout)
        blob = torch.empty_like(flat)
        for v, src in zip(_flat_views(blob, layout, list(batch) + [ratings]), list(batch) + [ratings]):
            v.copy_(src)
        return blob

    def stage(self, slot: int, batch=None, ratings: torch.Tensor | None = None, packed: torch.Tensor | None = None) -> None:
        sl = self._slots[slot]
        if self._feed is not None:
            return self._stage_ids(sl, batch, ratings, packed)
        if packed is not None:
            if packed.shape != sl.flat.shape or packed.dtype != torch.uint8:
                raise RuntimeError("packed batch does not match the step's input layout (use GraphedTrainStep.pack)")
            sl.flat.copy_(packed, non_blocking=True)
        if batch is not None:
            for dst, src in zip(sl.batch, batch):
                if dst is not src:
                    dst.copy_(src, non_blocking=True)
        if ratings is not None and ratings is not sl.ratings:
            sl.ratings.copy_(ratings, non_blocking=True)
# ... 36 lines not shown
```

Before: 756,700 pairs/s.

## Defer MSE loss into head backward and keep per-graph prod workspace state

Adds a loss-deferred path: the forward pool no longer needs a ticketed last-block MSE reduction, and the head backward kernel gets an extra block that computes the loss and d_pred from pred and target inline. It also adds a 'kept' prod-prepare variant that fuses the tile scan, used-word marking and id sanitization into one kernel with persistent per-graph workspace owned by the captured graphs. The aim is to remove serialized ticket work and extra launches from the train step. In exchange it widens the autograd arg list, adds state-lifetime handling across graph slots, and adds a synchronize per slot during capture.

Measured after the change: 771,100 pairs/s (median of 6 runs). 1.02x the previous value.

```diff
diff --git a/include/rbr_hip.h b/include/rbr_hip.h
--- a/include/rbr_hip.h
+++ b/include/rbr_hip.h
@@ -75,6 +75,10 @@
 int rbr_textcnn_prod_prepare_ids(const rbr_textcnn_desc* d, int32_t n_sets, const struct rbr_id_set* sets, int64_t* err,
                                  const int64_t* ids, const uint8_t* mask, const float* const* W, int32_t* pidx, void* ws,
                                  void* stream);
+int rbr_textcnn_prod_prepare_ids_kept(const rbr_textcnn_desc* d, int32_t n_sets, const struct rbr_id_set* sets, int64_t* err,
+                                      const int64_t* ids, const uint8_t* mask, const float* const* W, int32_t* pidx, void* ws,
+                                      void* stream);
+int rbr_textcnn_prod_list_state(const rbr_textcnn_desc* d, int64_t off[6]);
 
 int rbr_textcnn_pool_finalize(const rbr_textcnn_desc* d, const float* pval, const int32_t* pidx,
                               const float* const* bias, float* feat, int32_t* argmax, void* stream);
@@ -167,6 +171,11 @@
                       const int64_t* u_id, const int64_t* i_id, const rbr_head_params* p, const float* drop,
                       const float* ul, const float* il, const float* d_pred, int32_t pad_u, int32_t pad_i,
                       const rbr_head_grads* g, float* d_ufeat, float* d_ifeat, float* ws, void* stream);
+int rbr_pair_head_bwd_ex(int32_t B, int32_t H, int32_t K, const float* u_feat, const float* i_feat,
+                         const int64_t* u_id, const int64_t* i_id, const rbr_head_params* p, const float* drop,
+                         const float* ul, const float* il, const float* d_pred, int32_t pad_u, int32_t pad_i,
+                         const rbr_head_grads* g, float* d_ufeat, float* d_ifeat, const float* pred, const float* target,
+                         float* loss, float* d_pred_unit, void* stream);
 int rbr_dropout_multiplier(int64_t n, float p, uint64_t seed, uint64_t* state, float* out, void* stream);
 
 int rbr_mse_loss_fwd(int64_t n, const float* pred, const float* target, float* loss, float* d_pred_unit, void* stream);
diff --git a/review-based-recommender_amd/_lib.py b/review-based-recommender_amd/_lib.py
--- a/review-based-recommender_amd/_lib.py
+++ b/review-based-recommender_amd/_lib.py
@@ -106,6 +106,9 @@
     "rbr_textcnn_token_list": (C.c_int, [_DESC, C.c_void_p, _PP, _PP, _PP, C.POINTER(i32)]),
     "rbr_textcnn_prod_prepare_ids": (C.c_int, [_DESC, i32, C.POINTER(IdSet), C.c_void_p, c_i64p, c_u8p, _PP, c_i32p, C.c_void_p,
                                                c_stream]),
+    "rbr_textcnn_prod_prepare_ids_kept": (C.c_int, [_DESC, i32, C.POINTER(IdSet), C.c_void_p, c_i64p, c_u8p, _PP, c_i32p, C.c_void_p,
+                                                    c_stream]),
+    "rbr_textcnn_prod_list_state": (C.c_int, [_DESC, C.POINTER(C.c_int64)]),
     "rbr_dedup_fold_rows": (C.c_int, [i32, i32, c_i64p, c_f32p, c_stream]),
     "rbr_pair_head_fwd_pool": (C.c_int, [_DESC, c_f32p, c_i32p, _PP, c_f32p, c_i32p, c_i64p, i32, c_i64p, c_i64p, C.POINTER(HeadParams),
                                          c_f32p, C.c_float, C.c_uint64, C.c_void_p, c_f32p, c_f32p, C.c_int64, c_f32p, c_f32p,
@@ -155,6 +158,9 @@
     "rbr_pair_head_bwd": (C.c_int, [i32, i32, i32, c_f32p, c_f32p, c_i64p, c_i64p, C.POINTER(HeadParams), c_f32p,
                                     c_f32p, c_f32p, c_f32p, i32, i32, C.POINTER(HeadGrads), c_f32p, c_f32p, c_f32p,
                                     c_stream]),
+    "rbr_pair_head_bwd_ex": (C.c_int, [i32, i32, i32, c_f32p, c_f32p, c_i64p, c_i64p, C.POINTER(HeadParams), c_f32p,
+                                       c_f32p, c_f32p, c_f32p, i32, i32, C.POINTER(HeadGrads), c_f32p, c_f32p, c_f32p, c_f32p,
+                                       c_f32p, c_f32p, c_stream]),
     "rbr_dropout_multiplier": (C.c_int, [C.c_int64, C.c_float, C.c_uint64, C.c_void_p, c_f32p, c_stream]),
     "rbr_mse_loss_fwd": (C.c_int, [C.c_int64, c_f32p, c_f32p, c_f32p, c_f32p, c_stream]),
     "rbr_pair_dot_fwd": (C.c_int, [i32, i32, c_f32p, c_f32p, c_stream]),
diff --git a/review-based-recommender_amd/csrc/pair_head.hip b/review-based-recommender_amd/csrc/pair_head.hip
--- a/review-based-recommender_amd/csrc/pair_head.hip
+++ b/review-based-recommender_amd/csrc/pair_head.hip
@@ -248,6 +248,7 @@
         head_pair_dfeat(P.C, K, s_bwd, s_bwd + K4, s_bwd + 2 * K4, s_dp, p, s_bwd, s_bwd + K4, d_feat_unit + (long)b * P.C,
                         d_feat_unit + (long)(B + b) * P.C);
     }
+    if (mse.ticket == nullptr) return;
     if (t == 0) {
         __threadfence();
         s_last = atomicAdd(mse.ticket, 1) == B - 1;
@@ -271,13 +272,20 @@
     }
 }
 
+struct HeadLoss {
+    const float* pred;
+    const float* target;
+    float* loss;
+    float* d_unit;
+};
+template <bool FROM_PRED>
 __global__ __launch_bounds__(256) void head_bwd_kernel(int B, int H, int K, const float* __restrict__ uf,
                                                        const float* __restrict__ itf, const long long* __restrict__ uid,
                                                        const long long* __restrict__ iid, const rbr_head_params p,
                                                        const float* __restrict__ drop, const float* __restrict__ ul,
                                                        const float* __restrict__ il, const float* __restrict__ d_pred,
                                                        int pad_u, int pad_i, const rbr_head_grads g,
-                                                       float* __restrict__ d_uf, float* __restrict__ d_if) {
+                                                       float* __restrict__ d_uf, float* __restrict__ d_if, const HeadLoss lj) {
     extern __shared__ __attribute__((aligned(16))) float sm[];
     const int t = threadIdx.x;
     if ((int)blockIdx.x < B) {
@@ -286,7 +294,7 @@
         float* s_dul = sm;
         float* s_dil = sm + K4;
         const long u = uid[b], it = iid[b];
-        const float dp = d_pred[b];
+        const float dp = FROM_PRED ? __fmul_rn(lj.pred[b] - lj.target[b], 2.f / (float)B) : d_pred[b];
         head_pair_dfeat(H, K, ul + (long)b * K, il + (long)b * K, drop != nullptr ? drop + (long)b * K : nullptr, dp, p, s_dul, s_dil,
                         d_uf != nullptr ? d_uf + (long)b * H : nullptr, d_uf != nullptr ? d_if + (long)b * H : nullptr);
         for (int k = t; k < K; k += 256) {
@@ -302,6 +310,19 @@
     float (*red)[8][32] = reinterpret_cast<float (*)[8][32]>(sm);
     const int rows = H + 1;
     const int rb = blockIdx.x - B;
+    if (FROM_PRED && rb == 2 * rows) {
+        float acc = 0.f;
+        for (int i = t; i < B; i += 256) {
+            const float d = lj.pred[i] - lj.target[i];
+            acc += d * d;
+            if (lj.d_unit != nullptr) lj.d_unit[i] = d * (2.f / (float)B);
+        }
+        acc = wave_sum(acc);
+        if ((t & 63) == 0) sm[t >> 6] = acc;
+        __syncthreads();
+        if (t == 0) *lj.loss = (sm[0] + sm[1] + sm[2] + sm[3]) / (float)B;
+        return;
+    }
     const int side = rb / rows, r = rb % rows;
     const int kk = t & 31, grp = t >> 5;
     const float* ft = side ? itf : uf;
@@ -311,7 +332,8 @@
         if (k < K) {
             const float hk = p.h[k];
             for (int b0 = grp; b0 < B; b0 += 64) {
-                float vu[8], vi[8], vd[8], vp[8], vf[8];
+                float vu[8], vi[8], vd[8], vp[8], vf[8], vt[8];
+                const float* pp = FROM_PRED ? lj.pred : d_pred;
 #pragma unroll
                 for (int u = 0; u < 8; ++u) {
                     const int b = b0 + 8 * u;
@@ -320,8 +342,13 @@
                     vu[u] = ul[bb * K + k];
                     vi[u] = il[bb * K + k];
                     vd[u] = (drop != nullptr) ? drop[bb * K + k] : 1.f;
-                    vp[u] = ok ? d_pred[bb] : 0.f;
+                    vp[u] = ok ? pp[bb] : 0.f;
+                    vt[u] = (FROM_PRED && ok) ? lj.target[bb] : 0.f;
                     vf[u] = (r < H) ? ft[bb * H + r] : 0.f;
+                }
+                if (FROM_PRED) {
+#pragma unroll
+                    for (int u = 0; u < 8; ++u) vp[u] = __fmul_rn(vp[u] - vt[u], 2.f / (float)B);
                 }
 #pragma unroll
                 for (int u = 0; u < 8; ++u) {
@@ -543,7 +570,8 @@
     if (!(p_drop >= 0.f && p_drop < 1.f)) { set_error("pair_head_fwd_pool: p_drop=%f outside [0,1)", (double)p_drop); return RBR_ERR_BAD_ARG; }
     if (p_drop > 0.f && (!rng_state || !drop_out)) { set_error("pair_head_fwd_pool: dropout needs rng_state and drop_out"); return RBR_ERR_BAD_ARG; }
     if (zero_n < 0 || (zero_n > 0 && !zero_buf)) { set_error("pair_head_fwd_pool: bad zero buffer"); return RBR_ERR_BAD_ARG; }
-    if (target != nullptr && (!loss || !ticket)) { set_error("pair_head_fwd_pool: the loss needs loss and ticket"); return RBR_ERR_BAD_ARG; }
+    if (target != nullptr && ticket == nullptr && d_feat_unit == nullptr) { set_error("pair_head_fwd_pool: the loss needs loss and ticket"); return RBR_ERR_BAD_ARG; }
+    if (target != nullptr && ticket != nullptr && !loss) { set_error("pair_head_fwd_pool: the loss needs loss and ticket"); return RBR_ERR_BAD_ARG; }
     if (d_feat_unit != nullptr && !target) { set_error("pair_head_fwd_pool: d_feat_unit needs the loss target"); return RBR_ERR_BAD_ARG; }
     HeadTrain tr{};
     tr.p_drop = p_drop; tr.seed = seed;
@@ -574,22 +602,50 @@
 
 extern "C" size_t rbr_pair_head_bwd_ws_floats(int32_t B, int32_t K) { (void)B; (void)K; return 0; }
 
+static int head_bwd_launch(int32_t B, int32_t H, int32_t K, const float* u_feat, const float* i_feat, const int64_t* u_id,
+                           const int64_t* i_id, const rbr_head_params* p, const float* drop, const float* ul, const float* il,
+                           const float* d_pred, int32_t pad_u, int32_t pad_i, const rbr_head_grads* g, float* d_ufeat, float* d_ifeat,
+                           const HeadLoss& lj, void* stream) {
+    if (!head_args_ok(B, H, K)) return RBR_ERR_BAD_ARG;
+    if (!u_feat || !i_feat || !u_id || !i_id || !p || !ul || !il || !g || (!d_ufeat != !d_ifeat)) {
+        set_error("null pointer");
+        return RBR_ERR_BAD_ARG;
+    }
+    if (d_pred == nullptr && (!lj.pred || !lj.target || !lj.loss)) {
+        set_error("pair_head_bwd: without d_pred the loss role needs pred, target and loss");
+        return RBR_ERR_BAD_ARG;
+    }
+    const bool loss_role = d_pred == nullptr;
+    const size_t lds = std::max((size_t)2 * ((K + 3) & ~3), (size_t)3 * 8 * 32) * sizeof(float);
+    if (loss_role)
+        hipLaunchKernelGGL(head_bwd_kernel<true>, dim3((unsigned)(B + 2 * (H + 1) + 1)), dim3(256), lds, (hipStream_t)stream,
+                           B, H, K, u_feat, i_feat, reinterpret_cast<const long long*>(u_id), reinterpret_cast<const long long*>(i_id), *p,
+                           drop, ul, il, d_pred, pad_u, pad_i, *g, d_ufeat, d_ifeat, lj);
+    else
+        hipLaunchKernelGGL(head_bwd_kernel<false>, dim3((unsigned)(B + 2 * (H + 1))), dim3(256), lds, (hipStream_t)stream,
+                           B, H, K, u_feat, i_feat, reinterpret_cast<const long long*>(u_id), reinterpret_cast<const long long*>(i_id), *p,
+                           drop, ul, il, d_pred, pad_u, pad_i, *g, d_ufeat, d_ifeat, HeadLoss{});
+    RBR_CHECK_LAUNCH("pair_head_bwd launch");
+    return 0;
+}
+
 extern "C" int rbr_pair_head_bwd(int32_t B, int32_t H, int32_t K, const float* u_feat, const float* i_feat,
                                  const int64_t* u_id, const int64_t* i_id, const rbr_head_params* p, const float* drop,
                                  const float* ul, const float* il, const float* d_pred, int32_t pad_u, int32_t pad_i,
                                  const rbr_head_grads* g, float* d_ufeat, float* d_ifeat, float* ws, void* stream) {
-    if (!head_args_ok(B, H, K)) return RBR_ERR_BAD_ARG;
-    if (!u_feat || !i_feat || !u_id || !i_id || !p || !ul || !il || !d_pred || !g || (!d_ufeat != !d_ifeat)) {
-        set_error("null pointer");
-        return RBR_ERR_BAD_ARG;
-    }
+    if (!d_pred) { set_error("null pointer"); return RBR_ERR_BAD_ARG; }
     (void)ws;
-    const size_t lds = std::max((size_t)2 * ((K + 3) & ~3), (size_t)3 * 8 * 32) * sizeof(float);
-    hipLaunchKernelGGL(head_bwd_kernel, dim3((unsigned)(B + 2 * (H + 1))), dim3(256), lds, (hipStream_t)stream, B, H, K, u_feat,
-                       i_feat, reinterpret_cast<const long long*>(u_id), reinterpret_cast<const long long*>(i_id), *p, drop,
-                       ul, il, d_pred, pad_u, pad_i, *g, d_ufeat, d_ifeat);
-    RBR_CHECK_LAUNCH("pair_head_bwd launch");
-    return 0;
+    return head_bwd_launch(B, H, K, u_feat, i_feat, u_id, i_id, p, drop, ul, il, d_pred, pad_u, pad_i, g, d_ufeat, d_ifeat, HeadLoss{},
+                           stream);
+}
+
+extern "C" int rbr_pair_head_bwd_ex(int32_t B, int32_t H, int32_t K, const float* u_feat, const float* i_feat,
+                                    const int64_t* u_id, const int64_t* i_id, const rbr_head_params* p, const float* drop,
+                                    const float* ul, const float* il, const float* d_pred, int32_t pad_u, int32_t pad_i,
+                                    const rbr_head_grads* g, float* d_ufeat, float* d_ifeat, const float* pred, const float* target,
+                                    float* loss, float* d_pred_unit, void* stream) {
+    return head_bwd_launch(B, H, K, u_feat, i_feat, u_id, i_id, p, drop, ul, il, d_pred, pad_u, pad_i, g, d_ufeat, d_ifeat,
+                           HeadLoss{pred, target, loss, d_pred_unit}, stream);
 }
 
 namespace rbr {
diff --git a/review-based-recommender_amd/csrc/rbr_common.h b/review-based-recommender_amd/csrc/rbr_common.h
--- a/review-based-recommender_amd/csrc/rbr_common.h
+++ b/review-based-recommender_amd/csrc/rbr_common.h
@@ -111,7 +111,7 @@
     int count;
 };
 int fill_id_sets(int n_sets, const rbr_id_set* sets, IdSets& S);
-__device__ __forceinline__ void sanitize_id(const IdSets& S, long long k, long long* __restrict__ err) {
+__device__ __forceinline__ long long sanitize_id(const IdSets& S, long long k, long long* __restrict__ err) {
     int s = 0;
 #pragma unroll
     for (int q = 1; q < RBR_MAX_ID_SETS; ++q)
@@ -125,12 +125,14 @@
         v = S.replace[s];
     }
     S.out[s][e] = v;
+    return v;
 }
 
 constexpr int kSlabDup = 2;
 constexpr int kPadRunHalo = 8;
 __device__ __forceinline__ void tile_scan_block(const ConvPlan& P, const unsigned char* __restrict__ mask,
-                                                int* __restrict__ sched, int blk, const long long* __restrict__ ids = nullptr) {
+                                                int* __restrict__ sched, int blk, const long long* __restrict__ ids = nullptr,
+                                                int* __restrict__ count = nullptr) {
     const int wt = blk * 256 + threadIdx.x;
     int act = 0;
     if (wt < P.total_wt) {
@@ -195,7 +197,7 @@
     act = act == 1;
     const int lane = threadIdx.x & 63;
     int base = 0;
-    if (lane == 0 && b) base = atomicAdd(sched + 2 * (long)P.total_wt, __popcll(b));
+    if (lane == 0 && b) base = atomicAdd(count != nullptr ? count : sched + 2 * (long)P.total_wt, __popcll(b));
     base = __shfl(base, 0);
     if (act) sched[(long)P.total_wt + base + __popcll(b & ((1ull << lane) - 1))] = wt;
 }
diff --git a/review-based-recommender_amd/csrc/textcnn_prod.hip b/review-based-recommender_amd/csrc/textcnn_prod.hip
--- a/review-based-recommender_amd/csrc/textcnn_prod.hip
+++ b/review-based-recommender_amd/csrc/textcnn_prod.hip
@@ -44,6 +44,38 @@
     }
 }
 
+constexpr int kKeptTicket = 62;
+constexpr int kKeptSlabs = 63;
+struct KeptState {
+    int* ticket;
+    int* slabs;
+    int* doc_counters;
+    int* gemm_counters;
+    int used_words;
+    int mask_bytes;
+};
+
+__global__ __launch_bounds__(256) void mark_scan_ids_kernel(const ConvPlan P, int nb_scan, int nb_mark, long n_tok, const IdSets S,
+                                                            long long* __restrict__ err, const unsigned char* __restrict__ mask,
+                                                            int* __restrict__ sched, int* __restrict__ slabs,
+                                                            unsigned char* __restrict__ used, int V) {
+    if ((int)blockIdx.x < nb_scan) {
+        tile_scan_block(P, mask, sched, blockIdx.x, nullptr, slabs);
+        return;
+    }
+    if ((int)blockIdx.x < nb_scan + nb_mark) {
+        for (long k = (long)(blockIdx.x - nb_scan) * 256 + threadIdx.x; k < n_tok; k += (long)nb_mark * 256) {
+            const long long v = sanitize_id(S, k, err);
+            if ((mask == nullptr || mask[k]) && (unsigned long long)v < (unsigned long long)V) used[v] = 1;
+        }
+        return;
+    }
+    const long long total = S.first[S.count];
+    const long nb = gridDim.x - nb_scan - nb_mark;
+    for (long long k = n_tok + (long long)(blockIdx.x - nb_scan - nb_mark) * 256 + threadIdx.x; k < total; k += (long long)nb * 256)
+        sanitize_id(S, k, err);
+}
+
 struct PackJob {
     ConvPlan P;
     int n_widths, D, cp_real;
@@ -60,44 +92,8 @@
     return W.p[w][((long)cl * J.D + d) * J.kz[w] + j];
 }
 
-__device__ __forceinline__ void compact_pack_kernel(const PackJob& J, int nb_compact, int V, int cap,
-                                                           const unsigned char* __restrict__ used, int* __restrict__ row_of_token,
-                                                           long long* __restrict__ tok_of_row, unsigned char* __restrict__ row_mask,
-                                                           int* __restrict__ counter, float* __restrict__ zero_row, int pitch,
-                                                           const PtrArray& W, float* __restrict__ packed, float* __restrict__ WT,
-                                                           const B16Pack& JB, unsigned char* __restrict__ bimg) {
-    if ((int)blockIdx.x < nb_compact) {
-        if (blockIdx.x == 0)
-            for (int k = threadIdx.x; k < pitch; k += 256) zero_row[k] = 0.f;
-        __shared__ int s_cnt[4], s_wave[4];
-        const int lane = threadIdx.x & 63, wave = threadIdx.x >> 6;
-        const int below = blockIdx.x * 256;
-        int c = 0;
-        const int4* u4 = reinterpret_cast<const int4*>(used);
-        for (int q = threadIdx.x; q < below / 16; q += 256) {
-            const int4 m = u4[q];
-            c += __popc(m.x) + __popc(m.y) + __popc(m.z) + __popc(m.w);
-        }
-        c = wave_sum(c);
-        const int v = below + threadIdx.x;
-        const int u = (v < V) ? used[v] : 0;
-        const unsigned long long b = __ballot(u);
-        if (lane == 0) { s_cnt[wave] = c; s_wave[wave] = __popcll(b); }
-        __syncthreads();
-        int base = (s_cnt[0] + s_cnt[1]) + (s_cnt[2] + s_cnt[3]);
-        for (int k = 0; k < wave; ++k) base += s_wave[k];
-        if (v < V) {
-            int row = -1;
-            if (u) {
-                row = base + __popcll(b & ((1ull << lane) - 1));
-                if (row < cap) { tok_of_row[row] = v; row_mask[row] = 1; } else row = -1;
-            }
-            row_of_token[v] = row;
-        }
-        if ((int)blockIdx.x == nb_compact - 1 && threadIdx.x == 0)
-            *counter = (s_cnt[0] + s_cnt[1]) + (s_cnt[2] + s_cnt[3]) + s_wave[0] + s_wave[1] + s_wave[2] + s_wave[3];
-        return;
-    }
+__device__ __forceinline__ void pack_blocks(const PackJob& J, int nb_compact, const PtrArray& W, float* __restrict__ packed,
+                                            float* __restrict__ WT, const B16Pack& JB, unsigned char* __restrict__ bimg) {
     const long nb = gridDim.x - nb_compact, b0 = blockIdx.x - nb_compact;
     const ConvPlan& P = J.P;
     const int DC = P.DC;
@@ -122,6 +118,111 @@
             WT[e] = prod_weight(J, W, pc, d);
         }
     }
+}
+
+__device__ __forceinline__ void compact_pack_kernel(const PackJob& J, int nb_compact, int V, int cap,
+                                                           const unsigned char* __restrict__ used, int* __restrict__ row_of_token,
+                                                           long long* __restrict__ tok_of_row, unsigned char* __restrict__ row_mask,
+                                                           int* __restrict__ counter, float* __restrict__ zero_row, int pitch,
+                                                           const PtrArray& W, float* __restrict__ packed, float* __restrict__ WT,
+                                                           const B16Pack& JB, unsigned char* __restrict__ bimg) {
+    if ((int)blockIdx.x < nb_compact) {
+        if (blockIdx.x == 0)
+            for (int k = threadIdx.x; k < pitch; k += 256) zero_row[k] = 0.f;
+        __shared__ int s_cnt[4], s_wave[4];
+        const int lane = threadIdx.x & 63, wave = threadIdx.x >> 6;
+        const int below = blockIdx.x * 256;
+        int c = 0;
+        const int4* u4 = reinterpret_cast<const int4*>(used);
+        for (int q = threadIdx.x; q < below / 16; q += 256) {
+            const int4 m = u4[q];
+            c += __popc(m.x) + __popc(m.y) + __popc(m.z) + __popc(m.w);
+        }
+        c = wave_sum(c);
+        const int v = below + threadIdx.x;
+        const int u = (v < V) ? used[v] : 0;
+        const unsigned long long b = __ballot(u);
+        if (lane == 0) { s_cnt[wave] = c; s_wave[wave] = __popcll(b); }
+        __syncthreads();
+        int base = (s_cnt[0] + s_cnt[1]) + (s_cnt[2] + s_cnt[3]);
+        for (int k = 0; k < wave; ++k) base += s_wave[k];
+        if (v < V) {
+            int row = -1;
+            if (u) {
+                row = base + __popcll(b & ((1ull << lane) - 1));
+                if (row < cap) { tok_of_row[row] = v; row_mask[row] = 1; } else row = -1;
+            }
+            row_of_token[v] = row;
+        }
+        if ((int)blockIdx.x == nb_compact - 1 && threadIdx.x == 0)
+            *counter = (s_cnt[0] + s_cnt[1]) + (s_cnt[2] + s_cnt[3]) + s_wave[0] + s_wave[1] + s_wave[2] + s_wave[3];
+        return;
+    }
+    pack_blocks(J, nb_compact, W, packed, WT, JB, bimg);
+}
+
+__device__ __forceinline__ void compact_kept_block(int nb_compact, int V, int cap, unsigned char* used, int* __restrict__ row_of_token,
+                                                   long long* __restrict__ tok_of_row, unsigned char* __restrict__ row_mask,
+                                                   int* __restrict__ counter, float* __restrict__ zero_row, int pitch,
+                                                   const KeptState& KS) {
+    if (blockIdx.x == 0)
+        for (int k = threadIdx.x; k < pitch; k += 256) zero_row[k] = 0.f;
+    __shared__ int s_cnt[4], s_all[4], s_wave[4], s_last;
+    const int lane = threadIdx.x & 63, wave = threadIdx.x >> 6;
+    const int below = blockIdx.x * 256;
+    int c = 0, call = 0;
+    const int4* u4 = reinterpret_cast<const int4*>(used);
+    for (int q = threadIdx.x; q < KS.used_words; q += 256) {
+        const int4 m = u4[q];
+        const int n = __popc(m.x) + __popc(m.y) + __popc(m.z) + __popc(m.w);
+        call += n;
+        if (q < below / 16) c += n;
+    }
+    c = wave_sum(c);
+    call = wave_sum(call);
+    const int v = below + threadIdx.x;
+    const int u = (v < V) ? used[v] : 0;
+    const unsigned long long b = __ballot(u);
+    if (lane == 0) { s_cnt[wave] = c; s_all[wave] = call; s_wave[wave] = __popcll(b); }
+    __syncthreads();
+    if (threadIdx.x == 0) s_last = atomicAdd(KS.ticket, 1) == nb_compact - 1;
+    int base = (s_cnt[0] + s_cnt[1]) + (s_cnt[2] + s_cnt[3]);
+    for (int k = 0; k < wave; ++k) base += s_wave[k];
+    const int total = (s_all[0] + s_all[1]) + (s_all[2] + s_all[3]);
+    if (v < V) {
+        int row = -1;
+        if (u) {
+            row = base + __popcll(b & ((1ull << lane) - 1));
+            if (row < cap) tok_of_row[row] = v; else row = -1;
+        }
+        row_of_token[v] = row;
+    }
+    if (v < KS.mask_bytes) row_mask[v] = v < min(total, cap) ? 1 : 0;
+    if ((int)blockIdx.x == nb_compact - 1 && threadIdx.x == 0) *counter = total;
+    if (blockIdx.x == 0) {
+        if (threadIdx.x == 0) { KS.doc_counters[0] = *KS.slabs; *KS.slabs = 0; }
+        else if (threadIdx.x < kSchedCounters) KS.doc_counters[threadIdx.x] = 0;
+        if (threadIdx.x >= 1 && threadIdx.x < kKeptTicket) KS.gemm_counters[threadIdx.x] = 0;
+    }
+    __syncthreads();
+    if (s_last) {
+        int4* w4 = reinterpret_cast<int4*>(used);
+        for (int q = threadIdx.x; q < KS.used_words; q += 256) w4[q] = make_int4(0, 0, 0, 0);
+        if (threadIdx.x == 0) *KS.ticket = 0;
+    }
+}
+
+__global__ __launch_bounds__(256) void compact_pack_kept_kernel(const PackJob J, int nb_compact, int V, int cap, unsigned char* used,
+                                                                int* __restrict__ row_of_token, long long* __restrict__ tok_of_row,
+                                                                unsigned char* __restrict__ row_mask, int* __restrict__ counter,
+                                                                float* __restrict__ zero_row, int pitch, const PtrArray W,
+                                                                float* __restrict__ packed, float* __restrict__ WT, const B16Pack JB,
+                                                                unsigned char* __restrict__ bimg, const KeptState KS) {
+    if ((int)blockIdx.x < nb_compact) {
+        compact_kept_block(nb_compact, V, cap, used, row_of_token, tok_of_row, row_mask, counter, zero_row, pitch, KS);
+        return;
+    }
+    pack_blocks(J, nb_compact, W, packed, WT, JB, bimg);
 }
 
 typedef float f32x4 __attribute__((ext_vector_type(4)));
@@ -1262,7 +1363,7 @@
 }
 
 static int prod_prepare(const rbr_textcnn_desc* d, const int64_t* ids, const uint8_t* mask, const float* const* W, int32_t* pidx,
-                        void* ws, void* stream, const IdSets* id_sets, int64_t* err) {
+                        void* ws, void* stream, const IdSets* id_sets, int64_t* err, bool kept = false) {
     ConvPlan plans[kMaxGroups];
     if (!build_plans(d, plans)) return RBR_ERR_BAD_ARG;
     if (!ids || !W || !pidx) { set_error("null pointer"); return RBR_ERR_BAD_ARG; }
@@ -1273,7 +1374,20 @@
     ZeroRegions zr{{reinterpret_cast<int*>(S.base + S.Lo.used), S.sched_p + 2 * (size_t)S.pp[0].total_wt,
                     sched + 2 * (size_t)plans[0].total_wt},
                    {(long)((S.Lo.row_of_token - S.Lo.used) / sizeof(int)), kSchedCounters, kSchedCounters}};
-    if (id_sets != nullptr) {
+    const long n_tok = (long)d->n_docs * d->L;
+    const int nb_scan = (plans[0].total_wt + 255) / 256;
+    const int nb_mark = (int)std::min<long>((n_tok + 255) / 256, 2048);
+    if (kept) {
+        if (mask == nullptr && plans[0].pad_runs >= 0) {
+            set_error("prod_prepare_ids_kept: an un-masked conv with RBR_CONV_PAD_RUNS scans the clean ids (use prod_prepare_ids)");
+            return RBR_ERR_UNSUPPORTED;
+        }
+        const long long rest = id_sets->first[id_sets->count] - n_tok;
+        const int nb_rest = (int)std::min<long long>((rest + 255) / 256, 2048);
+        hipLaunchKernelGGL(mark_scan_ids_kernel, dim3(nb_scan + nb_mark + nb_rest), dim3(256), 0, st, plans[0], nb_scan, nb_mark, n_tok,
+                           *id_sets, reinterpret_cast<long long*>(err), mask, sched, S.counter + kKeptSlabs, S.used, d->V);
+        RBR_CHECK_LAUNCH("textcnn mark_scan_ids launch");
+    } else if (id_sets != nullptr) {
         const long long total = id_sets->first[id_sets->count];
         const int nb_ids = (int)std::min<long long>((total + 255) / 256, 2048);
         const long nz = zr.n[0] + zr.n[1] + zr.n[2];
@@ -1283,10 +1397,8 @@
     } else if (int e = zero_regions(zr, st)) {
         return e;
     }
-    const long n_tok = (long)d->n_docs * d->L;
-    const int nb_scan = (plans[0].total_wt + 255) / 256;
-    const int nb_mark = (int)std::min<long>((n_tok + 255) / 256, 2048);
-    if (int e_ = rbr::launch<mark_scan_kernel, 256>(dim3(nb_scan + nb_mark), dim3(256), 0, st, "textcnn mark_scan launch", plans[0], nb_scan, n_tok, reinterpret_cast<const long long*>(ids), mask, sched, S.used)) return e_;
+    if (!kept)
+        if (int e_ = rbr::launch<mark_scan_kernel, 256>(dim3(nb_scan + nb_mark), dim3(256), 0, st, "textcnn mark_scan launch", plans[0], nb_scan, n_tok, reinterpret_cast<const long long*>(ids), mask, sched, S.used)) return e_;
     PackJob J{};
     J.P = S.pp[0]; J.n_widths = d->n_widths; J.D = d->D; J.cp_real = S.A.cp_real;
     for (int w = 0; w < d->n_widths; ++w) { J.kz[w] = d->kz[w]; J.ch[w] = d->ch[w]; J.poff[w] = S.A.poff[w]; }
@@ -1299,6 +1411,18 @@
     const long n_pack = (b16 ? (long)JB.ngroups * JB.nchunks * 4 * 64 : (long)S.pp[0].nchunks * S.pp[0].tiles_total * kTile * S.pp[0].DC) +
                         (long)S.A.cp_real * d->D;
     const int nb_pack = (int)std::min<long>((n_pack + 255) / 256, 2048);
+    if (kept) {
+        const bool tb16 = prod_t_bf16(d);
+        float* zero_row = tb16 ? reinterpret_cast<float*>(reinterpret_cast<unsigned short*>(S.T) + (size_t)S.Lo.cap * S.A.pitch)
+                               : S.T + (size_t)S.Lo.cap * S.A.pitch;
+        const KeptState KS{S.counter + kKeptTicket, S.counter + kKeptSlabs, sched + 2 * (size_t)plans[0].total_wt, S.counter,
+                           (int)(align256((size_t)d->V) / 16), (int)align256((size_t)S.Lo.cap)};
+        hipLaunchKernelGGL(compact_pack_kept_kernel, dim3(nb_compact + nb_pack), dim3(256), 0, st, J, nb_compact, d->V, S.Lo.cap, S.used,
+                           S.row_of_token, S.tok_of_row, S.row_mask, S.counter, zero_row, tb16 ? S.A.pitch / 2 : S.A.pitch, wp,
+                           b16 ? nullptr : S.packed_p, S.WT, JB, b16 ? reinterpret_cast<unsigned char*>(S.base + S.Lo.bimg) : nullptr, KS);
+        RBR_CHECK_LAUNCH("textcnn compact_pack_kept launch");
+        return 0;
+    }
     if (int e_ = rbr::launch<compact_pack_kernel, 256>(dim3(nb_compact + nb_pack), dim3(256), 0, st, "textcnn compact_pack launch", J, nb_compact, d->V, S.Lo.cap, S.used, S.row_of_token, S.tok_of_row, S.row_mask, S.counter, prod_t_bf16(d) ? reinterpret_cast<float*>(reinterpret_cast<unsigned short*>(S.T) + (size_t)S.Lo.cap * S.A.pitch)
                                       : S.T + (size_t)S.Lo.cap * S.A.pitch, prod_t_bf16(d) ? S.A.pitch / 2 : S.A.pitch, wp, b16 ? nullptr : S.packed_p, S.WT, JB, b16 ? reinterpret_cast<unsigned char*>(S.base + S.Lo.bimg) : nullptr)) return e_;
     return 0;
@@ -1320,6 +1444,37 @@
     const bool two = n_sets >= 2 && sets[0].out == ids && sets[1].out == sets[0].out + sets[0].n && sets[0].n + sets[1].n == n_tok;
     if (!one && !two) { set_error("prod_prepare_ids: `ids` is not the clean copy of the first id set(s)"); return RBR_ERR_BAD_ARG; }
     return prod_prepare(d, ids, mask, W, pidx, ws, stream, &S, err);
+}
+
+extern "C" int rbr_textcnn_prod_prepare_ids_kept(const rbr_textcnn_desc* d, int32_t n_sets, const rbr_id_set* sets, int64_t* err,
+                                                 const int64_t* ids, const uint8_t* mask, const float* const* W, int32_t* pidx,
+                                                 void* ws, void* stream) {
+    if (!err) { set_error("null err"); return RBR_ERR_BAD_ARG; }
+    if (pair_region_open()) { set_error("prod_prepare_ids_kept: not inside a pair region"); return RBR_ERR_UNSUPPORTED; }
+    IdSets S;
+    if (int e = fill_id_sets(n_sets, sets, S)) return e;
+    const long long n_tok = (long long)d->n_docs * d->L;
+    const bool one = sets[0].out == ids && sets[0].n == n_tok;
+    const bool two = n_sets >= 2 && sets[0].out == ids && sets[1].out == sets[0].out + sets[0].n && sets[0].n + sets[1].n == n_tok;
+    if (!one && !two) { set_error("prod_prepare_ids_kept: `ids` is not the clean copy of the first id set(s)"); return RBR_ERR_BAD_ARG; }
+    for (int s = 0; s < (one ? 1 : 2); ++s)
+        if (S.limit[s] > d->V || S.replace[s] < 0 || S.replace[s] >= d->V) {
+            set_error("prod_prepare_ids_kept: token set %d has limit %lld / replacement %lld outside the table of %d rows", s,
+                      S.limit[s], S.replace[s], d->V);
+            return RBR_ERR_BAD_ARG;
+        }
+    return prod_prepare(d, ids, mask, W, pidx, ws, stream, &S, err, true);
+}
+
+extern "C" int rbr_textcnn_prod_list_state(const rbr_textcnn_desc* d, int64_t off[6]) {
+    if (!off) { set_error("null pointer"); return RBR_ERR_BAD_ARG; }
+    if (!prod_applicable(d)) { set_error("token-product path does not apply to this shape"); return RBR_ERR_UNSUPPORTED; }
+    ProdLayout Lo;
+    if (!prod_layout(d, Lo)) return RBR_ERR_BAD_ARG;
+    off[0] = (int64_t)Lo.used; off[1] = (int64_t)align256((size_t)d->V);
+    off[2] = (int64_t)Lo.row_mask; off[3] = (int64_t)align256((size_t)Lo.cap);
+    off[4] = (int64_t)(Lo.counter + kKeptTicket * sizeof(int)); off[5] = (int64_t)((kKeptSlabs - kKeptTicket + 1) * sizeof(int));
+    return 0;
 }
 
 namespace {
diff --git a/review-based-recommender_amd/functional.py b/review-based-recommender_amd/functional.py
--- a/review-based-recommender_amd/functional.py
+++ b/review-based-recommender_amd/functional.py
@@ -274,7 +274,85 @@
     return table_c, ids, mask8, ws, _conv_desc(table_c, ids.shape[0], ids.shape[1], ws, pad_mode, act, padding_idx, flags)
 
 
-def _conv_fwd_buffers(rec, desc, dev, feat=None, argmax=None):
+_KEPT_WS: dict = {}
+_KEPT_OWNER: list = []
+
+
+def _kept_state(desc):
+    off = (C.c_int64 * 6)()
+    check(_lib.lib().rbr_textcnn_prod_list_state(C.byref(desc), off), "rbr_textcnn_prod_list_state")
+    return tuple((int(off[k]), int(off[k + 1])) for k in (0, 2, 4))
+
+
+class _KeptWs:
+    def __init__(self, state, nbytes, dev):
+        self.buf = torch.empty(nbytes, dtype=torch.uint8, device=dev)
+        self.busy, self.state = False, state
+        self.zero()
+
+    def fits(self, state, nbytes) -> bool:
+        return self.buf.numel() == nbytes and self.state == state
+
+    def zero(self):
+        for o, n in self.state:
+            self.buf[o:o + n].zero_()
+        self.dirty = False
+
+
+class _KeptLease:
+    def __init__(self, ws):
+        self.ws = ws
+        ws.busy = True
+
+    def __del__(self):
+        self.ws.busy = False
+
+
+@contextlib.contextmanager
+def kept_ws_owner(owned: list):
+    _KEPT_OWNER.append(owned)
+    try:
+        yield owned
+    finally:
+        _KEPT_OWNER.pop()
+
+
+def _kept_ws_checkout(desc, nbytes, dev):
+    if os.environ.get("RBR_PREP_TWO_LAUNCH", "1") == "0":
+        return None
+    idx = dev.index if dev.index is not None else torch.cuda.current_device()
+    free = _KEPT_WS.setdefault((idx, torch.cuda.current_stream(idx).cuda_stream), [])
+    capturing = torch.cuda.is_current_stream_capturing()
+    if capturing and not _KEPT_OWNER:
+        return None
+    state = _kept_state(desc)
+    ws = next((w for w in free if not w.busy and w.fits(state, nbytes) and not (capturing and w.dirty)), None)
+    if ws is None:
+        if capturing:
+            return None
+        ws = _KeptWs(state, nbytes, dev)
+        free.append(ws)
+    elif ws.dirty:
+        ws.zero()
+    t = ws.buf[:]
+    t._kept = ws
+    if capturing:
+        free.remove(ws)
+        _KEPT_OWNER[-1].append(ws)
+    else:
+        t._kept_lease = _KeptLease(ws)
+    return t
+
+
+def _kept_ws_prepare_stream(dev, idx) -> None:
+    cur = _KEPT_WS.setdefault((idx, torch.cuda.current_stream(idx).cuda_stream), [])
+    seen = {(w.buf.numel(), w.state) for (d, _), lst in list(_KEPT_WS.items()) if d == idx for w in lst}
+    for n, state in seen:
+        if not any(c.fits(state, n) and not c.busy and not c.dirty for c in cur):
+            cur.append(_KeptWs(state, n, dev))
+
+
+def _conv_fwd_buffers(rec, desc, dev, feat=None, argmax=None, kept=False):
     L_ = _lib.lib()
     n_part = L_.rbr_textcnn_partial_elems(C.byref(desc))
     if not n_part:
@@ -285,7 +363,9 @@
     rec.pidx = torch.empty(n_part, dtype=I32, device=dev)
     rec.feat = feat if feat is not None else torch.empty(desc.n_docs, Ctot, dtype=F32, device=dev)
     rec.argmax = argmax if argmax is not None else torch.empty(desc.n_docs, Ctot, dtype=I32, device=dev)
-    rec.prod_ws = torch.empty(ws_bytes, dtype=torch.uint8, device=dev) if ws_bytes else None
+    rec.prod_ws = (_kept_ws_checkout(desc, ws_bytes, dev) if kept else None) if ws_bytes else None
+    if rec.prod_ws is None and ws_bytes:
+        rec.prod_ws = torch.empty(ws_bytes, dtype=torch.uint8, device=dev)
     return rec
 
 
@@ -293,7 +373,15 @@
     L_ = _lib.lib()
     d, wsp = C.byref(desc), rec.prod_ws.data_ptr()
     ids_p, mask_p, pidx_p = dev_ptr(ids, I64, "ids"), dev_ptr(mask8, U8, "mask"), dev_ptr(rec.pidx, I32, "pidx")
-    if id_sets is not None:
+    kept = getattr(rec.prod_ws, "_kept", None) if id_sets is not None else None
+    if kept is not None:
+        try:
+            _call(prepare_key, L_.rbr_textcnn_prod_prepare_ids_kept, d, *id_sets, ids_p, mask_p, ptr_array(ws, F32, "conv weight"),
+                  pidx_p, wsp, st)
+        except Exception:
+            kept.dirty = True
+            raise
+    elif id_sets is not None:
         _call(prepare_key, L_.rbr_textcnn_prod_prepare_ids, d, *id_sets, ids_p, mask_p, ptr_array(ws, F32, "conv weight"), pidx_p,
               wsp, st)
     else:
@@ -760,8 +848,8 @@
 
 class _LossRequest:
 
-    def __init__(self, target):
-        self.target, self.pred_ptr, self.loss = target, None, None
+    def __init__(self, target, after_backward: bool = False):
+        self.target, self.pred_ptr, self.loss, self.after_backward = target, None, None, bool(after_backward)
 
     def loss_for(self, pred: torch.Tensor):
         if self.loss is not None and self.pred_ptr == pred.data_ptr() and pred.numel() == self.target.numel():
@@ -773,8 +861,8 @@
 
 
 @contextlib.contextmanager
-def fused_loss(target: torch.Tensor):
-    req = _LossRequest(target)
+def fused_loss(target: torch.Tensor, after_backward: bool = False):
+    req = _LossRequest(target, after_backward)
     _LOSS_REQUEST.append(req)
     try:
         yield req
@@ -801,6 +889,7 @@
     need = max((t.numel() for (d, _), t in _PS_WS.items() if d == idx), default=0)
     if need:
         _pair_softmax_ws(dev, need)
+    _kept_ws_prepare_stream(dev, idx)
 
 
 def encode_head_applicable(table, n_docs, L, kernel_sizes, channels, padding_idx) -> bool:
@@ -816,7 +905,9 @@
 class _EncodeHead(torch.autograd.Function):
 
     @staticmethod
-    def forward(ctx, table, id_sets, ids, mask, u_id, i_id, drop, target, padding_idx, pad_u, pad_i, n_widths, first, *params):
+    def forward(ctx, table, id_sets, ids, mask, u_id, i_id, drop, target, padding_idx, pad_u, pad_i, n_widths, first, opts,
+                *params):
+        defer_loss, own_ws = opts
         bs_ = [b.contiguous() for b in params[n_widths:2 * n_widths]]
         head = [t.contiguous() for t in params[2 * n_widths:]]
         L_ = _lib.lib()
@@ -842,7 +933,7 @@
             u_id, i_id = u_id.contiguous(), i_id.contiguous()
         table_c, ids, mask8, ws_, desc = _conv_operands(table, ids, mask, params[:n_widths], PAD_SAME, ACT_RELU, padding_idx)
         B = ids.shape[0] // 2
-        conv = _conv_fwd_buffers(_ConvSaved(), desc, dev)
+        conv = _conv_fwd_buffers(_ConvSaved(), desc, dev, kept=own_ws and sets is not None)
         if conv.prod_ws is None:
             check(-1, "encode_head plan (encode_head_applicable() was not consulted)")
         pval, pidx, feat, argmax = conv.pval, conv.pidx, conv.feat, conv.argmax
@@ -874,6 +965,10 @@
             if training and first is None and os.environ.get("RBR_HEAD_BWD_IN_FWD", "1") != "0" \
                     and L_.rbr_pair_head_fwd_pool_lds_bytes(C.byref(desc), K, 1):
                 d_feat_unit = torch.empty(2 * B, feat.shape[1], dtype=F32, device=dev)
+        ctx.deferred = None
+        if d_feat_unit is not None and defer_loss and os.environ.get("RBR_LOSS_IN_BWD", "1") != "0":
+            ctx.deferred = (pred.detach(), target, loss.detach())
+        ticketed = target is not None and ctx.deferred is None
         _call("pair_head_fwd_pool", L_.rbr_pair_head_fwd_pool_ex, C.byref(desc), dev_ptr(pval, F32, "pval"), dev_ptr(pidx, I32, "pidx"),
               ptr_array(bs_, F32, "conv bias"), dev_ptr(feat, F32, "feat"), dev_ptr(argmax, I32, "argmax"),
               dev_ptr(first, I64, "first"), K, dev_ptr(u_id, I64, "u_id"), dev_ptr(i_id, I64, "i_id"), C.byref(hp),
@@ -882,7 +977,7 @@
               dev_ptr(drop_t, F32, "drop") if p_drop > 0.0 else None, dev_ptr(flat_zero, F32, "zero_buf"),
               acc_n, dev_ptr(ul, F32, "ul"), dev_ptr(il, F32, "il"), dev_ptr(pred, F32, "pred"),
               dev_ptr(target, F32, "target"), dev_ptr(loss, F32, "loss"), dev_ptr(d_unit, F32, "d_unit"),
-              _ticket(dev).data_ptr() if target is not None else None, dev_ptr(d_feat_unit, F32, "d_feat_unit"), st)
+              _ticket(dev).data_ptr() if ticketed else None, dev_ptr(d_feat_unit, F32, "d_feat_unit"), st)
         ctx.d_feat_unit = d_feat_unit
         ctx.conv = _ConvSaved(table=table_c, ids=ids, packed=None, feat=feat, argmax=argmax, mask8=mask8, gate=None, ws=ws_,
                               desc=desc, prod_ws=conv.prod_ws, fanout_acc=None)
@@ -902,10 +997,15 @@
         S = ctx.conv
         dev = S.table.device
         L_ = _lib.lib()
-        need_conv = any(ctx.needs_input_grad[13:13 + 2 * n_widths]) or ctx.needs_input_grad[0]
+        need_conv = any(ctx.needs_input_grad[14:14 + 2 * n_widths]) or ctx.needs_input_grad[0]
         unit = _UNIT.get(dev)
         early = (ctx.d_feat_unit is not None and need_conv and d_pred is None and ctx.first is None and d_loss is not None
                  and unit is not None and d_loss.data_ptr() == unit.data_ptr())
+        deferred = ctx.deferred
+        if deferred is not None and not early:
+            _call(None, L_.rbr_mse_loss_fwd, B, dev_ptr(deferred[0], F32, "pred"), dev_ptr(deferred[1], F32, "target"),
+                  dev_ptr(deferred[2], F32, "loss"), dev_ptr(d_unit, F32, "d_pred_unit"), current_stream())
+            deferred = None
         if d_loss is not None:
             g = d_unit if (unit is not None and d_loss.data_ptr() == unit.data_ptr()) else d_unit * d_loss
             d_pred = g if d_pred is None else d_pred + g
@@ -924,6 +1024,13 @@
         feat = S.feat
 
         def head_bwd():
+            if deferred is not None:
+                _call(None, L_.rbr_pair_head_bwd_ex, B, H, K, dev_ptr(feat[:B], F32, "u_feat"), dev_ptr(feat[B:], F32, "i_feat"),
+                      dev_ptr(u_id, I64, "u_id"), dev_ptr(i_id, I64, "i_id"), C.byref(hp), dev_ptr(drop_t, F32, "drop"),
+                      dev_ptr(ul, F32, "ul"), dev_ptr(il, F32, "il"), None, pad_u, pad_i, C.byref(hg), None, None,
+                      dev_ptr(deferred[0], F32, "pred"), dev_ptr(deferred[1], F32, "target"), dev_ptr(deferred[2], F32, "loss"),
+                      dev_ptr(d_unit, F32, "d_pred_unit"), current_stream())
+                return
             _call(None, L_.rbr_pair_head_bwd, B, H, K, dev_ptr(feat[:B], F32, "u_feat"), dev_ptr(feat[B:], F32, "i_feat"),
                   dev_ptr(u_id, I64, "u_id"), dev_ptr(i_id, I64, "i_id"), C.byref(hp), dev_ptr(drop_t, F32, "drop"),
                   dev_ptr(ul, F32, "ul"), dev_ptr(il, F32, "il"), dev_ptr(d_pred, F32, "d_pred"), pad_u, pad_i, C.byref(hg),
@@ -932,7 +1039,7 @@
 
         if early:
             dtable, _, dWs, dbs = _textcnn_backward(S, d_pair, ctx.needs_input_grad[0], False, side_job=head_bwd)
-            return (dtable, None, None, None, None, None, None, None, None, None, None, None, None, *dWs, *dbs, *grads)
+            return (dtable, None, None, None, None, None, None, None, None, None, None, None, None, None, *dWs, *dbs, *grads)
         head_bwd()
         if need_conv and ctx.first is not None:
             _call(None, L_.rbr_dedup_fold_rows, 2 * B, H, dev_ptr(ctx.first, I64, "first"), dev_ptr(d_pair, F32, "d_feat"),
@@ -941,11 +1048,11 @@
             dtable, _, dWs, dbs = _textcnn_backward(S, d_pair, ctx.needs_input_grad[0], False)
         else:
             dtable, dWs, dbs = None, [None] * n_widths, [None] * n_widths
-        return (dtable, None, None, None, None, None, None, None, None, None, None, None, None, *dWs, *dbs, *grads)
+        return (dtable, None, None, None, None, None, None, None, None, None, None, None, None, None, *dWs, *dbs, *grads)
 
 
 def encode_head(table, ids, mask, u_id, i_id, conv_weights, conv_biases, head_params, *, id_sets=None, drop=None,
-                padding_idx=0, pad_u=0, pad_i=0, first=None):
+                padding_idx=0, pad_u=0, pad_i=0, first=None, own_workspace=False):
     req = _LOSS_REQUEST[-1] if _LOSS_REQUEST else None
     target = None
     if req is not None and req.loss is None and req.target.is_cuda and req.target.dtype == F32 and req.target.dim() == 1 \
@@ -954,7 +1061,8 @@
         if req.target.shape[0] == B:
             target = req.target
     pred, loss = _EncodeHead.apply(table, id_sets, ids, mask, u_id, i_id, drop, target, padding_idx, pad_u, pad_i,
-                                   len(conv_weights), first, *conv_weights, *conv_biases, *head_params)
+                                   len(conv_weights), first, (target is not None and req.after_backward, bool(own_workspace)),
+                                   *conv_weights, *conv_biases, *head_params)
     if target is not None:
         req.pred_ptr, req.loss = pred.data_ptr(), loss
     return pred
diff --git a/review-based-recommender_amd/models/deepconn/deepconn.py b/review-based-recommender_amd/models/deepconn/deepconn.py
--- a/review-based-recommender_amd/models/deepconn/deepconn.py
+++ b/review-based-recommender_amd/models/deepconn/deepconn.py
@@ -51,7 +51,7 @@
                         (i_ids, self.item_size, 0)]
                 preds = RF.encode_head(self.word_embeddings.weight, None, masks, None, None, conv.weights(), conv.biases(), head,
                                        id_sets=sets, drop=drop, padding_idx=pad, pad_u=fm.user_padding_idx, pad_i=fm.item_padding_idx,
-                                       first=first)
+                                       first=first, own_workspace=True)
             else:
                 preds = RF.encode_head(self.word_embeddings.weight, RF.stack_rows(u_revs, i_revs), masks, u_ids, i_ids,
                                        conv.weights(), conv.biases(), head, drop=drop, padding_idx=pad,
diff --git a/review-based-recommender_amd/train_step.py b/review-based-recommender_amd/train_step.py
--- a/review-based-recommender_amd/train_step.py
+++ b/review-based-recommender_amd/train_step.py
@@ -223,7 +223,7 @@
     scope = optimizer.row_grad_scope() if isinstance(optimizer, HipClipAdam) else contextlib.nullcontext()
     fusable = ratings.is_cuda and ratings.dtype == torch.float32
     with scope:
-        with (RF.fused_loss(ratings) if fusable else contextlib.nullcontext()) as req:
+        with (RF.fused_loss(ratings, after_backward=True) if fusable else contextlib.nullcontext()) as req:
             out = model(*batch)
             pred = out[0] if isinstance(out, tuple) else out
             loss = req.loss_for(pred) if req is not None else None
@@ -392,7 +392,8 @@
         torch.cuda.synchronize()
         self.graph = torch.cuda.CUDAGraph()
         self._capture_stream = _capture_stream(batch[0].device)
-        with torch.no_grad(), _lib_mod().capture_guard(self._capture_stream), \
+        self._kept_ws = []
+        with torch.no_grad(), _lib_mod().capture_guard(self._capture_stream), RF.kept_ws_owner(self._kept_ws), \
                 torch.cuda.graph(self.graph, stream=self._capture_stream, capture_error_mode=capture_error_mode):
             self._prologue()
             out = model(*self.batch)
@@ -517,17 +518,24 @@
         mode = capture_error_mode or ("thread_local" if grad_sync is not None else "global")
         self._capture_stream = _capture_stream(ratings.device)
         cs = self._capture_stream
+        self._kept_ws = []
         for sl in self._slots:
+            if sl is not first:
+                with torch.cuda.stream(cs):
+                    RF.prepare_stream_state(ratings.device)
+                torch.cuda.synchronize(ratings.device)
             optimizer.zero_grad(set_to_none=True)
             sl.g_fwd_bwd = torch.cuda.CUDAGraph(keep_graph=True) if self._keep_graph else torch.cuda.CUDAGraph()
             if grad_sync is None:
-                with _lib_mod().capture_guard(cs), torch.cuda.graph(sl.g_fwd_bwd, stream=cs, capture_error_mode=mode):
+                with _lib_mod().capture_guard(cs), RF.kept_ws_owner(self._kept_ws), \
+                        torch.cuda.graph(sl.g_fwd_bwd, stream=cs, capture_error_mode=mode):
                     self._prologue(sl)
                     sl.loss, sl.gnorm, sl.pred = train_step(model, optimizer, sl.batch, sl.ratings, max_grad_norm,
                                                             objective=objective)
                 sl.static_grads = [(p, p.grad) for p in model.parameters()]
             else:
-                with _lib_mod().capture_guard(cs), torch.cuda.graph(sl.g_fwd_bwd, stream=cs, capture_error_mode=mode):
+                with _lib_mod().capture_guard(cs), RF.kept_ws_owner(self._kept_ws), \
+                        torch.cuda.graph(sl.g_fwd_bwd, stream=cs, capture_error_mode=mode):
                     self._prologue(sl)
                     optimizer.zero_grad()
                     pred, loss = _forward_loss_backward(model, sl.batch, sl.ratings)
```
